# dafyddstephenson/ucla-roms

Hardware: AMD Instinct MI355X
Metric: grid-cell-updates/sec (higher is better)
Workload: dtype f64; 1 GPU; C3: basin 1024x1024x100, NONLIN+SPLIT EOS, T+S, LMD KPP/BKPP/RIMIX/NONLOCAL, dt=300s, ndtfast=60 (nfast=82); NT=2, nfast=82, parallelism=domain decomposition 1x1, halo_transport=none (single rank), fast_exchange_interval=1, exchange_order=none (single rank), s2d_window=True, comm_bootstrap=none (single rank)

## Files before the change

### include/roms_gpu.h

```cpp
#ifndef ROMS_GPU_H
#define ROMS_GPU_H

#ifdef __cplusplus
extern "C" {
#endif

#define ROMS_GPU_ABI_VERSION 20
#define ROMS_MAX_FAST 288

typedef struct roms_dims {
  int Lm, Mm, N, NT;
  int LLm, MMm;
  int np_xi, np_eta, inode, jnode;
  int iSW_corn, jSW_corn;
  int ew_periodic, ns_periodic;
  int west_exchng, east_exchng, south_exchng, north_exchng;
} roms_dims;

#define ROMS_LMD_MIXING   1
#define ROMS_LMD_KPP      2
#define ROMS_LMD_BKPP     4
#define ROMS_LMD_RIMIX    8
#define ROMS_LMD_CONVEC   16
#define ROMS_LMD_NONLOCAL 32
#define ROMS_LMD_ALL      63
#define ROMS_LMD_ICELAND  47
#define ROMS_LMD_DDMIX    64

typedef struct roms_cfg {
  int nonlin_eos;
  int salinity;
  int lmd_mixing;
  int uv_vis2, ts_dif2;
  double dt;
  int ndtfast, nfast;
  double weight[2][ROMS_MAX_FAST];
  double g, rho0, rdrg, rdrg2, Zob, gamma2;
  double Akv_bak, Akt_bak[2];
  double Tcoef, T0, Scoef, S0;
  double theta_s, theta_b, hc;
  int obc;
  double ubind;
  int curvgrid;
  int uv_adv, uv_cor;
  int pot_tides;
  int bulk_frc;
  int adv_isoneutral;
} roms_cfg;

typedef struct roms_tlev {
  int iic, ntstart, forw_start, iif, nfast, kstp, knew, nstp, nrhs, nnew;
} roms_tlev;

enum roms_field {
  ROMS_ALL = -1,
  ROMS_h = 0, ROMS_hinv, ROMS_f, ROMS_fomn, ROMS_pm, ROMS_pn, ROMS_dm_r, ROMS_dn_r, ROMS_dm_u, ROMS_dn_u,
  ROMS_dm_v, ROMS_dn_v, ROMS_dm_p, ROMS_dn_p, ROMS_pmon_u, ROMS_pnom_v, ROMS_rmask, ROMS_pmask, ROMS_umask,
  ROMS_vmask,
  ROMS_Cs_w, ROMS_Cs_r,
  ROMS_zeta, ROMS_ubar, ROMS_vbar, ROMS_u, ROMS_v, ROMS_t, ROMS_FlxU, ROMS_FlxV, ROMS_We, ROMS_Wi,
  ROMS_Hz, ROMS_Hz_u, ROMS_Hz_v, ROMS_z_r, ROMS_z_w,
  ROMS_rufrc, ROMS_rvfrc, ROMS_rhoA, ROMS_rhoS, ROMS_r_D, ROMS_Zt_avg1, ROMS_DU_avg1, ROMS_DV_avg1,
  ROMS_DU_avg2, ROMS_DV_avg2, ROMS_DU_avg_bak, ROMS_DV_avg_bak,
  ROMS_rho, ROMS_rho1, ROMS_qp1, ROMS_bvf, ROMS_Akv, ROMS_Akt, ROMS_visc2_r, ROMS_visc2_p, ROMS_diff2,
  ROMS_hbls, ROMS_hbbl, ROMS_ghat, ROMS_swr_frac,
  ROMS_sustr, ROMS_svstr, ROMS_stflx, ROMS_srflx, ROMS_swflx,
  ROMS_ru, ROMS_rv,
  ROMS_zeta_west, ROMS_zeta_east, ROMS_zeta_south, ROMS_zeta_north,
  ROMS_ubar_west, ROMS_ubar_east, ROMS_ubar_south, ROMS_ubar_north,
  ROMS_vbar_west, ROMS_vbar_east, ROMS_vbar_south, ROMS_vbar_north,
  ROMS_u_west, ROMS_u_east, ROMS_u_south, ROMS_u_north,
  ROMS_v_west, ROMS_v_east, ROMS_v_south, ROMS_v_north,
  ROMS_t_west, ROMS_t_east, ROMS_t_south, ROMS_t_north,
  ROMS_dndx, ROMS_dmde,
  ROMS_ptide,
  ROMS_uwnd, ROMS_vwnd, ROMS_tair, ROMS_qair, ROMS_prate, ROMS_swrad, ROMS_lwrad, ROMS_sustr_r, ROMS_svstr_r,
  ROMS_NFIELDS
};

int  roms_gpu_abi_version(void);
int  roms_gpu_init(const roms_dims *dims, const roms_cfg *cfg, int device, void *comm);
int  roms_gpu_finalize(void);
const char *roms_gpu_last_error(void);
long roms_gpu_field_size(int field_id);
int  roms_gpu_register(int field_id, double *host_ptr, long count);
int  roms_gpu_upload(int field_id);
int  roms_gpu_download(int field_id);
int  roms_gpu_copy_in(int field_id, const double *src, long count);
int  roms_gpu_copy_out(int field_id, double *dst, long count);
int  roms_gpu_sync(void);
void *roms_gpu_stream(void);

int roms_gpu_rho_eos(int tidx, const roms_tlev *t);
int roms_gpu_set_huv(const roms_tlev *t);
int roms_gpu_omega(const roms_tlev *t);
int roms_gpu_lmd_vmix(int tind, const roms_tlev *t);
int roms_gpu_prsgrd(const roms_tlev *t);
int roms_gpu_pre_step3d(const roms_tlev *t);
int roms_gpu_set_huv1(const roms_tlev *t);
int roms_gpu_step3d_uv1(const roms_tlev *t);
int roms_gpu_visc3d(const roms_tlev *t);
int roms_gpu_step2d(const roms_tlev *t);
int roms_gpu_step3d_uv2(const roms_tlev *t);
int roms_gpu_step3d_t(const roms_tlev *t);
int roms_gpu_t3dmix(const roms_tlev *t);
int roms_gpu_swr_frac(const roms_tlev *t);
int roms_gpu_set_pipe_frc(int npip, const int *pipe_idx, const double *pipe_flx, const double *pipe_prf,
                          const double *pipe_trc);
int roms_gpu_set_river_frc(int nriv, const double *riv_uflx, const double *riv_vflx, const double *riv_vol,
                           const double *riv_trc);
int roms_gpu_bulk_flux(const roms_tlev *t);
int roms_gpu_set_ub_tune(const double *ub_west, const double *ub_east, const double *ub_south, const double *ub_north);
int roms_gpu_set_depth(const roms_tlev *t);

int roms_gpu_step(roms_tlev *t);
int roms_gpu_init_sequence(roms_tlev *t);

enum roms_case_id { ROMS_CASE_FILAMENT = 0, ROMS_CASE_BASIN = 1, ROMS_CASE_PIPES = 2, ROMS_CASE_RIVERS = 3 };
typedef struct roms_case {
  int case_id, LLm, MMm, N, NT;
  int salinity, nonlin_eos, lmd_mixing;
  double dt; int ndtfast;
  double sizex, sizey;
  int surf_flux;
  int obc;
  double v_sponge;
  int island;
  int curvgrid;
  int uv_adv, uv_cor;
  int bulk_frc;
  int adv_isoneutral;
} roms_case;
int roms_gpu_init_case(const roms_case *c, int device, roms_tlev *t);
int roms_gpu_init_case_comm(const roms_case *c, int np_xi, int np_eta, void *comm, int device, roms_tlev *t);

int roms_gpu_comm_unique_id(void *id128);
int roms_gpu_comm_create(const void *id128, int nranks, int rank, int device, void **comm);
int roms_gpu_comm_create_local(int group, int nranks, int rank, void **comm);
typedef int (*roms_host_allgather_fn)(void *ctx, const void *send, long nbytes, void *recv);
int roms_gpu_comm_create_host(int nranks, int rank, int device, roms_host_allgather_fn allgather, void *ctx,
                              void **comm);
int roms_gpu_comm_destroy(void *comm);
int roms_gpu_halo_transport(void);
int roms_gpu_halo_exchanges(long *per_step, int *fast_interval);
int roms_gpu_halo_overlap(void);
int roms_gpu_s2d_window(void);
#define ROMS_COLPATH_SEG 1
#define ROMS_COLPATH_GLOBAL 2
int roms_gpu_column_path(void);
int roms_gpu_kpp_lean(void);
int roms_gpu_vgrid(void);
int roms_gpu_vgrid_check(long out[3]);
int roms_gpu_horizontal_path(int out[8]);
int roms_gpu_selftest_zero_fill(long n, int chunks, long *bad);
int roms_gpu_halo_plan(int Lm, int Mm, int np_xi, int np_eta, int inode, int jnode, int ew_periodic,
                       int ns_periodic, int peer[8], long count[8], int strip[4]);
long roms_gpu_halo_map(int Lm, int Mm, int np_xi, int np_eta, int inode, int jnode, int ew_periodic,
                       int ns_periodic, int dir, int unpack, int *i, int *j, long cap);
long roms_gpu_halo_map_wide(int Lm, int Mm, int np_xi, int np_eta, int inode, int jnode, int ew_periodic,
                            int ns_periodic, int width, int dir, int unpack, int *i, int *j, long cap);

#define ROMS_FRC_SURFACE 1
#define ROMS_FRC_BRY     2
int roms_gpu_frc_record(int field_id, int slot, double rec_time, const double *data);
int roms_gpu_frc_interp(double modtime, int kinds);
int roms_gpu_frc_clock(double start_time, int on);
int roms_gpu_set_tide_data(int ntides, const double *ftide, const double *pot_re, const double *pot_im,
                           const double *ztide_re, const double *ztide_im, const double *utide_re,
                           const double *utide_im, const double *vtide_re, const double *vtide_im);
int roms_gpu_set_tides(double time);

#define ROMS_WRT_Z    1
#define ROMS_WRT_UB   2
#define ROMS_WRT_VB   4
#define ROMS_WRT_U    8
#define ROMS_WRT_V    16
#define ROMS_WRT_T    32
#define ROMS_WRT_R    64
#define ROMS_WRT_O    128
#define ROMS_WRT_AKV  256
#define ROMS_WRT_AKT  512
#define ROMS_WRT_AKS  1024
#define ROMS_WRT_HBLS 2048
#define ROMS_WRT_HBBL 4096
#define ROMS_WRT_DEFAULT 63
int roms_gpu_wrt_rst(const char *path, int rec, int total_rec, double time, const roms_tlev *t);
int roms_gpu_wrt_his(const char *path, int rec, int total_rec, double time, const roms_tlev *t, int wrt_mask);
int roms_gpu_io_wait(void);
int roms_gpu_io_tracer_name(int itrc, const char *name, const char *units, const char *long_name);
int roms_gpu_get_init(const char *path, int req_rec, int tindx, roms_tlev *t, double *start_time);

int roms_gpu_diag(const roms_tlev *t, double norms[4]);
int roms_gpu_set_weights(int ndtfast, double weight[2][ROMS_MAX_FAST]);
int roms_gpu_time_steps(roms_tlev *t, int n, double *ms);
enum roms_routine {
  ROMS_R_RHO_EOS = 0, ROMS_R_SET_HUV, ROMS_R_OMEGA, ROMS_R_PRSGRD, ROMS_R_PRE_STEP3D, ROMS_R_SET_HUV1,
  ROMS_R_STEP3D_UV1, ROMS_R_VISC3D, ROMS_R_STEP2D, ROMS_R_STEP3D_UV2, ROMS_R_STEP3D_T, ROMS_R_T3DMIX,
  ROMS_R_LMD_VMIX,
  ROMS_R_K_S2D_FB,
  ROMS_R_K_PRE_UV_SEG,
  ROMS_R_K_UV1_SEG,
  ROMS_R_K_STEP3D_T_SEG,
  ROMS_R_K_PRSGRD_UV,
  ROMS_R_K_HALO_PACK,
  ROMS_R_K_HALO_WAIT,
  ROMS_R_K_HALO_UNPACK,
  ROMS_R_COUNT
};
int roms_gpu_time_routine(int routine, int nsteps, roms_tlev *t, double *avg_ms, long *launches);

#ifdef __cplusplus
}
#endif
#endif
```

### ucla-roms_amd/csrc/k_chain.h

```cpp
#pragma once
#include "roms_dev.h"

namespace roms {

constexpr int kChainCW = 16;
constexpr int kChainG = 4;

struct ChainLane {
  int col, g;
  int i, j;
  int lo, nk;
  bool in;
};
template <int KL>
__device__ __forceinline__ ChainLane chain_lane(const Range& R, const uint3& bI, int N) {
  ChainLane c;
  const int l = (int)(threadIdx.x & 63u), w = (int)(threadIdx.x >> 6);
  c.col = l & (kChainCW - 1);
  c.g = l / kChainCW;
  c.i = tile_i0(R.i0) + (int)bI.x * kChainCW + c.col;
  c.in = c.i >= R.i0;
  c.j = R.j0 + (int)bI.y * 4 + w;
  c.lo = 1 + c.g * KL;
  c.nk = max(0, min(N, c.lo + KL - 1) - c.lo + 1);
  return c;
}
inline dim3 chain_grid_of(const Range& R) {
  return dim3((R.i1 - tile_i0(R.i0) + kChainCW) / kChainCW, (R.j1 - R.j0 + 4) / 4);
}
inline int chain_kl(int N) {
  const int kl = (N + kChainG - 1) / kChainG;
  return kl <= 5 ? 5 : kl <= 13 ? 13 : kl <= 25 ? 25 : 0;
}

template <class Body>
__device__ __forceinline__ void chain_down(const ChainLane& c, double& s1, double& s2, Body&& body) {
  s1 = 0.0; s2 = 0.0;
#pragma unroll
  for (int st = kChainG - 1; st >= 0; st--) {
    const double in1 = __shfl_down(s1, kChainCW), in2 = __shfl_down(s2, kChainCW);
    if (c.g == st) {
      if (st < kChainG - 1) { s1 = in1; s2 = in2; }
      body(s1, s2);
    }
  }
  s1 = __shfl(s1, c.col);
  s2 = __shfl(s2, c.col);
}
template <class Body>
__device__ __forceinline__ void chain_up(const ChainLane& c, double& s, Body&& body) {
  s = 0.0;
#pragma unroll
  for (int st = 0; st < kChainG; st++) {
    const double in = __shfl_up(s, kChainCW);
    if (c.g == st) {
      if (st > 0) s = in;
      body(s);
    }
  }
  s = __shfl(s, (kChainG - 1) * kChainCW + c.col);
}

}
```

### ucla-roms_amd/csrc/k_step3d_t.hip

```cpp
#include "k_colseg.h"

namespace roms {

__global__ void __launch_bounds__(256) k_step3d_t_h(Dev d, Range R, int nnew, int nrhs, int up) {
  const uint3 bI = xcd_tile();
  __shared__ TracerWin W;
  const Bounds& b = d.b;
  const Fields& F = d.f;
  const int k = 1 + (int)bI.z;
  const int i0 = tile_i0(R.i0) + (int)bI.x * kBX, j0 = R.j0 + (int)bI.y * kBY;
  const int ib = i0 - 2, jb = j0 - 2;
  const long kk = (long)(k - 1) * b.n2;
  tracer_win_fill(b, F, W, ib, jb, kk, nullptr);
  const int i = i0 + (int)threadIdx.x, j = j0 + (int)threadIdx.y;
  const bool act = i >= R.i0 && i <= R.i1 && j <= R.j1;
  const long ij = IJ(b, i, j), o = ij + kk;
  const AccTL a{W.T, W.UM, W.VM, W.FU, W.FV, ib, jb};
  for (int itrc = 1; itrc <= b.NT; itrc++) {
    const long tb = (long)(itrc - 1) * 3 * b.n3;
    const double* Tr = F.t + (long)(nrhs - 1) * b.n3 + tb;
    __syncthreads();
    tracer_win_fill(b, F, W, ib, jb, kk, Tr);
    __syncthreads();
    if (!act) continue;
// ... 435 lines not shown
    const double c = DC0 * LD(Wi, vo, w);
    fc = in ? f : 0.0;
    wc = in ? c : 0.0;
  };
  double fcl, wcl;
  fcw(0, fcl, wcl);
  __syncthreads();
  SegTri<KR> T;
  T.template eliminate<ROMS_SEG_T_GROUP>(n, [&](int p, double& a, double& bb, double& c, double& dd) {
    double fcu, wcu;
    fcw(p + 1, fcu, wcu);
    a = -(fcl + fmax0(wcl));
    bb = hz[p + 1] + fcu + fmax0(wcu) + fcl - fmin0(wcl);
    c = -(fcu - fmin0(wcu));
    dd = rhs[p];
    fcl = fcu; wcl = wcu;
  });
  double xL, xR;
  T.couple(sg, n, X, xL, xR);
  T.solve(n, xL, xR);
  const double rm = BufF64(F.rmask).ld(vo, 0);
  const unsigned vs = act ? vo : kBufOff;
#pragma unroll
  for (int p = 0; p < KR; p++) Tn.st(T.D[p] * rm, (p < n ? vs : kBufOff) + lev(c0 + p), 0u);
}

void setup_column_kernels_t(size_t bytes) {
  (void)hipFuncSetAttribute((const void*)k_step3d_t_v<ColLds>, hipFuncAttributeMaxDynamicSharedMemorySize,
                            (int)bytes);
  (void)hipFuncSetAttribute((const void*)k_step3d_t_v<ColLds, true>, hipFuncAttributeMaxDynamicSharedMemorySize,
                            (int)bytes);
}

void launch_step3d_t(const Dev& d, hipStream_t s, const Tlev& t, bool exchange) {
  const Bounds& b = d.b;
  Range R{b.istr, b.iend, b.jstr, b.jend};
  if (d.p.iso) {
    hipLaunchKernelGGL(k_step3d_t_h, grid3_of(R, b.N), dim3(kBX, kBY), 0, s, d, R, t.nnew, t.nrhs, 0);
    for (int itrc = 1; itrc <= b.NT; itrc++) launch_iso_tracer(d, s, t, itrc);
    dim3 gt = gridc_of(R);
    gt.z = b.NT;
    if (d.f.colscr)
      hipLaunchKernelGGL((k_step3d_t_v<ColGlb, true>), gt, dim3(kCX), 0, s, d, R, t.nnew, t.nrhs);
    else
      hipLaunchKernelGGL((k_step3d_t_v<ColLds, true>), gt, dim3(kCX), col_lds_bytes(2, b.N), s, d, R, t.nnew, t.nrhs);
    for (int itrc = 1; itrc <= b.NT; itrc++) launch_t3dbc(d, s, t, itrc);
    launch_exchange_tracers(d, s, t.nnew);
    return;
  }
  auto h_tiles = [&](const Range& r) {
    const dim3 gh = grid3_of(r, b.N), bh(kBX, kBY);
    if (d.p.hoist && b.NT == 2)
      hipLaunchKernelGGL(k_step3d_t_h1<2>, gh, bh, 0, s, d, r, t.nnew, t.nrhs);
    else if (d.p.hoist && b.NT == 1)
      hipLaunchKernelGGL(k_step3d_t_h1<1>, gh, bh, 0, s, d, r, t.nnew, t.nrhs);
    else
      hipLaunchKernelGGL(k_step3d_t_h, gh, bh, 0, s, d, r, t.nnew, t.nrhs, 1);
  };
  auto run = [&](const Range& r) {
    int jA = 0, jB = -1;
    if (d.p.hoist && launch_tracer_strip(d, s, r, 0, true, false, t.nnew, t.nrhs, 0.0, 0.0, 0.0, 0, jA, jB)) {
      if (jA > r.j0) h_tiles(Range{r.i0, r.i1, r.j0, jA - 1});
      if (jB < r.j1) h_tiles(Range{r.i0, r.i1, jB + 1, r.j1});
    } else {
      h_tiles(r);
    }
    dim3 gt = gridc_of(r);
    gt.z = b.NT;
    if (d.p.colseg) {
      ktimer_mark(s, kTimedStep3dTSeg, 0);
      if (d.p.seg_buf)
        hipLaunchKernelGGL(k_step3d_t_segb, seg_grid_of(r, b.NT), dim3(kCX, seg_waves(b.N)), 0, s, d, r, t.nnew, t.nrhs);
      else
        hipLaunchKernelGGL(k_step3d_t_seg, seg_grid_of(r, b.NT), dim3(kCX, seg_waves(b.N)), 0, s, d, r, t.nnew, t.nrhs);
      ktimer_mark(s, kTimedStep3dTSeg, 1, 1);
    }
    else if (d.f.colscr)
      hipLaunchKernelGGL(k_step3d_t_v<ColGlb>, gt, dim3(kCX), 0, s, d, r, t.nnew, t.nrhs);
    else
      hipLaunchKernelGGL(k_step3d_t_v<ColLds>, gt, dim3(kCX), col_lds_bytes(2, b.N), s, d, r, t.nnew, t.nrhs);
  };
  auto edges = [&] {
    for (int itrc = 1; itrc <= b.NT; itrc++) launch_t3dbc(d, s, t, itrc);
  };
  ExchList L;
  if (!exchange) {
    run(R);
    edges();
  } else if (tracer_exch_list(d, t.nnew, L)) {
    launch_rim_first(d, s, R, L, run, edges);
  } else {
    run(R);
    edges();
    launch_exchange_tracers(d, s, t.nnew);
  }
}

__global__ void __launch_bounds__(256) k_t3dmix(Dev d, Range R, int nnew, int nrhs) {
  ROMS_IJ_OR_RETURN(R)
  const Bounds& b = d.b;
  const Fields& F = d.f;
  const long ij = IJ(b, i, j), sj = b.nx2, n2 = b.n2;
  const double* __restrict__ Hz = F.Hz;
  const double pmn = d.p.dt * F.pm[ij] * F.pn[ij];
  if (b.NT == 2) {
    double ax0[2], ax1[2], ay0[2], ay1[2];
    const double* __restrict__ Tr[2];
    double* __restrict__ Tn[2];
#pragma unroll
    for (int q = 0; q < 2; q++) {
      const double* d2 = F.diff2 + (long)q * n2;
      Tr[q] = F.t + (long)(nrhs - 1) * b.n3 + (long)q * 3 * b.n3;
      Tn[q] = F.t + (long)(nnew - 1) * b.n3 + (long)q * 3 * b.n3;
      ax0[q] = 0.25 * (d2[ij] + d2[ij - 1]) * F.pmon_u[ij];
      ax1[q] = 0.25 * (d2[ij + 1] + d2[ij]) * F.pmon_u[ij + 1];
      ay0[q] = 0.25 * (d2[ij] + d2[ij - sj]) * F.pnom_v[ij];
      ay1[q] = 0.25 * (d2[ij + sj] + d2[ij]) * F.pnom_v[ij + sj];
    }
    const double um0 = F.umask[ij], um1 = F.umask[ij + 1], vm0 = F.vmask[ij], vm1 = F.vmask[ij + sj];
#pragma unroll 2
    for (int k = 1; k <= b.N; k++) {
      const long o = ij + (long)(k - 1) * n2;
#pragma unroll
      for (int q = 0; q < 2; q++) {
        const double FX1 = ax1[q] * (Hz[o + 1] + Hz[o]) * (Tr[q][o + 1] - Tr[q][o]) * um1;
        const double FX0 = ax0[q] * (Hz[o] + Hz[o - 1]) * (Tr[q][o] - Tr[q][o - 1]) * um0;
        const double FE1 = ay1[q] * (Hz[o + sj] + Hz[o]) * (Tr[q][o + sj] - Tr[q][o]) * vm1;
        const double FE0 = ay0[q] * (Hz[o] + Hz[o - sj]) * (Tr[q][o] - Tr[q][o - sj]) * vm0;
        Tn[q][o] = Tn[q][o] + pmn * (FX1 - FX0 + FE1 - FE0) / Hz[o];
      }
    }
    return;
  }
  for (int itrc = 1; itrc <= b.NT; itrc++) {
    const double* d2 = F.diff2 + (long)(itrc - 1) * n2;
    const double* __restrict__ Tr = F.t + (long)(nrhs - 1) * b.n3 + (long)(itrc - 1) * 3 * b.n3;
    double* __restrict__ Tn = F.t + (long)(nnew - 1) * b.n3 + (long)(itrc - 1) * 3 * b.n3;
    const double ax0 = 0.25 * (d2[ij] + d2[ij - 1]) * F.pmon_u[ij], ax1 = 0.25 * (d2[ij + 1] + d2[ij]) * F.pmon_u[ij + 1];
    const double ay0 = 0.25 * (d2[ij] + d2[ij - sj]) * F.pnom_v[ij], ay1 = 0.25 * (d2[ij + sj] + d2[ij]) * F.pnom_v[ij + sj];
    const double um0 = F.umask[ij], um1 = F.umask[ij + 1], vm0 = F.vmask[ij], vm1 = F.vmask[ij + sj];
#pragma unroll 2
    for (int k = 1; k <= b.N; k++) {
      const long o = ij + (long)(k - 1) * n2;
      const double FX1 = ax1 * (Hz[o + 1] + Hz[o]) * (Tr[o + 1] - Tr[o]) * um1;
      const double FX0 = ax0 * (Hz[o] + Hz[o - 1]) * (Tr[o] - Tr[o - 1]) * um0;
      const double FE1 = ay1 * (Hz[o + sj] + Hz[o]) * (Tr[o + sj] - Tr[o]) * vm1;
      const double FE0 = ay0 * (Hz[o] + Hz[o - sj]) * (Tr[o] - Tr[o - sj]) * vm0;
      Tn[o] = Tn[o] + pmn * (FX1 - FX0 + FE1 - FE0) / Hz[o];
    }
  }
}

constexpr int kTMW = kBX + 2, kTMN = kTMW * (kBY + 2), kTMQ = (3 * kTMN + kBX * kBY - 1) / (kBX * kBY);
__global__ void __launch_bounds__(256) k_t3dmix_stg(Dev d, Range R, int nnew, int nrhs) {
  const uint3 bI = xcd_tile();
  __shared__ double sW[3 * kTMN];
  const Bounds& b = d.b;
  const Fields& F = d.f;
  const int i0 = tile_i0(R.i0) + (int)bI.x * kBX, j0 = R.j0 + (int)bI.y * kBY;
  int i = i0 + (int)threadIdx.x, j = j0 + (int)threadIdx.y;
  const bool act = i >= R.i0 && i <= R.i1 && j <= R.j1;
  if (!act) { i = i < R.i0 ? R.i0 : (i < R.i1 ? i : R.i1); j = j < R.j1 ? j : R.j1; }
  const long ij = IJ(b, i, j), sj = b.nx2, n2 = b.n2;
  const int tid = threadIdx.x + kBX * threadIdx.y;
  const double pmn = d.p.dt * F.pm[ij] * F.pn[ij];
  double ax0[2], ax1[2], ay0[2], ay1[2];
  double* __restrict__ Tn[2];
  const double* Tr[2];
#pragma unroll
  for (int q = 0; q < 2; q++) {
    const double* d2 = F.diff2 + (long)q * n2;
    Tr[q] = F.t + (long)(nrhs - 1) * b.n3 + (long)q * 3 * b.n3;
    Tn[q] = F.t + (long)(nnew - 1) * b.n3 + (long)q * 3 * b.n3;
    ax0[q] = 0.25 * (d2[ij] + d2[ij - 1]) * F.pmon_u[ij];
    ax1[q] = 0.25 * (d2[ij + 1] + d2[ij]) * F.pmon_u[ij + 1];
    ay0[q] = 0.25 * (d2[ij] + d2[ij - sj]) * F.pnom_v[ij];
    ay1[q] = 0.25 * (d2[ij + sj] + d2[ij]) * F.pnom_v[ij + sj];
  }
  const double um0 = F.umask[ij], um1 = F.umask[ij + 1], vm0 = F.vmask[ij], vm1 = F.vmask[ij + sj];
  long wo[kTMQ];
  int wf[kTMQ];
#pragma unroll
  for (int m = 0; m < kTMQ; m++) {
    const int q = tid + m * kBX * kBY;
    const int f = q < 3 * kTMN ? q / kTMN : -1, qq = q - (f < 0 ? 0 : f) * kTMN;
    const int ii = i0 - 1 + qq % kTMW, jj = j0 - 1 + qq / kTMW;
    const bool ok = f >= 0 && ii >= -1 && ii <= b.Lm + 2 && jj >= -1 && jj <= b.Mm + 2;
    wf[m] = ok ? f : -1;
    wo[m] = ok ? IJ(b, ii, jj) : 0;
  }
  auto ldw = [&](int k, double (&x)[kTMQ]) {
    const long kk = (long)(k - 1) * n2;
#pragma unroll
    for (int m = 0; m < kTMQ; m++)
      x[m] = wf[m] == 0 ? F.Hz[wo[m] + kk] : wf[m] == 1 ? Tr[0][wo[m] + kk] : wf[m] == 2 ? Tr[1][wo[m] + kk] : 0.0;
  };
  const int c = (threadIdx.x + 1) + (threadIdx.y + 1) * kTMW;
  double w[kTMQ];
  ldw(1, w);
  for (int k = 1; k <= b.N; k++) {
    const long o = ij + (long)(k - 1) * n2;
    const double tn0 = Tn[0][o], tn1 = Tn[1][o];
    if (k > 1) __syncthreads();
#pragma unroll
    for (int m = 0; m < kTMQ; m++) {
      const int q = tid + m * kBX * kBY;
      if (q < 3 * kTMN) sW[q] = w[m];
    }
    if (k < b.N) ldw(k + 1, w);
    __syncthreads();
    const double* H = sW;
    const double hz = H[c];
#pragma unroll
    for (int q = 0; q < 2; q++) {
      const double* T = sW + (1 + q) * kTMN;
      const double FX1 = ax1[q] * (H[c + 1] + hz) * (T[c + 1] - T[c]) * um1;
      const double FX0 = ax0[q] * (hz + H[c - 1]) * (T[c] - T[c - 1]) * um0;
      const double FE1 = ay1[q] * (H[c + kTMW] + hz) * (T[c + kTMW] - T[c]) * vm1;
      const double FE0 = ay0[q] * (hz + H[c - kTMW]) * (T[c] - T[c - kTMW]) * vm0;
      if (act) Tn[q][o] = (q == 0 ? tn0 : tn1) + pmn * (FX1 - FX0 + FE1 - FE0) / hz;
    }
  }
}

void launch_t3dmix(const Dev& d, hipStream_t s, const Tlev& t) {
  const Bounds& b = d.b;
  Range R{b.istr, b.iend, b.jstr, b.jend};
  const bool stg = d.p.t3dmix_stg && b.NT == 2;
  auto run = [&](const Range& r) {
    if (stg) hipLaunchKernelGGL(k_t3dmix_stg, grid_of(r), dim3(kBX, kBY), 0, s, d, r, t.nnew, t.nrhs);
    else hipLaunchKernelGGL(k_t3dmix, grid_of(r), dim3(kBX, kBY), 0, s, d, r, t.nnew, t.nrhs);
  };
  ExchList L;
  if (tracer_exch_list(d, t.nnew, L)) {
    launch_rim_first(d, s, R, L, run, [] {});
  } else {
    run(R);
    launch_exchange_tracers(d, s, t.nnew);
  }
}

}
```

### ucla-roms_amd/csrc/k_step3d_uv.hip

```cpp
#include <vector>

#include "k_colseg.h"
#include "k_chain.h"

namespace roms {

void launch_uv_horiz(const Dev& d, hipStream_t s, int nrhs, int up);

#ifndef ROMS_UV1_PF
#define ROMS_UV1_PF 8
#endif
constexpr int kUv1PF = ROMS_UV1_PF;
template <class C>
__device__ __forceinline__ void uv1_col(const Dev& d, int i, int j, int dir, int nnew, int nrhs, const C& A,
                                        const C& B) {
  const Bounds& b = d.b;
  const Fields& F = d.f;
  const int N = b.N;
  const double dt = d.p.dt;
  const long n2 = b.n2, ij = IJ(b, i, j);
  const long s = dir == 0 ? 1 : b.nx2;
  uv_vert_flux_lds<(kUv1PF > 0)>(d, ij, nrhs, dir, A, B);
  double* __restrict__ Un = (dir == 0 ? F.u : F.v) + (long)(nnew - 1) * b.n3 + ij;
  double* __restrict__ rr = (dir == 0 ? F.ru : F.rv) + ij;
// ... 375 lines not shown
    hipLaunchKernelGGL(k_uv1<ColLds>, g, dim3(kCX), col_lds_bytes(2, b.N), s, d, R, t.nnew, t.nrhs);
}

__device__ __forceinline__ void visc_rho(const Dev& d, int i, int j, int k, int nstp, double& UFx, double& VFe) {
  const Bounds& b = d.b;
  const Fields& F = d.f;
  const long ij = IJ(b, i, j), o = ij + (long)(k - 1) * b.n2, l = (long)(nstp - 1) * b.n3;
  const double* pm = F.pm;
  const double* pn = F.pn;
  const long sj = b.nx2;
  const double cff = 0.5 * F.Hz[o] * F.visc2_r[ij] *
                     (F.dn_r[ij] * pm[ij] * ((pn[ij] + pn[ij + 1]) * F.u[o + 1 + l] - (pn[ij - 1] + pn[ij]) * F.u[o + l]) -
                      F.dm_r[ij] * pn[ij] * ((pm[ij] + pm[ij + sj]) * F.v[o + sj + l] - (pm[ij - sj] + pm[ij]) * F.v[o + l]));
  UFx = cff * F.dn_r[ij] * F.dn_r[ij];
  VFe = -cff * F.dm_r[ij] * F.dm_r[ij];
}
__device__ __forceinline__ void visc_psi(const Dev& d, int i, int j, int k, int nstp, double& UFe, double& VFx) {
  const Bounds& b = d.b;
  const Fields& F = d.f;
  const long sj = b.nx2;
  const long ij = IJ(b, i, j), o = ij + (long)(k - 1) * b.n2, l = (long)(nstp - 1) * b.n3;
  const double* pm = F.pm;
  const double* pn = F.pn;
  const double cff =
      0.125 * (F.Hz[o - 1] + F.Hz[o] + F.Hz[o - 1 - sj] + F.Hz[o - sj]) * F.visc2_p[ij] *
      (0.25 * (pm[ij - 1] + pm[ij] + pm[ij - 1 - sj] + pm[ij - sj]) * F.dn_p[ij] *
           ((pn[ij - sj] + pn[ij]) * F.v[o + l] - (pn[ij - 1 - sj] + pn[ij - 1]) * F.v[o - 1 + l]) +
       0.25 * (pn[ij - 1] + pn[ij] + pn[ij - 1 - sj] + pn[ij - sj]) * F.dm_p[ij] *
           ((pm[ij - 1] + pm[ij]) * F.u[o + l] - (pm[ij - 1 - sj] + pm[ij - sj]) * F.u[o - sj + l])) *
      F.pmask[ij];
  UFe = cff * F.dm_p[ij] * F.dm_p[ij];
  VFx = cff * F.dn_p[ij] * F.dn_p[ij];
}

constexpr int kVW = kBX + 1, kVN = kVW * (kBY + 1), kVQ = (kVN + kBX * kBY - 1) / (kBX * kBY);
struct ViscRho {
  double v2, X, sx1, sx0, Y, sy1, sy0, dn, dm;
  long ij;
  bool on;
};
struct ViscPsi {
  double v2, P1, P2, a1, a0, b1, b0, msk, dm, dn;
  long ij;
  bool on;
};
__global__ void __launch_bounds__(256) k_visc3d(Dev d, Range R, int nstp) {
  const uint3 bI = xcd_tile();
  __shared__ double sUFx[kVN], sVFe[kVN], sUFe[kVN], sVFx[kVN];
  const Bounds& b = d.b;
  const Fields& F = d.f;
  const int indx = 3 - nstp;
  const int i0 = tile_i0(R.i0) + (int)bI.x * kBX, j0 = R.j0 + (int)bI.y * kBY;
  const long sj = b.nx2;
  const double* pm = F.pm;
  const double* pn = F.pn;
  const int tid = threadIdx.x + kBX * threadIdx.y;
  ViscRho gr[kVQ];
  ViscPsi gp[kVQ];
#pragma unroll
  for (int m = 0; m < kVQ; m++) {
    const int q = tid + m * kBX * kBY;
    const int li = q % kVW, lj = q / kVW;
    const int ir = i0 - 1 + li, jr = j0 - 1 + lj;
    ViscRho& r = gr[m];
    r.on = q < kVN && ir >= 0 && ir <= b.Lm + 1 && jr >= 0 && jr <= b.Mm + 1;
    r.ij = IJ(b, ir, jr);
    if (r.on) {
      const long ij = r.ij;
      r.v2 = F.visc2_r[ij];
      r.X = F.dn_r[ij] * pm[ij]; r.sx1 = pn[ij] + pn[ij + 1]; r.sx0 = pn[ij - 1] + pn[ij];
      r.Y = F.dm_r[ij] * pn[ij]; r.sy1 = pm[ij] + pm[ij + sj]; r.sy0 = pm[ij - sj] + pm[ij];
      r.dn = F.dn_r[ij]; r.dm = F.dm_r[ij];
    }
    const int ip = i0 + li, jp = j0 + lj;
    ViscPsi& p = gp[m];
    p.on = q < kVN && ip >= 0 && ip <= b.Lm + 2 && jp >= 0 && jp <= b.Mm + 2;
    p.ij = IJ(b, ip, jp);
    if (p.on) {
      const long ij = p.ij;
      p.v2 = F.visc2_p[ij];
      p.P1 = 0.25 * (pm[ij - 1] + pm[ij] + pm[ij - 1 - sj] + pm[ij - sj]) * F.dn_p[ij];
      p.a1 = pn[ij - sj] + pn[ij]; p.a0 = pn[ij - 1 - sj] + pn[ij - 1];
      p.P2 = 0.25 * (pn[ij - 1] + pn[ij] + pn[ij - 1 - sj] + pn[ij - sj]) * F.dm_p[ij];
      p.b1 = pm[ij - 1] + pm[ij]; p.b0 = pm[ij - 1 - sj] + pm[ij - sj];
      p.msk = F.pmask[ij]; p.dm = F.dm_p[ij]; p.dn = F.dn_p[ij];
    }
  }
  const int i = i0 + (int)threadIdx.x, j = j0 + (int)threadIdx.y;
  const bool act = i >= R.i0 && i <= R.i1 && j <= R.j1;
  const long ij = IJ(b, i, j);
  const bool du = act && i >= b.istrU && i <= b.iend, dv = act && j >= b.jstrV && j <= b.jend;
  double cum = 0.0, cun = 0.0, cvm = 0.0, cvn = 0.0, fu = 0.0, fv = 0.0;
  if (du) { cum = pm[ij - 1] + pm[ij]; cun = pn[ij - 1] + pn[ij]; fu = F.rufrc[ij]; }
  if (dv) { cvm = pm[ij] + pm[ij - sj]; cvn = pn[ij] + pn[ij - sj]; fv = F.rvfrc[ij]; }
  const double cu0 = 0.125 * cum * cun, cv0 = 0.125 * cvm * cvn;
  const double* U = F.u + (long)(nstp - 1) * b.n3;
  const double* V = F.v + (long)(nstp - 1) * b.n3;
  double* Ui = F.u + (long)(indx - 1) * b.n3;
  double* Vi = F.v + (long)(indx - 1) * b.n3;
  const int qr = (threadIdx.x + 1) + (threadIdx.y + 1) * kVW;
  const int qp = threadIdx.x + threadIdx.y * kVW;
  for (int k = 1; k <= b.N; k++) {
    const long kk = (long)(k - 1) * b.n2;
    const double* Hk = F.Hz + kk;
    const double* Uk = U + kk;
    const double* Vk = V + kk;
    const double ui = du ? Ui[ij + kk] : 0.0, vi = dv ? Vi[ij + kk] : 0.0;
    if (k > 1) __syncthreads();
#pragma unroll
    for (int m = 0; m < kVQ; m++) {
      const int q = tid + m * kBX * kBY;
      if (q >= kVN) break;
      double ufx = 0.0, vfe = 0.0, ufe = 0.0, vfx = 0.0;
      const ViscRho& r = gr[m];
      if (r.on) {
        const long o = r.ij;
        const double cff = 0.5 * Hk[o] * r.v2 * (r.X * (r.sx1 * Uk[o + 1] - r.sx0 * Uk[o]) -
                                                 r.Y * (r.sy1 * Vk[o + sj] - r.sy0 * Vk[o]));
        ufx = cff * r.dn * r.dn;
        vfe = -cff * r.dm * r.dm;
      }
      const ViscPsi& p = gp[m];
      if (p.on) {
        const long o = p.ij;
        const double cff = 0.125 * (Hk[o - 1] + Hk[o] + Hk[o - 1 - sj] + Hk[o - sj]) * p.v2 *
                           (p.P1 * (p.a1 * Vk[o] - p.a0 * Vk[o - 1]) + p.P2 * (p.b1 * Uk[o] - p.b0 * Uk[o - sj])) *
                           p.msk;
        ufe = cff * p.dm * p.dm;
        vfx = cff * p.dn * p.dn;
      }
      sUFx[q] = ufx; sVFe[q] = vfe; sUFe[q] = ufe; sVFx[q] = vfx;
    }
    __syncthreads();
    const long o = ij + kk;
    if (du) {
      const double cff = cu0 * (cun * (sUFx[qr] - sUFx[qr - 1]) + cum * (sUFe[qp + kVW] - sUFe[qp]));
      Ui[o] = ui + d.p.dt * cff;
      fu = fu + cff;
    }
    if (dv) {
      const double cff = cv0 * (cvn * (sVFx[qp + 1] - sVFx[qp]) + cvm * (sVFe[qr] - sVFe[qr - kVW]));
      Vi[o] = vi + d.p.dt * cff;
      fv = fv + cff;
    }
  }
  if (du) F.rufrc[ij] = fu;
  if (dv) F.rvfrc[ij] = fv;
}

constexpr int kVUW = kBX + 3, kVUN = kVUW * (kBY + 2);
constexpr int kVVW = kBX + 2, kVVN = kVVW * (kBY + 3);
constexpr int kVHW = kBX + 2, kVHN = kVHW * (kBY + 2);
constexpr int kVSN = kVUN + kVVN + kVHN, kVSQ = (kVSN + kBX * kBY - 1) / (kBX * kBY);
__global__ void __launch_bounds__(256, 3) k_visc3d_stg(Dev d, Range R, int nstp) {
  const uint3 bI = xcd_tile();
  __shared__ double sUFx[kVN], sVFe[kVN], sUFe[kVN], sVFx[kVN];
  __shared__ double sRaw[kVSN];
  const Bounds& b = d.b;
  const Fields& F = d.f;
  const int indx = 3 - nstp;
  const int i0 = tile_i0(R.i0) + (int)bI.x * kBX, j0 = R.j0 + (int)bI.y * kBY;
  const long sj = b.nx2;
  const double* pm = F.pm;
  const double* pn = F.pn;
  const int tid = threadIdx.x + kBX * threadIdx.y;
  ViscRho gr[kVQ];
  ViscPsi gp[kVQ];
#pragma unroll
  for (int m = 0; m < kVQ; m++) {
    const int q = tid + m * kBX * kBY;
    const int li = q % kVW, lj = q / kVW;
    const int ir = i0 - 1 + li, jr = j0 - 1 + lj;
    ViscRho& r = gr[m];
    r.on = q < kVN && ir >= 0 && ir <= b.Lm + 1 && jr >= 0 && jr <= b.Mm + 1;
    r.ij = IJ(b, ir, jr);
    if (r.on) {
      const long ij = r.ij;
      r.v2 = F.visc2_r[ij];
      r.X = F.dn_r[ij] * pm[ij]; r.sx1 = pn[ij] + pn[ij + 1]; r.sx0 = pn[ij - 1] + pn[ij];
      r.Y = F.dm_r[ij] * pn[ij]; r.sy1 = pm[ij] + pm[ij + sj]; r.sy0 = pm[ij - sj] + pm[ij];
      r.dn = F.dn_r[ij]; r.dm = F.dm_r[ij];
    }
    const int ip = i0 + li, jp = j0 + lj;
    ViscPsi& p = gp[m];
    p.on = q < kVN && ip >= 0 && ip <= b.Lm + 2 && jp >= 0 && jp <= b.Mm + 2;
    p.ij = IJ(b, ip, jp);
    if (p.on) {
      const long ij = p.ij;
      p.v2 = F.visc2_p[ij];
      p.P1 = 0.25 * (pm[ij - 1] + pm[ij] + pm[ij - 1 - sj] + pm[ij - sj]) * F.dn_p[ij];
      p.a1 = pn[ij - sj] + pn[ij]; p.a0 = pn[ij - 1 - sj] + pn[ij - 1];
      p.P2 = 0.25 * (pn[ij - 1] + pn[ij] + pn[ij - 1 - sj] + pn[ij - sj]) * F.dm_p[ij];
      p.b1 = pm[ij - 1] + pm[ij]; p.b0 = pm[ij - 1 - sj] + pm[ij - sj];
      p.msk = F.pmask[ij]; p.dm = F.dm_p[ij]; p.dn = F.dn_p[ij];
    }
  }
  const double* U = F.u + (long)(nstp - 1) * b.n3;
  const double* V = F.v + (long)(nstp - 1) * b.n3;
  long wo[kVSQ];
  int wf[kVSQ];
#pragma unroll
  for (int m = 0; m < kVSQ; m++) {
    const int q = tid + m * kBX * kBY;
    int ii = 0, jj = 0, f = -1;
    if (q < kVUN) { f = 0; ii = i0 - 1 + q % kVUW; jj = j0 - 1 + q / kVUW; }
    else if (q < kVUN + kVVN) { const int qq = q - kVUN; f = 1; ii = i0 - 1 + qq % kVVW; jj = j0 - 1 + qq / kVVW; }
    else if (q < kVSN) { const int qq = q - kVUN - kVVN; f = 2; ii = i0 - 1 + qq % kVHW; jj = j0 - 1 + qq / kVHW; }
    if (f >= 0 && !(ii >= -1 && ii <= b.Lm + 2 && jj >= -1 && jj <= b.Mm + 2)) f = -1;
    wf[m] = f;
    wo[m] = f >= 0 ? IJ(b, ii, jj) : 0;
  }
  auto ldraw = [&](int k, double (&x)[kVSQ]) {
    const long kk = (long)(k - 1) * b.n2;
#pragma unroll
    for (int m = 0; m < kVSQ; m++)
      x[m] = wf[m] == 0 ? U[wo[m] + kk] : wf[m] == 1 ? V[wo[m] + kk] : wf[m] == 2 ? F.Hz[wo[m] + kk] : 0.0;
  };
  auto Uw = [&](int ii, int jj) { return sRaw[(ii - (i0 - 1)) + (jj - (j0 - 1)) * kVUW]; };
  auto Vw = [&](int ii, int jj) { return sRaw[kVUN + (ii - (i0 - 1)) + (jj - (j0 - 1)) * kVVW]; };
  auto Hw = [&](int ii, int jj) { return sRaw[kVUN + kVVN + (ii - (i0 - 1)) + (jj - (j0 - 1)) * kVHW]; };
  const int i = i0 + (int)threadIdx.x, j = j0 + (int)threadIdx.y;
  const bool act = i >= R.i0 && i <= R.i1 && j <= R.j1;
  const long ij = IJ(b, i, j);
  const bool du = act && i >= b.istrU && i <= b.iend, dv = act && j >= b.jstrV && j <= b.jend;
  double cum = 0.0, cun = 0.0, cvm = 0.0, cvn = 0.0, fu = 0.0, fv = 0.0;
  if (du) { cum = pm[ij - 1] + pm[ij]; cun = pn[ij - 1] + pn[ij]; fu = F.rufrc[ij]; }
  if (dv) { cvm = pm[ij] + pm[ij - sj]; cvn = pn[ij] + pn[ij - sj]; fv = F.rvfrc[ij]; }
  const double cu0 = 0.125 * cum * cun, cv0 = 0.125 * cvm * cvn;
  double* Ui = F.u + (long)(indx - 1) * b.n3;
  double* Vi = F.v + (long)(indx - 1) * b.n3;
  const int qr = (threadIdx.x + 1) + (threadIdx.y + 1) * kVW;
  const int qp = threadIdx.x + threadIdx.y * kVW;
  double raw[kVSQ];
  ldraw(1, raw);
  double nui = du ? Ui[ij] : 0.0, nvi = dv ? Vi[ij] : 0.0;
  for (int k = 1; k <= b.N; k++) {
    const long kk = (long)(k - 1) * b.n2;
    const double ui = nui, vi = nvi;
#pragma unroll
    for (int m = 0; m < kVSQ; m++) {
      const int q = tid + m * kBX * kBY;
      if (q < kVSN) sRaw[q] = raw[m];
    }
    if (k < b.N) {
      ldraw(k + 1, raw);
      nui = du ? Ui[ij + kk + b.n2] : 0.0;
      nvi = dv ? Vi[ij + kk + b.n2] : 0.0;
    }
    __syncthreads();
#pragma unroll
    for (int m = 0; m < kVQ; m++) {
      const int q = tid + m * kBX * kBY;
      if (q >= kVN) break;
      const int li = q % kVW, lj = q / kVW;
      double ufx = 0.0, vfe = 0.0, ufe = 0.0, vfx = 0.0;
      const ViscRho& r = gr[m];
      if (r.on) {
        const int ir = i0 - 1 + li, jr = j0 - 1 + lj;
        const double cff = 0.5 * Hw(ir, jr) * r.v2 * (r.X * (r.sx1 * Uw(ir + 1, jr) - r.sx0 * Uw(ir, jr)) -
                                                      r.Y * (r.sy1 * Vw(ir, jr + 1) - r.sy0 * Vw(ir, jr)));
        ufx = cff * r.dn * r.dn;
        vfe = -cff * r.dm * r.dm;
      }
      const ViscPsi& p = gp[m];
      if (p.on) {
        const int ip = i0 + li, jp = j0 + lj;
        const double cff = 0.125 * (Hw(ip - 1, jp) + Hw(ip, jp) + Hw(ip - 1, jp - 1) + Hw(ip, jp - 1)) * p.v2 *
                           (p.P1 * (p.a1 * Vw(ip, jp) - p.a0 * Vw(ip - 1, jp)) +
                            p.P2 * (p.b1 * Uw(ip, jp) - p.b0 * Uw(ip, jp - 1))) *
                           p.msk;
        ufe = cff * p.dm * p.dm;
        vfx = cff * p.dn * p.dn;
      }
      sUFx[q] = ufx; sVFe[q] = vfe; sUFe[q] = ufe; sVFx[q] = vfx;
    }
    __syncthreads();
    const long o = ij + kk;
    if (du) {
      const double cff = cu0 * (cun * (sUFx[qr] - sUFx[qr - 1]) + cum * (sUFe[qp + kVW] - sUFe[qp]));
      Ui[o] = ui + d.p.dt * cff;
      fu = fu + cff;
    }
    if (dv) {
      const double cff = cv0 * (cvn * (sVFx[qp + 1] - sVFx[qp]) + cvm * (sVFe[qr] - sVFe[qr - kVW]));
      Vi[o] = vi + d.p.dt * cff;
      fv = fv + cff;
    }
  }
  if (du) F.rufrc[ij] = fu;
  if (dv) F.rvfrc[ij] = fv;
}

void launch_visc3d(const Dev& d, hipStream_t s, const Tlev& t) {
  const Bounds& b = d.b;
  Range R{b.istr, b.iend, b.jstr, b.jend};
  if (d.p.visc_stg)
    hipLaunchKernelGGL(k_visc3d_stg, grid_of(R), dim3(kBX, kBY), 0, s, d, R, t.nstp);
  else
    hipLaunchKernelGGL(k_visc3d, grid_of(R), dim3(kBX, kBY), 0, s, d, R, t.nstp);
}

__host__ __device__ __forceinline__ bool uv2_fused_in(const Bounds& b, int dir, int i, int j) {
  if (dir == 0)
    return i >= b.istrU && i <= b.iend && j >= b.jstr + (b.south_edge ? 1 : 0) && j <= b.jend - (b.north_edge ? 1 : 0);
  return i >= b.istr + (b.west_edge ? 1 : 0) && i <= b.iend - (b.east_edge ? 1 : 0) && j >= b.jstrV && j <= b.jend;
}

__global__ void __launch_bounds__(256) k_uv2_couple(Dev d, Range R, int nnew, int edges) {
  ROMS_IJ_OR_RETURN(R)
  const Bounds& b = d.b;
  const Fields& F = d.f;
  const int N = b.N;
  const long ij = IJ(b, i, j), n2 = b.n2;
  for (int dir = 0; dir < 2; dir++) {
    if (dir == 0 && !(i >= b.istrU)) continue;
    if (dir == 1 && !(j >= b.jstrV)) continue;
    if (edges && uv2_fused_in(b, dir, i, j)) continue;
    const long s = dir == 0 ? 1 : b.nx2;
    double* __restrict__ Un = (dir == 0 ? F.u : F.v) + (long)(nnew - 1) * b.n3 + ij;
    const double* __restrict__ Hz = F.Hz + ij;
    const double dn = dir == 0 ? F.dn_u[ij] : F.dm_v[ij];
    const double avg1 = dir == 0 ? F.DU_avg1[ij] : F.DV_avg1[ij];
    const double msk = dir == 0 ? F.umask[ij] : F.vmask[ij];
    long o = (long)(N - 1) * n2;
    double CF0 = 0.5 * (Hz[o] + Hz[o - s]);
    double DC0 = Un[o];
#pragma unroll 8
    for (int k = N - 1; k >= 1; k--) {
      o = (long)(k - 1) * n2;
      CF0 = CF0 + 0.5 * (Hz[o] + Hz[o - s]);
      DC0 = DC0 + Un[o];
    }
    DC0 = (DC0 * dn - avg1) / (CF0 * dn);
    constexpr int CH = 8;
    for (int k0 = 1; k0 <= N; k0 += CH) {
      double uc[CH], cc[CH];
#pragma unroll
      for (int q = 0; q < CH; q++) {
        const long oq = (long)(min(k0 + q, N) - 1) * n2;
        uc[q] = Un[oq];
        cc[q] = 0.5 * (Hz[oq] + Hz[oq - s]);
      }
#pragma unroll
      for (int q = 0; q < CH; q++)
        if (k0 + q <= N) Un[(long)(k0 + q - 1) * n2] = (uc[q] / cc[q] - DC0) * msk;
    }
  }
}

__global__ void __launch_bounds__(256) k_uv2_flux(Dev d, Range R, int nnew, int nstp, int knew, int iu0, int iu1, int iv0,
                                                  int iv1, int edges) {
  ROMS_IJ_OR_RETURN(R)
  const Bounds& b = d.b;
  const Fields& F = d.f;
  const int N = b.N;
  const long ij = IJ(b, i, j), n2 = b.n2;
  const double DELTA = 0.28, EPSIL = 0.36;
  for (int dir = 0; dir < 2; dir++) {
    if (dir == 0 && !(i >= iu0 && i <= iu1)) continue;
    if (dir == 1 && !(i >= iv0 && i <= iv1 && j >= b.jstr)) continue;
    if (edges && uv2_fused_in(b, dir, i, j)) continue;
    const long s = dir == 0 ? 1 : b.nx2;
    double* __restrict__ Un = (dir == 0 ? F.u : F.v) + (long)(nnew - 1) * b.n3 + ij;
    const double* __restrict__ Us = (dir == 0 ? F.u : F.v) + (long)(nstp - 1) * b.n3 + ij;
    double* __restrict__ Flx = (dir == 0 ? F.FlxU : F.FlxV) + ij;
    const double* __restrict__ Hz = F.Hz + ij;
    double* __restrict__ CFs = F.c0 + ij;
    const double dn = dir == 0 ? F.dn_u[ij] : F.dm_v[ij];
    const double avg1 = dir == 0 ? F.DU_avg1[ij] : F.DV_avg1[ij];
    const double avg2 = dir == 0 ? F.DU_avg2[ij] : F.DV_avg2[ij];
    const double msk = dir == 0 ? F.umask[ij] : F.vmask[ij];
    auto DCk = [&](int k) { const long o = (long)(k - 1) * n2; return 0.5 * (Hz[o] + Hz[o - s]) * dn; };
    long o = (long)(N - 1) * n2;
    const double dcN = DCk(N);
    double DC0 = dcN, FC0 = dcN * Un[o];
#pragma unroll 8
    for (int k = N - 1; k >= 1; k--) {
      o = (long)(k - 1) * n2;
      const double dck = DCk(k);
      DC0 = DC0 + dck;
      FC0 = FC0 + dck * Un[o];
    }
    DC0 = 1.0 / DC0;
    if (dir == 0) F.ubar[IJL(b, i, j, knew)] = DC0 * avg1;
    else F.vbar[IJL(b, i, j, knew)] = DC0 * avg1;
    FC0 = DC0 * (FC0 - avg1);
    double CF0 = 0.0;
    constexpr int CH = 8;
    for (int k0 = N; k0 >= 1; k0 -= CH) {
      double uc[CH], fc[CH], sc[CH], dc[CH];
#pragma unroll
      for (int q = 0; q < CH; q++) {
        const int k = max(k0 - q, 1);
        const long oq = (long)(k - 1) * n2;
        uc[q] = Un[oq]; fc[q] = Flx[oq]; sc[q] = Us[oq]; dc[q] = DCk(k);
      }
#pragma unroll
      for (int q = 0; q < CH; q++) {
        const int k = k0 - q;
        if (k >= 1) {
          const long oq = (long)(k - 1) * n2;
          const double un = (uc[q] - FC0) * msk;
          Un[oq] = un;
          const double cfk = DELTA * fc[q] + EPSIL * dc[q] * (sc[q] + un);
          CFs[(long)k * n2] = cfk;
          CF0 = CF0 + cfk;
        }
      }
    }
    CF0 = DC0 * (CF0 - avg2);
#pragma unroll 8
    for (int k = 1; k <= N; k++) {
      o = (long)(k - 1) * n2;
      Flx[o] = CFs[(long)k * n2] - DCk(k) * CF0;
    }
  }
}

template <int KL, bool FULL = false>
__global__ void __launch_bounds__(256, KL > 13 ? 3 : 4) k_uv2_fused(Dev d, Range R, int nnew, int nstp, int knew) {
  constexpr bool kHcLds = KL > 13;
  __shared__ double sHc[kHcLds ? KL * 256 : 1];
  const uint3 bI = xcd_tile();
  const Bounds& b = d.b;
  const Fields& F = d.f;
  const int N = b.N;
  const double DELTA = 0.28, EPSIL = 0.36;
  const ChainLane cl = chain_lane<KL>(R, bI, N);
  const int i = cl.i, j = cl.j, g = cl.g, lo = cl.lo, nk = FULL ? KL : cl.nk;
  const long n2 = b.n2;
  auto chain2 = [&](double& s1, double& s2, auto&& body) { chain_down(cl, s1, s2, body); };
  const int d0 = gridDim.z == 2 ? (int)bI.z : 0, d1 = gridDim.z == 2 ? d0 + 1 : 2;
  for (int dir = d0; dir < d1; dir++) {
    const int ilo = dir == 0 ? b.istrU : b.istr, jlo = dir == 0 ? b.jstr : b.jstrV;
    const int ic = min(max(i, ilo), b.iend), jc = min(max(j, jlo), b.jend);
    const bool act = ic == i && jc == j && cl.in && uv2_fused_in(b, dir, i, j);
    const long ij = IJ(b, ic, jc), s = dir == 0 ? 1 : b.nx2;
    const double dn = dir == 0 ? F.dn_u[ij] : F.dm_v[ij];
    const double avg1 = dir == 0 ? F.DU_avg1[ij] : F.DV_avg1[ij];
    const double avg2 = dir == 0 ? F.DU_avg2[ij] : F.DV_avg2[ij];
    const double msk = dir == 0 ? F.umask[ij] : F.vmask[ij];
    const double* const Ub = (dir == 0 ? F.u : F.v);
    const BufF64 bUn(Ub + (long)(nnew - 1) * b.n3, b.n3), bUs(Ub + (long)(nstp - 1) * b.n3, b.n3), bHz(F.Hz, b.n3),
        bFl(dir == 0 ? F.FlxU : F.FlxV, b.n3);
    const unsigned vo = (unsigned)((ij + (long)(lo - 1) * n2) * 8), vom = vo - (unsigned)(s * 8);
    auto so = [&](int q) { return (unsigned)((long)q * n2 * 8); };
    auto vq = [&](int q) { return q < nk ? vo : kBufOff; };
    auto vqm = [&](int q) { return q < nk ? vom : kBufOff; };
    auto vsq = [&](int q) { return act && q < nk ? vo : kBufOff; };
    double un[KL];
    double hcr[kHcLds ? 1 : KL];
    struct HcRef {
      double* l;
      double* r;
      __device__ __forceinline__ double& operator[](int q) const { return kHcLds ? l[q * 256] : r[q]; }
    } const hc{sHc + threadIdx.x, hcr};
#pragma unroll
    for (int q = 0; q < KL; q++) {
      un[q] = bUn.ld(vq(q), so(q));
      hc[q] = 0.5 * (bHz.ld(vq(q), so(q)) + bHz.ld(vqm(q), so(q)));
      if (q % 8 == 7) __builtin_amdgcn_sched_barrier(0);
    }
    double CF0, DC0;
    chain2(CF0, DC0, [&](double& a, double& c) {
#pragma unroll
      for (int q = KL - 1; q >= 0; q--) {
        a = q < nk ? a + hc[q] : a;
        c = q < nk ? c + un[q] : c;
      }
    });
    DC0 = (DC0 * dn - avg1) / (CF0 * dn);
#pragma unroll
    for (int q = 0; q < KL; q++) un[q] = (un[q] / hc[q] - DC0) * msk;
    double DS, FC0;
    chain2(DS, FC0, [&](double& a, double& c) {
#pragma unroll
      for (int q = KL - 1; q >= 0; q--) {
        const double dck = hc[q] * dn;
        a = q < nk ? a + dck : a;
        c = q < nk ? c + dck * un[q] : c;
      }
    });
    const double DCi = 1.0 / DS;
    if (act && g == 0) {
      if (dir == 0) F.ubar[IJL(b, i, j, knew)] = DCi * avg1;
      else F.vbar[IJL(b, i, j, knew)] = DCi * avg1;
    }
    FC0 = DCi * (FC0 - avg1);
    __builtin_amdgcn_sched_barrier(0);
#pragma unroll
    for (int q = 0; q < KL; q++) {
      const double u1 = (un[q] - FC0) * msk;
      bUn.st(u1, vsq(q), so(q));
      un[q] = DELTA * bFl.ld(vq(q), so(q)) + EPSIL * (hc[q] * dn) * (bUs.ld(vq(q), so(q)) + u1);
      if (q % 8 == 7) __builtin_amdgcn_sched_barrier(0);
    }
    double CS, unused;
    chain2(CS, unused, [&](double& a, double& c) {
#pragma unroll
      for (int q = KL - 1; q >= 0; q--) a = q < nk ? a + un[q] : a;
    });
    const double CF1 = DCi * (CS - avg2);
#pragma unroll
    for (int q = 0; q < KL; q++) bFl.st(un[q] - (hc[q] * dn) * CF1, vsq(q), so(q));
  }
}

template <int KL, bool kCouple>
__global__ void __launch_bounds__(256) k_uv2_edge(Dev d, const int* __restrict__ cols, int ncol, int nnew, int nstp,
                                                  int knew) {
  const Bounds& b = d.b;
  const Fields& F = d.f;
  const int N = b.N;
  const double DELTA = 0.28, EPSIL = 0.36;
  const int l = (int)(threadIdx.x & 63u), w = (int)(threadIdx.x >> 6);
  ChainLane cl;
  cl.col = l & (kChainCW - 1);
  cl.g = l / kChainCW;
  cl.lo = 1 + cl.g * KL;
  cl.nk = max(0, min(N, cl.lo + KL - 1) - cl.lo + 1);
  const int c = ((int)blockIdx.x * 4 + w) * kChainCW + cl.col;
  const bool act = c < ncol;
  const int cc = act ? c : ncol - 1;
  const int dir = cols[3 * cc], i = cols[3 * cc + 1], j = cols[3 * cc + 2];
  cl.i = i; cl.j = j; cl.in = true;
  const long n2 = b.n2, ij = IJ(b, i, j), s = dir == 0 ? 1 : b.nx2;
  auto chain2 = [&](double& s1, double& s2, auto&& body) { chain_down(cl, s1, s2, body); };
  double* __restrict__ Un = (dir == 0 ? F.u : F.v) + (long)(nnew - 1) * b.n3 + ij;
  const double* __restrict__ Hz = F.Hz + ij;
  const double dn = dir == 0 ? F.dn_u[ij] : F.dm_v[ij];
  const double avg1 = dir == 0 ? F.DU_avg1[ij] : F.DV_avg1[ij];
  const double msk = dir == 0 ? F.umask[ij] : F.vmask[ij];
  double un[KL], hc[KL];
#pragma unroll
  for (int q = 0; q < KL; q++) {
    if (q < cl.nk) {
      const long o = (long)(cl.lo + q - 1) * n2;
      un[q] = Un[o];
      hc[q] = 0.5 * (Hz[o] + Hz[o - s]);
    }
  }
  if constexpr (kCouple) {
    double CF0, DC0;
    chain2(CF0, DC0, [&](double& a, double& c2) {
#pragma unroll
      for (int q = KL - 1; q >= 0; q--)
        if (q < cl.nk) { a = a + hc[q]; c2 = c2 + un[q]; }
    });
    DC0 = (DC0 * dn - avg1) / (CF0 * dn);
    if (act) {
#pragma unroll
      for (int q = 0; q < KL; q++)
        if (q < cl.nk) Un[(long)(cl.lo + q - 1) * n2] = (un[q] / hc[q] - DC0) * msk;
    }
  } else {
    const double* __restrict__ Us = (dir == 0 ? F.u : F.v) + (long)(nstp - 1) * b.n3 + ij;
    double* __restrict__ Flx = (dir == 0 ? F.FlxU : F.FlxV) + ij;
    const double avg2 = dir == 0 ? F.DU_avg2[ij] : F.DV_avg2[ij];
    double DS, FC0;
    chain2(DS, FC0, [&](double& a, double& c2) {
#pragma unroll
      for (int q = KL - 1; q >= 0; q--)
        if (q < cl.nk) { const double dck = hc[q] * dn; a = a + dck; c2 = c2 + dck * un[q]; }
    });
    const double DCi = 1.0 / DS;
    if (act && cl.g == 0) {
      if (dir == 0) F.ubar[IJL(b, i, j, knew)] = DCi * avg1;
      else F.vbar[IJL(b, i, j, knew)] = DCi * avg1;
    }
    FC0 = DCi * (FC0 - avg1);
#pragma unroll
    for (int q = 0; q < KL; q++) {
      if (q < cl.nk) {
        const long o = (long)(cl.lo + q - 1) * n2;
        const double u1 = (un[q] - FC0) * msk;
        if (act) Un[o] = u1;
        un[q] = DELTA * Flx[o] + EPSIL * (hc[q] * dn) * (Us[o] + u1);
      }
    }
    double CS, unused;
    chain2(CS, unused, [&](double& a, double& c2) {
#pragma unroll
      for (int q = KL - 1; q >= 0; q--)
        if (q < cl.nk) a = a + un[q];
    });
    const double CF1 = DCi * (CS - avg2);
    if (act) {
#pragma unroll
      for (int q = 0; q < KL; q++)
        if (q < cl.nk) Flx[(long)(cl.lo + q - 1) * n2] = un[q] - (hc[q] * dn) * CF1;
    }
  }
}

void uv2_edge_lists(const Bounds& b, std::vector<int>& couple, std::vector<int>& flux) {
  couple.clear();
  flux.clear();
  if (!(b.west_edge || b.east_edge || b.south_edge || b.north_edge)) return;
  const int iu0 = b.istr, iu1 = b.ew_periodic ? b.iend : b.iendR;
  const int iv0 = b.ew_periodic ? b.istr : b.istrR, iv1 = b.ew_periodic ? b.iend : b.iendR;
  const int j0 = b.ns_periodic ? b.jstr : b.jstrR, j1 = b.ns_periodic ? b.jend : b.jendR;
  for (int dir = 0; dir < 2; dir++)
    for (int j = b.jstr; j <= b.jend; j++)
      for (int i = b.istr; i <= b.iend; i++) {
        if (dir == 0 && !(i >= b.istrU)) continue;
        if (dir == 1 && !(j >= b.jstrV)) continue;
        if (uv2_fused_in(b, dir, i, j)) continue;
        couple.insert(couple.end(), {dir, i, j});
      }
  for (int dir = 0; dir < 2; dir++)
    for (int j = j0; j <= j1; j++)
      for (int i = (iv0 < iu0 ? iv0 : iu0); i <= (iu1 > iv1 ? iu1 : iv1); i++) {
        if (dir == 0 && !(i >= iu0 && i <= iu1)) continue;
        if (dir == 1 && !(i >= iv0 && i <= iv1 && j >= b.jstr)) continue;
        if (uv2_fused_in(b, dir, i, j)) continue;
        flux.insert(flux.end(), {dir, i, j});
      }
}

void launch_step3d_uv2(const Dev& d, hipStream_t s, const Tlev& t) {
  const Bounds& b = d.b;
  Range R1{b.istr, b.iend, b.jstr, b.jend};
  const int iu0 = b.istr, iu1 = b.ew_periodic ? b.iend : b.iendR;
  const int iv0 = b.ew_periodic ? b.istr : b.istrR, iv1 = b.ew_periodic ? b.iend : b.iendR;
  const int j0 = b.ns_periodic ? b.jstr : b.jstrR, j1 = b.ns_periodic ? b.jend : b.jendR;
  Range R2{iv0 < iu0 ? iv0 : iu0, iu1 > iv1 ? iu1 : iv1, j0, j1};
  const int kl = (b.N + 3) / 4;
  if (!d.p.obc && d.p.uv2_fused && kl <= 25) {
    dim3 gf = chain_grid_of(R1);
    gf.z = d.p.chain_dirz ? 2 : 1;
    if (kl <= 5) hipLaunchKernelGGL(k_uv2_fused<5>, gf, dim3(256), 0, s, d, R1, t.nnew, t.nstp, t.knew);
    else if (kl <= 13) hipLaunchKernelGGL(k_uv2_fused<13>, gf, dim3(256), 0, s, d, R1, t.nnew, t.nstp, t.knew);
    else if (b.N == 100) hipLaunchKernelGGL((k_uv2_fused<25, true>), gf, dim3(256), 0, s, d, R1, t.nnew, t.nstp, t.knew);
    else hipLaunchKernelGGL(k_uv2_fused<25>, gf, dim3(256), 0, s, d, R1, t.nnew, t.nstp, t.knew);
    if (d.f.uv2e_couple && d.p.uv2e_nc > 0 && d.p.uv2e_nf > 0) {
      const int nc = d.p.uv2e_nc, nf = d.p.uv2e_nf;
      const dim3 gc((nc + 63) / 64), gf2((nf + 63) / 64);
      if (kl <= 5) hipLaunchKernelGGL((k_uv2_edge<5, true>), gc, dim3(256), 0, s, d, d.f.uv2e_couple, nc, t.nnew, t.nstp, t.knew);
      else if (kl <= 13) hipLaunchKernelGGL((k_uv2_edge<13, true>), gc, dim3(256), 0, s, d, d.f.uv2e_couple, nc, t.nnew, t.nstp, t.knew);
      else hipLaunchKernelGGL((k_uv2_edge<25, true>), gc, dim3(256), 0, s, d, d.f.uv2e_couple, nc, t.nnew, t.nstp, t.knew);
      launch_u3dbc(d, s, t);
      launch_v3dbc(d, s, t);
      if (kl <= 5) hipLaunchKernelGGL((k_uv2_edge<5, false>), gf2, dim3(256), 0, s, d, d.f.uv2e_flux, nf, t.nnew, t.nstp, t.knew);
      else if (kl <= 13) hipLaunchKernelGGL((k_uv2_edge<13, false>), gf2, dim3(256), 0, s, d, d.f.uv2e_flux, nf, t.nnew, t.nstp, t.knew);
      else hipLaunchKernelGGL((k_uv2_edge<25, false>), gf2, dim3(256), 0, s, d, d.f.uv2e_flux, nf, t.nnew, t.nstp, t.knew);
    } else if (b.west_edge || b.east_edge || b.south_edge || b.north_edge) {
      hipLaunchKernelGGL(k_uv2_couple, grid_of(R1), dim3(kBX, kBY), 0, s, d, R1, t.nnew, 1);
      launch_u3dbc(d, s, t);
      launch_v3dbc(d, s, t);
      hipLaunchKernelGGL(k_uv2_flux, grid_of(R2), dim3(kBX, kBY), 0, s, d, R2, t.nnew, t.nstp, t.knew, iu0, iu1, iv0,
                         iv1, 1);
    }
  } else {
    hipLaunchKernelGGL(k_uv2_couple, grid_of(R1), dim3(kBX, kBY), 0, s, d, R1, t.nnew, 0);
    launch_u3dbc(d, s, t);
    launch_v3dbc(d, s, t);
    hipLaunchKernelGGL(k_uv2_flux, grid_of(R2), dim3(kBX, kBY), 0, s, d, R2, t.nnew, t.nstp, t.knew, iu0, iu1, iv0, iv1,
                       0);
  }
  if (d.p.iso) launch_iso_diff3(d, s, t, iu0, iu1, iv0, iv1, j0, j1);
  launch_river_uv(d, s, t.nnew, 0);
  if (d.p.iso) launch_iso_exch_diff3(d, s);
  launch_exchange_list(d, s, ExchList{{d.f.FlxU, d.f.u + (long)(t.nnew - 1) * b.n3, d.f.ubar + (long)(t.knew - 1) * b.n2,
                                        d.f.FlxV, d.f.v + (long)(t.nnew - 1) * b.n3, d.f.vbar + (long)(t.knew - 1) * b.n2},
                                       {b.N, b.N, 1, b.N, b.N, 1}, 6});
}

}
```

### ucla-roms_amd/csrc/k_vertical.hip

```cpp
#include "roms_dev.h"
#include "k_chain.h"
#include "k_colseg.h"

namespace roms {

__global__ void __launch_bounds__(256) k_set_depth(Dev d, Range R, int iic, int knew, int last) {
  ROMS_IJ_OR_RETURN(R)
  const Bounds& b = d.b;
  const Fields& F = d.f;
  const long ij = IJ(b, i, j);
  if (iic == 0) {
    F.hinv[ij] = 1.0 / (F.h[ij] + d.p.hc);
    if (i >= b.istr)
      F.DU_avg1[ij] = 0.5 * (F.h[IJ(b, i - 1, j)] + F.h[ij] + F.zeta[IJL(b, i, j, 1)] + F.zeta[IJL(b, i - 1, j, 1)]) *
                      F.dn_u[ij] * (F.ubar[IJL(b, i, j, 1)]);
    if (j >= b.jstr)
      F.DV_avg1[ij] = 0.5 * (F.h[ij] + F.h[IJ(b, i, j - 1)] + F.zeta[IJL(b, i, j, 1)] + F.zeta[IJL(b, i, j - 1, 1)]) *
                      F.dm_v[ij] * (F.vbar[IJL(b, i, j, 1)]);
  }
  const int N = b.N;
  const double hh = F.h[ij];
  const double hi = iic == 0 ? 1.0 / (hh + d.p.hc) : F.hinv[ij];
  double z;
  if (last) {
// ... 21 lines not shown
  const Bounds& b = d.b;
  const Fields& F = d.f;
  const long ij = IJ(b, i, j);
  const VGrid vg = vg_column(d, ij);
  auto differ = [](double a, double c) { return __builtin_bit_cast(long long, a) != __builtin_bit_cast(long long, c); };
  unsigned nw = 0, nr = 0, nh = 0;
  double zw_prev = vg.zw0();
  nw += differ(F.z_w[ij], zw_prev);
  for (int k = 1; k <= b.N; k++) {
    const double zw = vg.zw1(k);
    nw += differ(F.z_w[ij + (long)k * b.n2], zw);
    nr += differ(F.z_r[ij + (long)(k - 1) * b.n2], vg.zr(k));
    nh += differ(F.Hz[ij + (long)(k - 1) * b.n2], zw - zw_prev);
    zw_prev = zw;
  }
  if (nw) atomicAdd(cnt, (unsigned long long)nw);
  if (nr) atomicAdd(cnt + 1, (unsigned long long)nr);
  if (nh) atomicAdd(cnt + 2, (unsigned long long)nh);
}
void launch_vgrid_check(const Dev& d, hipStream_t s, unsigned long long* cnt) {
  const Bounds& b = d.b;
  const Range R{b.istrE, b.iendE, b.jstrE, b.jendE};
  hipLaunchKernelGGL(k_vgrid_check, grid_of(R), dim3(kBX, kBY), 0, s, d, R, cnt);
}

void launch_set_depth(const Dev& d, hipStream_t s, const Tlev& t, bool exchange, bool last) {
  const Bounds& b = d.b;
  Range R{b.istrR, b.iendR, b.jstrR, b.jendR};
  hipLaunchKernelGGL(k_set_depth, grid_of(R), dim3(kBX, kBY), 0, s, d, R, t.iic, t.knew, (int)last);
  if (t.iic == 0) launch_exchange(d, s, d.f.hinv, 1);
  if (exchange) launch_exchange_list(d, s, ExchList{{d.f.z_w, d.f.z_r, d.f.Hz, d.f.z_sd}, {b.N + 1, b.N, b.N, 1}, 4});
}

template <bool VG>
__global__ void __launch_bounds__(256) k_set_huv(Dev d, Range R, int nrhs, int huv) {
  ROMS_IJ_OR_RETURN(R)
  const Bounds& b = d.b;
  const Fields& F = d.f;
  const bool du = i >= b.istr && i <= b.iendR && j >= b.jstrR && j <= b.jendR;
  const bool dv = i >= b.istrR && i <= b.iendR && j >= b.jstr && j <= b.jendR;
  const long ij = IJ(b, i, j), n2 = b.n2;
  if constexpr (VG) {
    const double dnu = du ? F.dn_u[ij] : 0.0, dmv = dv ? F.dm_v[ij] : 0.0;
    const VGrid g0 = vg_column(d, ij), gx = vg_column(d, du ? ij - 1 : ij), gy = vg_column(d, dv ? ij - b.nx2 : ij);
    const double* __restrict__ U = F.u + (long)(nrhs - 1) * b.n3 + ij;
    const double* __restrict__ V = F.v + (long)(nrhs - 1) * b.n3 + ij;
    double* __restrict__ FU = F.FlxU + ij;
    double* __restrict__ FV = F.FlxV + ij;
    double* __restrict__ HU = F.Hz_u + ij;
    double* __restrict__ HV = F.Hz_v + ij;
    double w0 = g0.zw0(), wx = gx.zw0(), wy = gy.zw0();
#pragma unroll 4
    for (int k = 1; k <= b.N; k++) {
      const long o = (long)(k - 1) * n2;
      const double z0 = g0.zw1(k), zx = gx.zw1(k), zy = gy.zw1(k);
      const double hz = z0 - w0;
      if (du) {
        const double hzm = zx - wx;
        FU[o] = 0.5 * (hz + hzm) * dnu * (U[o]);
        if (huv) HU[o] = 0.5 * (hz + hzm);
      }
      if (dv) {
        const double hzm = zy - wy;
        FV[o] = 0.5 * (hz + hzm) * dmv * (V[o]);
        if (huv) HV[o] = 0.5 * (hz + hzm);
      }
      w0 = z0; wx = zx; wy = zy;
    }
    return;
  }
  const double dnu = du ? F.dn_u[ij] : 0.0, dmv = dv ? F.dm_v[ij] : 0.0;
  const double* __restrict__ Hz = F.Hz + ij;
  const double* __restrict__ U = F.u + (long)(nrhs - 1) * b.n3 + ij;
  const double* __restrict__ V = F.v + (long)(nrhs - 1) * b.n3 + ij;
  double* __restrict__ FU = F.FlxU + ij;
  double* __restrict__ FV = F.FlxV + ij;
  double* __restrict__ HU = F.Hz_u + ij;
  double* __restrict__ HV = F.Hz_v + ij;
#pragma unroll 4
  for (int k = 1; k <= b.N; k++) {
    const long o = (long)(k - 1) * n2;
    const double hz = Hz[o];
    if (du) {
      const double hzm = Hz[o - 1];
      FU[o] = 0.5 * (hz + hzm) * dnu * (U[o]);
      if (huv) HU[o] = 0.5 * (hz + hzm);
    }
    if (dv) {
      const double hzm = Hz[o - b.nx2];
      FV[o] = 0.5 * (hz + hzm) * dmv * (V[o]);
      if (huv) HV[o] = 0.5 * (hz + hzm);
    }
  }
}

void launch_set_huv(const Dev& d, hipStream_t s, const Tlev& t, bool store_huv) {
  const Bounds& b = d.b;
  Range R{b.istrR < b.istr ? b.istrR : b.istr, b.iendR, b.jstrR < b.jstr ? b.jstrR : b.jstr, b.jendR};
  launch_rim_first(
      d, s, R, ExchList{{d.f.FlxU, d.f.FlxV}, {b.N, b.N}, 2},
      [&](const Range& r) {
        if (d.p.vg & kVgHuv)
          hipLaunchKernelGGL(k_set_huv<true>, grid_of(r), dim3(kBX, kBY), 0, s, d, r, t.nrhs, (int)store_huv);
        else
          hipLaunchKernelGGL(k_set_huv<false>, grid_of(r), dim3(kBX, kBY), 0, s, d, r, t.nrhs, (int)store_huv);
      },
      [] {});
}

__global__ void __launch_bounds__(256) k_set_huv1(Dev d, Range R, int nnew, int first) {
  ROMS_IJ_OR_RETURN(R)
  const Bounds& b = d.b;
  const Fields& F = d.f;
  const double NOW = 3.63, MID = 4.47, BAK = 2.05;
  const int N = b.N;
  const long ij = IJ(b, i, j), n2 = b.n2;
  for (int dir = 0; dir < 2; dir++) {
    if (dir == 0 && !(i >= b.istr && i <= b.iendR && j >= b.jstrR && j <= b.jendR)) continue;
    if (dir == 1 && !(i >= b.istrR && i <= b.iendR && j >= b.jstr && j <= b.jendR)) continue;
    const long s = dir == 0 ? 1 : b.nx2;
    const double dn = dir == 0 ? F.dn_u[ij] : F.dm_v[ij];
    double* __restrict__ u = (dir == 0 ? F.u : F.v) + (long)(nnew - 1) * b.n3 + ij;
    double* __restrict__ Flx = (dir == 0 ? F.FlxU : F.FlxV) + ij;
    const double* __restrict__ Hz = F.Hz + ij;
    long o = (long)(N - 1) * n2;
    double dcN = 0.5 * (Hz[o] + Hz[o - s]) * dn;
    double DC0 = dcN, FC0 = dcN * u[o];
#pragma unroll 8
    for (int k = N - 1; k >= 1; k--) {
      o = (long)(k - 1) * n2;
      const double dck = 0.5 * (Hz[o] + Hz[o - s]) * dn;
      DC0 = DC0 + dck;
      FC0 = FC0 + dck * u[o];
    }
    const double a1 = dir == 0 ? F.DU_avg1[ij] : F.DV_avg1[ij];
    if (first) FC0 = (FC0 - a1) / DC0;
    else {
      const double a2 = dir == 0 ? F.DU_avg2[ij] : F.DV_avg2[ij];
      const double ab = dir == 0 ? F.DU_avg_bak[ij] : F.DV_avg_bak[ij];
      FC0 = (FC0 - NOW * a1 + MID * a2 - BAK * ab) / DC0;
    }
    const double um = dir == 0 ? F.umask[ij] : F.vmask[ij];
#pragma unroll 8
    for (int k = 1; k <= N; k++) {
      o = (long)(k - 1) * n2;
      const double dck = 0.5 * (Hz[o] + Hz[o - s]) * dn;
      const double un = (u[o] - FC0) * um;
      u[o] = un;
      Flx[o] = dck * (un);
    }
  }
}

template <int KL, bool FULL = false>
__global__ void __launch_bounds__(256, KL > 13 ? 3 : 4) k_set_huv1_chain(Dev d, Range R, int nnew, int first) {
  constexpr bool kDcLds = KL > 13;
  __shared__ double sDc[kDcLds ? KL * 256 : 1];
  const uint3 bI = xcd_tile();
  const Bounds& b = d.b;
  const Fields& F = d.f;
  const double NOW = 3.63, MID = 4.47, BAK = 2.05;
  const int N = b.N;
  const ChainLane cl = chain_lane<KL>(R, bI, N);
  const int nk = FULL ? KL : cl.nk;
  const long n2 = b.n2;
  const int d0 = gridDim.z == 2 ? (int)bI.z : 0, d1 = gridDim.z == 2 ? d0 + 1 : 2;
#pragma unroll 1
  for (int dir = d0; dir < d1; dir++) {
    const int ilo = dir == 0 ? b.istr : b.istrR, jlo = dir == 0 ? b.jstrR : b.jstr;
    const int ic = min(max(cl.i, ilo), b.iendR), jc = min(max(cl.j, jlo), b.jendR);
    const bool act = ic == cl.i && jc == cl.j && cl.in;
    const long ij = IJ(b, ic, jc), s = dir == 0 ? 1 : b.nx2;
    const double dn = dir == 0 ? F.dn_u[ij] : F.dm_v[ij];
    const BufF64 bU((dir == 0 ? F.u : F.v) + (long)(nnew - 1) * b.n3, b.n3), bHz(F.Hz, b.n3),
        bFl(dir == 0 ? F.FlxU : F.FlxV, b.n3);
    const unsigned vo = (unsigned)((ij + (long)(cl.lo - 1) * n2) * 8), vom = vo - (unsigned)(s * 8);
    auto so = [&](int q) { return (unsigned)((long)q * n2 * 8); };
    auto vq = [&](int q) { return q < nk ? vo : kBufOff; };
    auto vqm = [&](int q) { return q < nk ? vom : kBufOff; };
    auto vsq = [&](int q) { return act && q < nk ? vo : kBufOff; };
    double uu[KL], dcr[kDcLds ? 1 : KL];
    struct DcRef {
      double* l;
      double* r;
      __device__ __forceinline__ double& operator[](int q) const { return kDcLds ? l[q * 256] : r[q]; }
    } const dc{sDc + threadIdx.x, dcr};
#pragma unroll
    for (int q = 0; q < KL; q++) {
      uu[q] = bU.ld(vq(q), so(q));
      dc[q] = 0.5 * (bHz.ld(vq(q), so(q)) + bHz.ld(vqm(q), so(q))) * dn;
      if (q % 8 == 7) __builtin_amdgcn_sched_barrier(0);
    }
    double DC0, FC0;
    chain_down(cl, DC0, FC0, [&](double& a, double& c) {
#pragma unroll
      for (int q = KL - 1; q >= 0; q--) {
        a = q < nk ? a + dc[q] : a;
        c = q < nk ? c + dc[q] * uu[q] : c;
      }
    });
    const double a1 = dir == 0 ? F.DU_avg1[ij] : F.DV_avg1[ij];
    if (first) FC0 = (FC0 - a1) / DC0;
    else {
      const double a2 = dir == 0 ? F.DU_avg2[ij] : F.DV_avg2[ij];
      const double ab = dir == 0 ? F.DU_avg_bak[ij] : F.DV_avg_bak[ij];
      FC0 = (FC0 - NOW * a1 + MID * a2 - BAK * ab) / DC0;
    }
    const double um = dir == 0 ? F.umask[ij] : F.vmask[ij];
#pragma unroll
    for (int q = 0; q < KL; q++) {
      const double un = (uu[q] - FC0) * um;
      bU.st(un, vsq(q), so(q));
      bFl.st(dc[q] * (un), vsq(q), so(q));
    }
  }
}

void launch_set_huv1(const Dev& d, hipStream_t s, const Tlev& t) {
  const Bounds& b = d.b;
  Range R{b.istrR < b.istr ? b.istrR : b.istr, b.iendR, b.jstrR < b.jstr ? b.jstrR : b.jstr, b.jendR};
  const int kl = chain_kl(b.N), first = (int)(t.iic == t.forw_start);
  dim3 gc = chain_grid_of(R);
  gc.z = d.p.chain_dirz ? 2 : 1;
  if (d.p.chain && kl == 5) hipLaunchKernelGGL(k_set_huv1_chain<5>, gc, dim3(256), 0, s, d, R, t.nnew, first);
  else if (d.p.chain && kl == 13) hipLaunchKernelGGL(k_set_huv1_chain<13>, gc, dim3(256), 0, s, d, R, t.nnew, first);
  else if (d.p.chain && kl == 25 && b.N == 100)
    hipLaunchKernelGGL((k_set_huv1_chain<25, true>), gc, dim3(256), 0, s, d, R, t.nnew, first);
  else if (d.p.chain && kl == 25) hipLaunchKernelGGL(k_set_huv1_chain<25>, gc, dim3(256), 0, s, d, R, t.nnew, first);
  else hipLaunchKernelGGL(k_set_huv1, grid_of(R), dim3(kBX, kBY), 0, s, d, R, t.nnew, first);
  launch_exchange_list(d, s, ExchList{{d.f.FlxU, d.f.FlxV, d.f.u + (long)(t.nnew - 1) * b.n3,
                                        d.f.v + (long)(t.nnew - 1) * b.n3}, {b.N, b.N, b.N, b.N}, 4});
}

#ifndef ROMS_OMEGA_PF
#define ROMS_OMEGA_PF 4
#endif
__global__ void __launch_bounds__(256) k_omega(Dev d, Range R, double dtau) {
  ROMS_IJ_OR_RETURN(R)
  const Bounds& b = d.b;
  const Fields& F = d.f;
  const int N = b.N;
  const double cu_min = 0.6, cu_max = 1.0, cmnx_ratio = cu_min / cu_max, cutoff = 2.0 - cmnx_ratio,
               r4cmx = 0.25 / (1.0 - cmnx_ratio);
  const long ij = IJ(b, i, j), n2 = b.n2, sj = b.nx2;
  const double* __restrict__ FU = F.FlxU + ij;
  const double* __restrict__ FV = F.FlxV + ij;
  const double* __restrict__ Hz = F.Hz + ij;
  const double* __restrict__ zw = F.z_w + ij;
  double* __restrict__ Wi = F.Wi + ij;
  double* __restrict__ We = F.We + ij;
  auto cx = [&](long o) { return fmax0(FU[o + 1]) - fmin0(FU[o]) + fmax0(FV[o + sj]) - fmin0(FV[o]); };
  const int pidx = d.p.npip > 0 ? F.pipe_idx[ij] : 0;
  const double pflx = pidx > 0 ? F.pipe_flx[ij] : 0.0;
  const double* __restrict__ prf = pidx > 0 ? F.pipe_prf + (pidx - 1) : nullptr;
  auto div = [&](int k, double wi) {
    const long o = (long)(k - 1) * n2;
    wi = wi - FU[o + 1] + FU[o] - FV[o + sj] + FV[o];
    if (pidx > 0) wi = wi + pflx * prf[(long)(k - 1) * d.p.npip];
    return wi;
  };
  double wi = 0.0;
#pragma unroll 8
  for (int k = 1; k <= N; k++) wi = div(k, wi);
  wi = wi + F.swflx[ij] * F.dm_r[ij] * F.dn_r[ij];
  const double zw0 = zw[0];
  const double wrk = wi / (zw[(long)N * n2] - zw0);
  Wi[0] = 0.0;
  We[0] = 0.0;
  Wi[(long)N * n2] = 0.0;
  We[(long)N * n2] = 0.0;
  const double CX0 = dtau * F.pm[ij] * F.pn[ij];
#if ROMS_OMEGA_PF > 0
  struct Lv { double fu1, fu0, fv1, fv0, hz, zw; };
  auto ld = [&](int m) {
    m = m > N ? N : m;
    const long o = (long)(m - 1) * n2;
    return Lv{FU[o + 1], FU[o], FV[o + sj], FV[o], Hz[o], zw[o]};
  };
  Lv cur = ld(1);
  double cx_k = fmax0(cur.fu1) - fmin0(cur.fu0) + fmax0(cur.fv1) - fmin0(cur.fv0), hz_k = cur.hz;
  wi = 0.0;
  auto lev = [&](int k, const Lv& up) {
    const long o1 = (long)k * n2;
    wi = wi - cur.fu1 + cur.fu0 - cur.fv1 + cur.fv0;
    if (pidx > 0) wi = wi + pflx * prf[(long)(k - 1) * d.p.npip];
    double w = wi - wrk * (up.zw - zw0);
    const double cx_up = fmax0(up.fu1) - fmin0(up.fu0) + fmax0(up.fv1) - fmin0(up.fv0);
    const double hz_up = up.hz;
    const double c2d = dmax(cx_k, cx_up);
    const double dh = dmin(hz_k, hz_up);
    const double cw_max = cu_max * dh - c2d * CX0;
    double we;
    if (cw_max > 0.0) {
      const double cw_max2 = cw_max * cw_max;
      const double cw_min = cw_max * cmnx_ratio;
      const double cw = fabs(w) * CX0;
      double cff;
      if (cw < cw_min) cff = cw_max2;
      else if (cw < cutoff * cw_max) cff = cw_max2 + r4cmx * ((cw - cw_min) * (cw - cw_min));
      else cff = cw_max * cw;
      we = cw_max2 * w / cff;
      w = w - we;
    } else {
      we = 0.0;
    }
    We[o1] = we;
    Wi[o1] = w;
    cx_k = cx_up;
    hz_k = hz_up;
    cur = up;
  };
  constexpr int PF = ROMS_OMEGA_PF;
  Lv ring[PF];
#pragma unroll
  for (int q = 0; q < PF; q++) ring[q] = ld(2 + q);
  int k0 = 1;
  for (; k0 + PF - 1 <= N - 1; k0 += PF) {
#pragma unroll
    for (int q = 0; q < PF; q++) {
      const Lv up = ring[q];
      ring[q] = ld(k0 + q + 1 + PF);
      lev(k0 + q, up);
    }
  }
#pragma unroll
  for (int q = 0; q < PF; q++)
    if (k0 + q <= N - 1) lev(k0 + q, ring[q]);
}
#else
  double cx_k = cx(0), hz_k = Hz[0];
  wi = 0.0;
#pragma unroll 8
  for (int k = 1; k <= N - 1; k++) {
    const long o1 = (long)k * n2;
    wi = div(k, wi);
    double w = wi - wrk * (zw[o1] - zw0);
    const double cx_up = cx(o1);
    const double hz_up = Hz[o1];
    const double c2d = dmax(cx_k, cx_up);
    const double dh = dmin(hz_k, hz_up);
    const double cw_max = cu_max * dh - c2d * CX0;
    double we;
    if (cw_max > 0.0) {
      const double cw_max2 = cw_max * cw_max;
      const double cw_min = cw_max * cmnx_ratio;
      const double cw = fabs(w) * CX0;
      double cff;
      if (cw < cw_min) cff = cw_max2;
      else if (cw < cutoff * cw_max) cff = cw_max2 + r4cmx * ((cw - cw_min) * (cw - cw_min));
      else cff = cw_max * cw;
      we = cw_max2 * w / cff;
      w = w - we;
    } else {
      we = 0.0;
    }
    We[o1] = we;
    Wi[o1] = w;
    cx_k = cx_up;
    hz_k = hz_up;
  }
}
#endif

constexpr int kOmR = kSegRows;
constexpr int kOmCW = kCX, kOmBlock = kSegMaxS * kOmCW;
template <bool kHB, int CW = kOmCW>
__global__ void __launch_bounds__(kSegMaxS * CW, 2) k_omega_seg(Dev d, Range R, double dtau, double hcff) {
  const uint3 bI = xcd_tile();
  const Bounds& b = d.b;
  const Fields& F = d.f;
  const int N = b.N;
  const double cu_min = 0.6, cu_max = 1.0, cmnx_ratio = cu_min / cu_max, cutoff = 2.0 - cmnx_ratio,
               r4cmx = 0.25 / (1.0 - cmnx_ratio);
  SegSpan sg = seg_span<CW>(N);
  constexpr bool kU = CW == kCX;
  if constexpr (kU) seg_uniform<CW>(sg);
  const int s = sg.s, S = sg.S, c0 = sg.c0, n = sg.n, l = sg.col;
  const int iu = tile_i0(R.i0) + (int)bI.x * CW + l, ju = R.j0 + (int)bI.y;
  const bool act = iu >= R.i0 && iu <= R.i1 && ju <= R.j1;
  const int i = iu < R.i0 ? R.i0 : (iu < R.i1 ? iu : R.i1), j = ju < R.j1 ? ju : R.j1;
  const long ij = IJ(b, i, j), n2 = b.n2, sj = b.nx2;
  const unsigned vo = (unsigned)ij * 8u, lv = (unsigned)n2 * 8u;
  const BufF64 FU(F.FlxU), FV(F.FlxV), Hz(F.Hz), zw(F.z_w);
  auto LD = [&](const BufF64& B, unsigned v, unsigned o) { return kU ? B.ld(v, o) : B.ld(v + o, 0u); };
  auto ST = [&](const BufF64& B, double x, unsigned v, unsigned o) {
    if constexpr (kU) B.st(x, v, o);
    else B.st(x, v + o, 0u);
  };
  __shared__ double Lw[kSegMaxS][CW], Lcx[kSegMaxS][CW], Lhz[kSegMaxS][CW];
  __shared__ double Lte[kHB ? kSegMaxS : 1][CW], Lti[kHB ? kSegMaxS : 1][CW];
  double fu1[kOmR], fu0[kOmR], fv1[kOmR], fv0[kOmR], cx[kOmR], hz[kOmR], zk[kOmR];
#pragma unroll
  for (int q = 0; q < kOmR; q++) {
    const int k = min(c0 + q, N);
    const unsigned o = (unsigned)(k - 1) * lv;
    fu1[q] = LD(FU, vo + 8u, o); fu0[q] = LD(FU, vo, o); fv1[q] = LD(FV, vo + (unsigned)sj * 8u, o); fv0[q] = LD(FV, vo, o);
    hz[q] = LD(Hz, vo, o);
    zk[q] = LD(zw, vo, (unsigned)k * lv);
  }
  const double zw0 = zw.ld(vo, 0), zwN = zw.ld(vo, (unsigned)N * lv);
  const double wsrf = F.swflx[ij] * F.dm_r[ij] * F.dn_r[ij];
  const double CX0 = dtau * F.pm[ij] * F.pn[ij];
  const int pidx = d.p.npip > 0 ? F.pipe_idx[ij] : 0;
  const double pflx = pidx > 0 ? F.pipe_flx[ij] : 0.0;
  const double* __restrict__ prf = pidx > 0 ? F.pipe_prf + (pidx - 1) : nullptr;
#pragma unroll
  for (int q = 0; q < kOmR; q++) cx[q] = fmax0(fu1[q]) - fmin0(fu0[q]) + fmax0(fv1[q]) - fmin0(fv0[q]);
  const int nthr = (int)(blockDim.x * blockDim.y);
  int tl = (int)(threadIdx.x + blockDim.x * threadIdx.y);
  __asm__ volatile("" : "+v"(tl));
  if constexpr (kHB) {
#pragma unroll
    for (int q = 0; q < kOmR; q++) roms_smem[q * nthr + tl] = fu1[q] - fu0[q] + fv1[q] - fv0[q];
  }
  Lcx[s][l] = cx[0];
  Lhz[s][l] = hz[0];
  double wk[kOmR];
  for (int t = 0; t < S; t++) {
    if (s == t) {
      double wi = t == 0 ? 0.0 : Lw[t - 1][l];
#pragma unroll
      for (int q = 0; q < kOmR; q++) {
        double v = wi - fu1[q] + fu0[q] - fv1[q] + fv0[q];
        if (pidx > 0) v = v + pflx * prf[(long)(min(c0 + q, N) - 1) * d.p.npip];
        wi = q < n ? v : wi;
        wk[q] = wi;
      }
      Lw[t][l] = wi;
    }
    __syncthreads();
  }
  const double wrk = (Lw[S - 1][l] + wsrf) / (zwN - zw0);
  const double cx_top = s + 1 < S ? Lcx[s + 1][l] : 0.0, hz_top = s + 1 < S ? Lhz[s + 1][l] : 0.0;
  if (!kHB && !act) return;
  const BufF64 Wi(F.Wi), We(F.We);
  const unsigned vs = act ? vo : kBufOff;
  const double hbf = kHB ? hcff * F.pm[ij] * F.pn[ij] : 0.0;
  const BufF64 Hf(F.c2), Hb(F.c3);
  double we_p = 0.0, wi_p = 0.0, we_f = 0.0, wi_f = 0.0;
  int tr = tl;
  __asm__ volatile("" : "+v"(tr));
  auto hb_store = [&](int q, double we1, double wi1, double we0, double wi0) {
    const double div = roms_smem[q * nthr + tr];
    const double FlxDiv = hbf * (div + we1 + wi1 - we0 - wi0);
    const unsigned o = (unsigned)(c0 + q - 1) * lv;
    ST(Hf, hz[q] - FlxDiv, vs, o);
    ST(Hb, hz[q] + FlxDiv, vs, o);
  };
  if (s == 0) {
    ST(Wi, 0.0, vs, 0);
    ST(We, 0.0, vs, 0);
    ST(Wi, 0.0, vs, (unsigned)N * lv);
    ST(We, 0.0, vs, (unsigned)N * lv);
  }
#pragma unroll
  for (int q = 0; q < kOmR; q++) {
    const int k = c0 + q;
    double w = wk[q] - wrk * (zk[q] - zw0);
    const double cx_up = q + 1 < n ? cx[q + 1 < kOmR ? q + 1 : kOmR - 1] : cx_top;
    const double hz_up = q + 1 < n ? hz[q + 1 < kOmR ? q + 1 : kOmR - 1] : hz_top;
    const double c2d = dmax(cx[q], cx_up);
    const double dh = dmin(hz[q], hz_up);
    const double cw_max = cu_max * dh - c2d * CX0;
    double we;
    if (cw_max > 0.0) {
      const double cw_max2 = cw_max * cw_max;
      const double cw_min = cw_max * cmnx_ratio;
      const double cw = fabs(w) * CX0;
      double cff;
      if (cw < cw_min) cff = cw_max2;
      else if (cw < cutoff * cw_max) cff = cw_max2 + r4cmx * ((cw - cw_min) * (cw - cw_min));
      else cff = cw_max * cw;
      we = cw_max2 * w / cff;
      w = w - we;
    } else {
      we = 0.0;
    }
    if (q < n && k <= N - 1) {
      ST(We, we, vs, (unsigned)k * lv);
      ST(Wi, w, vs, (unsigned)k * lv);
    }
    if constexpr (kHB) {
      const double we1 = k <= N - 1 ? we : 0.0, wi1 = k <= N - 1 ? w : 0.0;
      if (q == 0) { we_f = we1; wi_f = wi1; }
      if (q >= 1 && q < n) hb_store(q, we1, wi1, we_p, wi_p);
      if (q == n - 1) { Lte[s][l] = we1; Lti[s][l] = wi1; }
      we_p = we1; wi_p = wi1;
    }
  }
  if constexpr (kHB) {
    __syncthreads();
    const double we0 = s > 0 ? Lte[s - 1][l] : 0.0, wi0 = s > 0 ? Lti[s - 1][l] : 0.0;
    hb_store(0, we_f, wi_f, we0, wi0);
  }
}

__global__ void k_omega_edges(Dev d) {
  const Bounds& b = d.b;
  const Fields& F = d.f;
  const int p = blockIdx.x * blockDim.x + threadIdx.x, k = (int)blockIdx.y;
  const int nj = b.jend - b.jstr + 1, ni = b.iend - b.istr + 1;
  int di = 0, dj = 0, si = 0, sj = 0;
  if (p < nj) {
    if (!b.west_edge) return;
    dj = sj = b.jstr + p; di = b.istr - 1; si = b.istr;
  } else if (p < 2 * nj) {
    if (!b.east_edge) return;
    dj = sj = b.jstr + p - nj; di = b.iend + 1; si = b.iend;
  } else if (p < 2 * nj + ni) {
    if (!b.south_edge) return;
    di = si = b.istr + p - 2 * nj; dj = b.jstr - 1; sj = b.jstr;
  } else if (p < 2 * nj + 2 * ni) {
    if (!b.north_edge) return;
    di = si = b.istr + p - 2 * nj - ni; dj = b.jend + 1; sj = b.jend;
  } else {
    const int c = p - 2 * nj - 2 * ni;
    if (c == 0 && b.west_edge && b.south_edge) { di = b.istr - 1; dj = b.jstr - 1; si = b.istr; sj = b.jstr; }
    else if (c == 1 && b.west_edge && b.north_edge) { di = b.istr - 1; dj = b.jend + 1; si = b.istr; sj = b.jend; }
    else if (c == 2 && b.east_edge && b.south_edge) { di = b.iend + 1; dj = b.jstr - 1; si = b.iend; sj = b.jstr; }
    else if (c == 3 && b.east_edge && b.north_edge) { di = b.iend + 1; dj = b.jend + 1; si = b.iend; sj = b.jend; }
    else return;
  }
  const long dst = IJ(b, di, dj) + (long)k * b.n2, src = IJ(b, si, sj) + (long)k * b.n2;
  F.We[dst] = F.We[src];
  F.Wi[dst] = F.Wi[src];
}

static size_t omega_hb_lds_bytes(unsigned nthr) { return (size_t)kOmR * nthr * sizeof(double); }
void setup_omega_seg() {
  (void)hipFuncSetAttribute((const void*)k_omega_seg<true>, hipFuncAttributeMaxDynamicSharedMemorySize,
                            (int)omega_hb_lds_bytes(kOmBlock));
}

template <bool kHB, int CW>
static void omega_seg_cw(const Dev& d, hipStream_t s, const Range& r, double dtau, double hcff) {
  const Bounds& b = d.b;
  const dim3 gs((r.i1 - tile_i0(r.i0) + CW) / CW, r.j1 - r.j0 + 1), bs(kCX, seg_waves<CW>(b.N));
  const size_t lds = kHB ? omega_hb_lds_bytes(bs.x * bs.y) : 0;
  hipLaunchKernelGGL((k_omega_seg<kHB, CW>), gs, bs, lds, s, d, r, dtau, hcff);
}
template <bool kHB>
static void omega_seg(const Dev& d, hipStream_t s, const Range& r, double dtau, double hcff) {
  if (d.p.omega_cw == 16) omega_seg_cw<kHB, 16>(d, s, r, dtau, hcff);
  else if (d.p.omega_cw == 32) omega_seg_cw<kHB, 32>(d, s, r, dtau, hcff);
  else omega_seg_cw<kHB, kOmCW>(d, s, r, dtau, hcff);
}

bool omega_takes_seg(const Dev& d, int width) {
  return d.p.omega_seg && d.b.N <= kSegRows * kSegMaxS && width >= 32;
}
bool launch_omega(const Dev& d, hipStream_t s, const Tlev& t, double hcff) {
  const Bounds& b = d.b;
  double dtau;
  if (t.nrhs == 3) dtau = d.p.dt;
  else if (t.iic == t.forw_start) dtau = 0.5 * d.p.dt;
  else dtau = 0.6 * d.p.dt;
  Range R{b.istr, b.iend, b.jstr, b.jend};
  const bool hb = hcff > 0.0 && omega_takes_seg(d, R.i1 - R.i0 + 1) && !rim_overlap_on(d, R);
  launch_rim_first(
      d, s, R, ExchList{{d.f.We, d.f.Wi}, {b.N + 1, b.N + 1}, 2},
      [&](const Range& r) {
        if (hb)
          omega_seg<true>(d, s, r, dtau, hcff);
        else if (omega_takes_seg(d, r.i1 - r.i0 + 1))
          omega_seg<false>(d, s, r, dtau, 0.0);
        else
          hipLaunchKernelGGL(k_omega, grid_of(r), dim3(kBX, kBY), 0, s, d, r, dtau);
      },
      [&] {
        if (b.west_edge || b.east_edge || b.south_edge || b.north_edge) {
          const int n = 2 * (b.jend - b.jstr + 1) + 2 * (b.iend - b.istr + 1) + 4;
          hipLaunchKernelGGL(k_omega_edges, dim3((n + 255) / 256, b.N + 1), dim3(256), 0, s, d);
        }
      });
  return hb;
}

struct PColumn {
  double g, grho, HalfGRho, qp2, zwN, ptide;
  bool split, tides;
  BufF64 Pb{nullptr};
  unsigned vP, lv;
  int N;
  double zC, rC, qC;
  double eZk, eRk, dZ1, dR1, P1, z1, v1;
  __device__ __forceinline__ double rhov(double r1, double q1, double z) const {
    if (split) {
      const double dpth = -z;
      return r1 + q1 * dpth * (1.0 - qp2 * dpth);
    }
    return r1;
  }
  __device__ __forceinline__ double eRof(double ru, double rl, double qu, double ql, double zu, double zl) const {
    if (split) {
      const double dpth = -0.5 * (zu + zl);
      return ru - rl + (qu - ql) * dpth * (1.0 - qp2 * dpth);
    }
    return ru - rl;
  }
  __device__ __forceinline__ void iter(int m, double zM, double rM, double qM) {
    const double OneFifth = 0.2, OneTwelfth = 1.0 / 12.0;
    if (m == N) {
      eZk = zC - zM;
      eRk = eRof(rC, rM, qC, qM, zC, zM);
      dZ1 = 0.0; dR1 = 0.0; P1 = 0.0; z1 = 0.0; v1 = 0.0;
    }
    double eZm, eRm;
    if (m >= 2) { eZm = zC - zM; eRm = eRof(rC, rM, qC, qM, zC, zM); }
    else { eZm = eZk; eRm = eRk; }
    const double dZk = [&] { const double c = 2.0 * eZk * eZm; return c / (eZk + eZm); }();
    double dRk;
    {
      const double c = 2.0 * eRk * eRm;
      dRk = c > 0.0 ? c / (eRk + eRm) : 0.0;
    }
    const double v0 = rhov(rC, qC, zC);
    if (split) {
      const double dpth = -zC;
      dRk = dRk - qC * dZk * (1.0 - 2.0 * qp2 * dpth);
    }
    double Pk;
    if (m == N) {
      const double rNm = rhov(rM, qM, zM);
      Pk = g * zwN + grho * (v0 + 0.5 * (v0 - rNm) * (zwN - zC) / (zC - zM)) * (zwN - zC);
      if (tides) Pk = Pk - g * ptide;
    } else {
      Pk = P1 + HalfGRho * ((v1 + v0) * (z1 - zC) -
                            OneFifth * ((dR1 - dRk) * (z1 - zC - OneTwelfth * (dZ1 + dZk)) -
                                        (dZ1 - dZk) * (v1 - v0 - OneTwelfth * (dR1 + dRk))));
    }
    Pb.st(Pk, vP, (unsigned)(m - 1) * lv);
    P1 = Pk;
    dZ1 = dZk; dR1 = dRk;
    eZk = eZm; eRk = eRm;
    z1 = zC; v1 = v0;
  }
  __device__ __forceinline__ void level(int k, double z, double r, double q) {
    if (k < N) iter(k + 1, z, r, q);
    zC = z; rC = r; qC = q;
  }
  __device__ __forceinline__ void last() { iter(1, 0.0, 0.0, 0.0); }
};
__device__ __forceinline__ PColumn p_column(const Dev& d, int i, int j, long ij, bool split, bool have_zwN = false,
                                            double zwN = 0.0) {
  const Bounds& b = d.b;
  PColumn c;
  c.g = d.p.g; c.grho = d.p.g / d.p.rho0; c.HalfGRho = 0.5 * c.grho; c.qp2 = d.p.qp2;
  c.split = split; c.tides = d.p.tides != 0; c.N = b.N; c.lv = (unsigned)b.n2 * 8u;
  const bool doP = i >= 0 && i <= b.Lm && j >= 0 && j <= b.Mm && i >= b.istrU - 1 && i <= b.iend;
  c.Pb = BufF64(d.f.P);
  c.vP = doP ? (unsigned)ij * 8u : kBufOff;
  c.zwN = have_zwN ? zwN : d.f.z_w[ij + (long)b.N * b.n2];
  c.ptide = c.tides ? d.f.ptide[ij] : 0.0;
  return c;
}

template <bool kP>
__global__ void __launch_bounds__(256) k_rho_eos_linear(Dev d, Range R, int tidx) {
  ROMS_IJ_OR_RETURN(R)
  const Bounds& b = d.b;
  const Fields& F = d.f;
  const Params& P = d.p;
  const int N = b.N;
  const long ij = IJ(b, i, j), n2 = b.n2;
  const double rm = F.rmask[ij];
  const double cff0 = P.salinity ? (P.Tcoef * P.T0 - P.Scoef * P.S0) : (P.Tcoef * P.T0);
  const double* __restrict__ T = F.t + (long)(tidx - 1) * b.n3 + ij;
  const double* __restrict__ Sa = T + 3 * b.n3;
  const double* __restrict__ Hz = F.Hz + ij;
  double* __restrict__ rho = F.rho + ij;
  const bool salt = P.salinity;
  auto rhok = [&](long o) {
    double r = cff0 - P.Tcoef * T[o];
    if (salt) r = r + P.Scoef * Sa[o];
    return r * rm;
  };
  PColumn pc;
  if constexpr (kP) pc = p_column(d, i, j, ij, false);
  const double* __restrict__ zrp = F.z_r + ij;
  long o = (long)(N - 1) * n2;
  double rk = rhok(o);
  rho[o] = rk;
  if constexpr (kP) pc.level(N, zrp[o], rk, 0.0);
  double cff = Hz[o] * rk;
  double rhoS = 0.5 * cff * Hz[o];
  double rhoA = cff;
#pragma unroll 8
  for (int k = N - 1; k >= 1; k--) {
    o = (long)(k - 1) * n2;
    rk = rhok(o);
    rho[o] = rk;
    if constexpr (kP) pc.level(k, zrp[o], rk, 0.0);
// ... 166 lines not shown
```

### ucla-roms_amd/csrc/roms_dev.h

```cpp
#pragma once
#include <hip/hip_runtime.h>
#include <cstddef>
#include <cstdint>

namespace roms {

constexpr int kMaxFast = 288;
constexpr int kRowAlign = 16;
constexpr int kAlignOff = 14;

struct Bounds {
  int Lm, Mm, N, NT, nTS, nx2;
  long n2, n3, n3w;
  int gx;
  int istr, iend, jstr, jend;
  int istrU, istrR, iendR, jstrV, jstrR, jendR;
  int istrE, iendE, jstrE, jendE;
  int west_edge, east_edge, south_edge, north_edge;
  int ew_periodic, ns_periodic;
  int west_exch, east_exch, south_exch, north_exch;
};

struct Params {
  int nonlin_eos, salinity, lmd, uv_vis2, ts_dif2;
  int lmd_rimix, lmd_convec, lmd_nonlocal;
  int lmd_ddmix;
  int iso;
  int uv_adv, uv_cor;
  int tides;
  int bulk_frc;
  int prs_split;
  int s2d_split;
  int colseg;
  int colreg;
  int uv2_fused;
  int chain;
  int seg_order;
  int seg_xg;
  int s2d_fold;
  int hoist;
  int chain_dirz;
  int prs_fuse_uv;
  int h_jc;
  int prs_buf;
  int prs_strip;
  int t_strip;
  int visc_stg;
  int t3dmix_stg;
  int kpp_ty;
  int uv1_lds;
  int omega_seg;
  int omega_cw;
  int p_in_rho;
  int omega_hb;
  int preuv_lds;
  int seg_jrows;
  int seg_buf;
  int reserved_[8];
  int s2d_k;
  int uv2e_nc, uv2e_nf;
  int npip;
  int nriv, nrivf;
  int curvgrid;
  int obc;
  short kpp_lean;
  short kpp_fckeep;
  short vgrid;
  short vg;
  double ubind;
  double dt, dtfast, g, rho0, vonKar, qp2, gamma2, hc;
  double rdrg, Zob, Tcoef, T0, Scoef, S0;
  double Akv_bak, Akt_bak[2];
};

struct Fields {
  double *h, *hinv, *f, *fomn, *pm, *pn, *dm_r, *dn_r, *dm_u, *dn_u, *dm_v, *dn_v, *dm_p, *dn_p,
      *pmon_u, *pnom_v, *rmask, *pmask, *umask, *vmask;
  double *dndx, *dmde;
  double* ptide;
  double *uwnd, *vwnd, *tair, *qair, *prate, *swrad, *lwrad, *sustr_r, *svstr_r;
  double *Cs_w, *Cs_r;
  double* z_sd;
  double *zeta, *ubar, *vbar, *u, *v, *t;
  double *FlxU, *FlxV, *We, *Wi, *Hz, *Hz_u, *Hz_v, *z_r, *z_w;
  double *rufrc, *rvfrc, *rhoA, *rhoS, *r_D, *Zt_avg1, *DU_avg1, *DV_avg1, *DU_avg2, *DV_avg2,
      *DU_avg_bak, *DV_avg_bak;
  double *rho, *rho1, *qp1, *bvf, *Akv, *Akt, *visc2_r, *visc2_p, *diff2;
  double *hbls, *hbbl, *ghat, *swr_frac;
  double *sustr, *svstr, *stflx, *srflx, *swflx;
  double *ru, *rv, *P, *rhos;
  double *c0, *c1, *c2, *c3;
  double *s0, *s1, *s2, *s3, *s4, *s5, *s6, *s7, *s8, *s9;
  double *lmd_rig, *lmd_hbl, *lmd_bbl, *lmd_Bo, *lmd_Bosol, *lmd_ustar;
  int* pipe_idx;
  double *pipe_flx, *pipe_prf, *pipe_trc;
  double *riv_uflx, *riv_vflx, *riv_vol, *riv_trc;
  int* riv_face;
  int *uv2e_couple, *uv2e_flux;
  double *bzeta[4], *bubar[4], *bvbar[4], *bu[4], *bv[4], *bt[4];
  double* ub[4];
  double* colscr;
  double *dRdx, *dRde, *idRz, *diff3u, *diff3v, *Akz;
  double *iso_dTdz, *iso_FSC, *iso_dTdx, *iso_dTde, *iso_LapT;
};

enum S2dWinField : int {
  kW_zeta, kW_ubar, kW_vbar, kW_h, kW_dn_u, kW_dm_v, kW_pm, kW_pn, kW_swflx, kW_rmask, kW_rhoS, kW_rhoA, kW_umask,
  kW_vmask, kW_rufrc, kW_rvfrc, kW_DU_avg1, kW_DV_avg1, kW_DU_avg2, kW_DV_avg2, kW_Zt_avg1, kW_DU_avg_bak,
  kW_DV_avg_bak, kW_s0, kW_s1, kWinN
};
struct S2dWin {
  const double* base;
  int lead;
  unsigned off[kWinN];
};

struct Halo;
struct Dev {
  Bounds b;
  Params p;
  Fields f;
  const Halo* halo;
  S2dWin w2;
};

__host__ __device__ __forceinline__ long IJ(const Bounds& b, int i, int j) {
  return (long)(i + 1) + (long)(j + 1) * b.nx2;
}
__host__ __device__ __forceinline__ long IJK(const Bounds& b, int i, int j, int k) {
  return IJ(b, i, j) + (long)(k - 1) * b.n2;
}
__host__ __device__ __forceinline__ long IJW(const Bounds& b, int i, int j, int k) {
  return IJ(b, i, j) + (long)k * b.n2;
}
__host__ __device__ __forceinline__ long IJL(const Bounds& b, int i, int j, int l) {
  return IJ(b, i, j) + (long)(l - 1) * b.n2;
}
__host__ __device__ __forceinline__ long IJKL(const Bounds& b, int i, int j, int k, int l) {
  return IJ(b, i, j) + (long)(k - 1) * b.n2 + (long)(l - 1) * b.n3;
}
__host__ __device__ __forceinline__ long TIDX(const Bounds& b, int i, int j, int k, int l, int itrc) {
  return IJKL(b, i, j, k, l) + (long)(itrc - 1) * 3 * b.n3;
}

__device__ __forceinline__ double fmax0(double a) { return a > 0.0 ? a : 0.0; }
__device__ __forceinline__ double fmin0(double a) { return a < 0.0 ? a : 0.0; }
__device__ __forceinline__ double dmax(double a, double b) { return a > b ? a : b; }
__device__ __forceinline__ double dmin(double a, double b) { return a < b ? a : b; }
__device__ __forceinline__ int iclamp(int x, int lo, int hi) { return x < lo ? lo : (x > hi ? hi : x); }

constexpr int kVgRho = 1, kVgKppExt = 2, kVgKppInt = 4, kVgHuv = 8, kVgAll = 15;
constexpr int kVgDefault = kVgRho | kVgKppExt | kVgHuv;
struct VGrid {
  const double *Cs_w, *Cs_r;
  double z, h, hinv, hc, ds;
  int N;
  __device__ __forceinline__ double zw0() const { return -h; }
  __device__ __forceinline__ double zw1(int k, double csw) const {
    const double cff_w = hc * ds * (double)(k - N);
    return z + (z + h) * (cff_w + csw * h) * hinv;
  }
  __device__ __forceinline__ double zr(int k, double csr) const {
    const double cff_r = hc * ds * ((double)(k - N) - 0.5);
    return z + (z + h) * (cff_r + csr * h) * hinv;
  }
  __device__ __forceinline__ double zw(int k, double csw) const { return k == 0 ? zw0() : zw1(k, csw); }
  __device__ __forceinline__ double zw1(int k) const { return zw1(k, Cs_w[k]); }
  __device__ __forceinline__ double zr(int k) const { return zr(k, Cs_r[k]); }
};
__device__ __forceinline__ double vg_zw(const VGrid& g, int k) { return k == 0 ? g.zw0() : g.zw1(k); }
__device__ __forceinline__ double vg_zr(const VGrid& g, int k) { return g.zr(k); }
__device__ __forceinline__ double vg_hz(const VGrid& g, int k) { return g.zw1(k) - vg_zw(g, k - 1); }
__device__ __forceinline__ VGrid vg_make(const Dev& d, double z, double h, double hinv) {
  return VGrid{d.f.Cs_w, d.f.Cs_r, z, h, hinv, d.p.hc, 1.0 / (double)d.b.N, d.b.N};
}
__device__ __forceinline__ VGrid vg_column(const Dev& d, long ij) {
  return vg_make(d, d.f.z_sd[ij], d.f.h[ij], d.f.hinv[ij]);
}

__device__ __forceinline__ uint3 xcd_tile() {
  const unsigned gx = gridDim.x, gy = gridDim.y;
  const unsigned total = gx * gy * gridDim.z;
  const unsigned phys = blockIdx.x + gx * (blockIdx.y + gy * blockIdx.z);
  const unsigned q = total >> 3, r = total & 7u, x = phys & 7u, slot = phys >> 3;
  const unsigned logical = x * q + (x < r ? x : r) + slot;
  uint3 t;
  t.x = logical % gx;
  t.y = (logical / gx) % gy;
  t.z = logical / (gx * gy);
  return t;
}

#define ROMS_LEVEL_FENCE() __asm__ volatile("" ::: "memory")
#ifndef ROMS_FENCE_EVERY
#define ROMS_FENCE_EVERY 1000
#endif
#define ROMS_LEVEL_FENCE_AT(k) do { if ((k) % ROMS_FENCE_EVERY == 0) ROMS_LEVEL_FENCE(); } while (0)

struct Range {
  int i0, i1, j0, j1;
};
constexpr int kBX = 64, kBY = 4;
#ifndef ROMS_TILE_ALIGN
#define ROMS_TILE_ALIGN 1
#endif
__host__ __device__ __forceinline__ int tile_i0(int i0) { return ROMS_TILE_ALIGN ? i0 - ((i0 - 1) & (kRowAlign - 1)) : i0; }
inline dim3 grid_of(const Range& r) {
  int ni = r.i1 - tile_i0(r.i0) + 1, nj = r.j1 - r.j0 + 1;
  if (ni < 1) ni = 1;
  if (nj < 1) nj = 1;
  return dim3((ni + kBX - 1) / kBX, (nj + kBY - 1) / kBY, 1);
}
inline dim3 grid3_of(const Range& r, int nk) {
  dim3 g = grid_of(r);
  g.z = nk;
  return g;
}
constexpr int kCX = 64;
#ifndef ROMS_SEG_ROWS
#define ROMS_SEG_ROWS 13
#endif
#ifndef ROMS_SEG_MAXS
#define ROMS_SEG_MAXS 8
#endif
constexpr int kSegRows = ROMS_SEG_ROWS;
constexpr int kSegMaxS = ROMS_SEG_MAXS;
#ifndef ROMS_SEG_CW
#define ROMS_SEG_CW 16
#endif
constexpr int kSegCW = ROMS_SEG_CW;
constexpr int kSegBlock = ((kSegMaxS * kSegCW + 63) / 64) * 64;
#ifndef ROMS_SEG_JMAX
#define ROMS_SEG_JMAX 1
#endif
constexpr int kSegJMax = ROMS_SEG_JMAX;
#ifndef ROMS_SEG_NMIN
#define ROMS_SEG_NMIN 11
#endif
constexpr int kSegNMin = ROMS_SEG_NMIN;
#ifndef ROMS_SEG_BUF_WAVES
#define ROMS_SEG_BUF_WAVES 2
#endif
#ifndef ROMS_PRE_T_SEG_WAVES
#define ROMS_PRE_T_SEG_WAVES ROMS_SEG_BUF_WAVES
#endif
#ifndef ROMS_T_SEG_WAVES
#define ROMS_T_SEG_WAVES ROMS_SEG_BUF_WAVES
#endif
inline int seg_count(int N) {
  const int per = kCX / kSegCW, S = (N + kSegRows - 1) / kSegRows;
  return (S + per - 1) / per * per;
}
inline bool seg_rows_ok(int N) { return N / seg_count(N) >= kSegNMin; }
inline dim3 gridc_of(const Range& r) {
  int ni = r.i1 - tile_i0(r.i0) + 1, nj = r.j1 - r.j0 + 1;
  if (ni < 1) ni = 1;
  if (nj < 1) nj = 1;
  return dim3((ni + kCX - 1) / kCX, nj, 1);
}
#define ROMS_IJC_OR_RETURN(R)                                       \
  const uint3 bI = xcd_tile();                                      \
  const int i = tile_i0((R).i0) + (int)(bI.x * kCX + threadIdx.x);  \
  const int j = (R).j0 + (int)bI.y;                                 \
  if (i < (R).i0 || i > (R).i1 || j > (R).j1) return;
#define ROMS_IJ_OR_RETURN(R)                                        \
  const uint3 bI = xcd_tile();                                      \
  const int i = tile_i0((R).i0) + (int)(bI.x * kBX + threadIdx.x); \
  const int j = (R).j0 + (int)(bI.y * kBY + threadIdx.y);           \
  if (i < (R).i0 || i > (R).i1 || j > (R).j1) return;

struct Tlev {
  int iic, ntstart, forw_start, iif, nfast, kstp, knew, nstp, nrhs, nnew;
};

constexpr int kTimedS2dFb = 13;
constexpr int kTimedPreUvSeg = 14, kTimedUv1Seg = 15, kTimedStep3dTSeg = 16;
constexpr int kTimedPrsgrdUv = 17;
constexpr int kTimedHaloPack = 18, kTimedHaloWait = 19, kTimedHaloUnpack = 20;
void ktimer_mark(hipStream_t s, int kernel_id, int end, int count = 0);

inline bool buffer_span_ok(const Bounds& b) { return b.n3w * 8 < 2147483648L; }

void launch_exchange(const Dev& d, hipStream_t s, double* a, int nlev);
constexpr int kExchMax = 16;
struct ExchList {
  double* p[kExchMax];
  int nlev[kExchMax];
  int n;
  int w = 2;
};
void launch_exchange_list(const Dev& d, hipStream_t s, const ExchList& L);
bool rim_overlap_on(const Dev& d, const Range& R);
void rim_fork(const Dev& d, hipStream_t s, const ExchList& L);
void rim_join(const Dev& d, hipStream_t s);
template <class Run, class Edges>
void launch_rim_first(const Dev& d, hipStream_t s, const Range& R, const ExchList& L, Run&& run, Edges&& edges) {
  if (!rim_overlap_on(d, R)) {
    run(R);
    edges();
    launch_exchange_list(d, s, L);
    return;
  }
  run(Range{R.i0, R.i0 + 1, R.j0, R.j1});
  run(Range{R.i1 - 1, R.i1, R.j0, R.j1});
  run(Range{R.i0 + 2, R.i1 - 2, R.j0, R.j0 + 1});
// ... 61 lines not shown
```

### ucla-roms_amd/csrc/roms_shim.cpp

```cpp
#include <hip/hip_runtime.h>

#include <algorithm>
#include <cmath>
#include <cstdlib>
#include <cstdio>
#include <cstring>
#include <map>
#include <string>
#include <vector>

#include "../../include/roms_gpu.h"
#include "halo.h"
#include "host_init.h"
#include "roms_dev.h"
#include "shim_state.h"

using namespace roms;

namespace {

struct FieldDesc {
  double* d = nullptr;
  long count = 0;
  long hcount = 0;
  bool planar = false;
  double* host = nullptr;
  long host_count = 0;
};

struct Ctx {
  bool inited = false;
  Dev d{};
  hipStream_t s = nullptr;
  FieldDesc f[ROMS_NFIELDS];
  std::vector<double*> scratch;
  roms_dims dims{};
  roms_cfg cfg{};
  double w1[kMaxFast], w2[kMaxFast];
  double area = 0.0, volume = 0.0;
  bool have_volume = false;
  long riv_maxidx = 0;
  bool have_swr = false;
  long graph_frc_gen = 0;
  int rho_slot = 0;
  bool hzuv_env = false;
  bool hzuv_valid = true;
  bool rho_reuse = true;
  bool vgrid_valid = false;
  std::string err;
  std::map<long, hipGraphExec_t> graphs;
  bool use_graphs = true;
  double* h_diag = nullptr;
  double* d_diag = nullptr;
  Halo halo;
  int timed = -1;
  std::vector<hipEvent_t> ev;
  size_t nev = 0;
  long kcount = 0;
  bool guard = false;
  std::map<double*, double*> guard_base;
  double* arena = nullptr;
  long arena_n = 0, arena_used = 0;
  double* small = nullptr;
  long small_n = 0;
  long off = 0;
  Bounds hb{};
  double* stage = nullptr;
  long stage_n = 0;
  int par = 0;
  long step_exch = 0;
  hipStream_t s2 = nullptr;
  hipEvent_t pev[8] = {};
};
thread_local Ctx g;

double tree_sum(std::vector<double> v) {
  int size = (int)v.size();
  while (size > 1) {
    const int step = (size + 1) / 2;
    for (int r = 0; r < size - step; r++) v[r] = v[r] + v[r + step];
    size = step;
  }
  return v.empty() ? 0.0 : v[0];
}
void rank_extent(int LL, int np, int node, int& len, int& sw) {
  const int base = (LL + np - 1) / np, off = np * base - LL;
  sw = node == 0 ? 0 : node * base - off / 2;
  len = base;
  if (node == 0) len -= off / 2;
  if (node == np - 1) len -= (off + 1) / 2;
}
int min_rank_extent(int LL, int np) {
  int mn = LL, len, sw;
  for (int node : {0, np - 1}) {
    rank_extent(LL, np, node, len, sw);
    mn = len < mn ? len : mn;
  }
  if (np > 2) {
    rank_extent(LL, np, 1, len, sw);
    mn = len < mn ? len : mn;
  }
  return mn;
}

void drop_graphs() {
  for (auto& kv : g.graphs) (void)hipGraphExecDestroy(kv.second);
  g.graphs.clear();
}
void vg_set(bool valid) {
  g.vgrid_valid = valid;
  g.d.p.vg = valid ? g.d.p.vgrid : (short)0;
}
void vg_host_write(int id) {
  if (id != ROMS_Hz && id != ROMS_z_r && id != ROMS_z_w && id != ROMS_h && id != ROMS_hinv && id != ROMS_Cs_w &&
      id != ROMS_Cs_r)
    return;
  if (g.vgrid_valid && !g.graphs.empty()) {
    (void)hipStreamSynchronize(g.s);
    drop_graphs();
  }
  vg_set(false);
}

#define CHECK_HIP(x)                                                                  \
  do {                                                                                \
    hipError_t e_ = (x);                                                              \
    if (e_ != hipSuccess) {                                                           \
      g.err = std::string(#x) + ": " + hipGetErrorString(e_);                         \
      return -2;                                                                      \
    }                                                                                 \
  } while (0)

#define REQUIRE_INIT_NOJOIN()                           \
  do {                                                  \
    if (!g.inited) {                                    \
      g.err = "roms_gpu: not initialised";              \
      return -1;                                        \
    }                                                   \
  } while (0)
#define REQUIRE_HALO_OK()                                                                    \
  do {                                                                                       \
    if (g.d.halo && halo_failed(g.halo)) {                                                   \
      g.err = "roms_gpu: a halo exchange wait timed out (IPC transport, ROMS_GPU_IPC_TIMEOUT);" \
              " the state since is invalid";                                                 \
      return -6;                                                                             \
    }                                                                                        \
  } while (0)
#define REQUIRE_INIT()                                  \
  do {                                                  \
    REQUIRE_INIT_NOJOIN();                              \
    REQUIRE_HALO_OK();                                  \
    if (g.d.halo) halo_join(g.halo, g.s);               \
    g.rho_slot = 0;                                     \
  } while (0)
#define REQUIRE_INIT_RO()                               \
  const int rho_keep_ = g.rho_slot;                     \
  REQUIRE_INIT();                                       \
  g.rho_slot = rho_keep_

int post_launch() {
  hipError_t e = hipGetLastError();
  if (e != hipSuccess) {
    g.err = std::string("kernel launch: ") + hipGetErrorString(e);
    return -3;
  }
  return 0;
}

bool env_off(const char* name) {
  const char* e = getenv(name);
  return e && e[0] == '0';
}
bool env_on(const char* name) {
  const char* e = getenv(name);
  return e && e[0] == '1';
}
int env_int(const char* name, int def, int lo, int hi) {
  const char* e = getenv(name);
  if (!e || !((e[0] >= '0' && e[0] <= '9') || (e[0] == '-' && e[1] >= '0' && e[1] <= '9'))) return def;
  const int v = atoi(e);
  return v >= lo && v <= hi ? v : def;
}

Bounds make_bounds(const roms_dims& D, int pitch, int gx = 0) {
  Bounds b{};
  b.Lm = D.Lm; b.Mm = D.Mm; b.N = D.N; b.NT = D.NT;
  b.nTS = 1;
  b.nx2 = pitch;
  b.gx = gx;
  b.n2 = (long)pitch * (D.Mm + 4 + 2 * gx);
  b.n3 = b.n2 * D.N;
  b.n3w = b.n2 * (D.N + 1);
  b.istr = 1; b.iend = D.Lm; b.jstr = 1; b.jend = D.Mm;
  b.ew_periodic = D.ew_periodic; b.ns_periodic = D.ns_periodic;
  b.west_exch = D.west_exchng; b.east_exch = D.east_exchng;
  b.south_exch = D.south_exchng; b.north_exch = D.north_exchng;
  b.west_edge = !D.ew_periodic && !D.west_exchng;
  b.east_edge = !D.ew_periodic && !D.east_exchng;
  b.south_edge = !D.ns_periodic && !D.south_exchng;
  b.north_edge = !D.ns_periodic && !D.north_exchng;
  b.istrR = b.west_edge ? b.istr - 1 : b.istr;
  b.istrU = b.west_edge ? b.istr + 1 : b.istr;
  b.iendR = b.east_edge ? b.iend + 1 : b.iend;
  b.jstrR = b.south_edge ? b.jstr - 1 : b.jstr;
  b.jstrV = b.south_edge ? b.jstr + 1 : b.jstr;
  b.jendR = b.north_edge ? b.jend + 1 : b.jend;
  b.istrE = (D.ew_periodic || D.west_exchng) ? b.istr - 2 : b.istr - 1;
  b.iendE = (D.ew_periodic || D.east_exchng) ? b.iend + 2 : b.iend + 1;
  b.jstrE = (D.ns_periodic || D.south_exchng) ? b.jstr - 2 : b.jstr - 1;
  b.jendE = (D.ns_periodic || D.north_exchng) ? b.jend + 2 : b.jend + 1;
  return b;
}

bool planar_field(int id) { return !(id == ROMS_Cs_w || id == ROMS_Cs_r || (id >= ROMS_zeta_west && id <= ROMS_t_north)); }

long field_count(int id, const Bounds& b) {
  const long n2 = b.n2, n3 = b.n3, n3w = b.n3w;
  switch (id) {
    case ROMS_Cs_w: case ROMS_Cs_r: return b.N + 1;
    case ROMS_zeta: case ROMS_ubar: case ROMS_vbar: return 4 * n2;
    case ROMS_u: case ROMS_v: return 3 * n3;
    case ROMS_t: return 3 * n3 * b.NT;
    case ROMS_FlxU: case ROMS_FlxV: case ROMS_Hz: case ROMS_Hz_u: case ROMS_Hz_v: case ROMS_z_r: case ROMS_rho:
    case ROMS_rho1: case ROMS_qp1: case ROMS_ru: case ROMS_rv: return n3;
    case ROMS_We: case ROMS_Wi: case ROMS_z_w: case ROMS_bvf: case ROMS_Akv: case ROMS_ghat: case ROMS_swr_frac:
      return n3w;
    case ROMS_Akt: return n3w * b.nTS;
    case ROMS_diff2: case ROMS_stflx: return n2 * b.NT;
    default: break;
  }
  if (id >= ROMS_zeta_west && id <= ROMS_t_north) {
    const int side = (id - ROMS_zeta_west) % 4, var = (id - ROMS_zeta_west) / 4;
    const long nb = side < 2 ? b.Mm + 2 : b.Lm + 2;
    return var < 3 ? nb : var < 5 ? nb * b.N : nb * b.N * b.NT;
  }
  return n2;
}

double** field_slot(Fields& F, int id) {
  switch (id) {
    case ROMS_h: return &F.h; case ROMS_hinv: return &F.hinv; case ROMS_f: return &F.f; case ROMS_fomn: return &F.fomn;
    case ROMS_pm: return &F.pm; case ROMS_pn: return &F.pn; case ROMS_dm_r: return &F.dm_r; case ROMS_dn_r: return &F.dn_r;
    case ROMS_dm_u: return &F.dm_u; case ROMS_dn_u: return &F.dn_u; case ROMS_dm_v: return &F.dm_v;
    case ROMS_dn_v: return &F.dn_v; case ROMS_dm_p: return &F.dm_p; case ROMS_dn_p: return &F.dn_p;
    case ROMS_pmon_u: return &F.pmon_u; case ROMS_pnom_v: return &F.pnom_v; case ROMS_rmask: return &F.rmask;
    case ROMS_pmask: return &F.pmask; case ROMS_umask: return &F.umask; case ROMS_vmask: return &F.vmask;
    case ROMS_Cs_w: return &F.Cs_w; case ROMS_Cs_r: return &F.Cs_r;
    case ROMS_zeta: return &F.zeta; case ROMS_ubar: return &F.ubar; case ROMS_vbar: return &F.vbar;
    case ROMS_u: return &F.u; case ROMS_v: return &F.v; case ROMS_t: return &F.t; case ROMS_FlxU: return &F.FlxU;
    case ROMS_FlxV: return &F.FlxV; case ROMS_We: return &F.We; case ROMS_Wi: return &F.Wi; case ROMS_Hz: return &F.Hz;
    case ROMS_Hz_u: return &F.Hz_u; case ROMS_Hz_v: return &F.Hz_v; case ROMS_z_r: return &F.z_r; case ROMS_z_w: return &F.z_w;
    case ROMS_rufrc: return &F.rufrc; case ROMS_rvfrc: return &F.rvfrc; case ROMS_rhoA: return &F.rhoA;
    case ROMS_rhoS: return &F.rhoS; case ROMS_r_D: return &F.r_D; case ROMS_Zt_avg1: return &F.Zt_avg1;
    case ROMS_DU_avg1: return &F.DU_avg1; case ROMS_DV_avg1: return &F.DV_avg1; case ROMS_DU_avg2: return &F.DU_avg2;
    case ROMS_DV_avg2: return &F.DV_avg2; case ROMS_DU_avg_bak: return &F.DU_avg_bak;
    case ROMS_DV_avg_bak: return &F.DV_avg_bak; case ROMS_rho: return &F.rho; case ROMS_rho1: return &F.rho1;
    case ROMS_qp1: return &F.qp1; case ROMS_bvf: return &F.bvf; case ROMS_Akv: return &F.Akv; case ROMS_Akt: return &F.Akt;
    case ROMS_visc2_r: return &F.visc2_r; case ROMS_visc2_p: return &F.visc2_p; case ROMS_diff2: return &F.diff2;
    case ROMS_hbls: return &F.hbls; case ROMS_hbbl: return &F.hbbl; case ROMS_ghat: return &F.ghat;
    case ROMS_swr_frac: return &F.swr_frac; case ROMS_sustr: return &F.sustr; case ROMS_svstr: return &F.svstr;
    case ROMS_stflx: return &F.stflx; case ROMS_srflx: return &F.srflx; case ROMS_swflx: return &F.swflx;
    case ROMS_ru: return &F.ru; case ROMS_rv: return &F.rv;
    case ROMS_dndx: return &F.dndx; case ROMS_dmde: return &F.dmde; case ROMS_ptide: return &F.ptide;
    case ROMS_uwnd: return &F.uwnd; case ROMS_vwnd: return &F.vwnd; case ROMS_tair: return &F.tair;
// ... 339 lines not shown
        (void)hipFree(dev_base(p));
        g.guard_base.erase(p);
      } else {
        (void)hipFree(p);
      }
      p = nullptr;
    }
    if (cnt) { (void)hipFree(cnt); cnt = nullptr; }
  };
  auto fail = [&](hipError_t e, const char* what) -> int {
    g.err = std::string("roms_gpu_selftest_zero_fill: ") + what + ": " + hipGetErrorString(e);
    release();
    return -2;
  };
  hipError_t e;
  for (double*& p : a) {
    if ((e = hipMalloc(&p, (size_t)n * sizeof(double))) != hipSuccess) { p = nullptr; return fail(e, "hipMalloc"); }
    launch_fill_ones(p, n, g.s);
  }
  if ((e = hipStreamSynchronize(g.s)) != hipSuccess) return fail(e, "fill");
  for (double*& p : a) {
    (void)hipFree(p);
    p = nullptr;
  }
  if ((e = hipMalloc(&cnt, 2 * sizeof(unsigned long long))) != hipSuccess) { cnt = nullptr; return fail(e, "hipMalloc"); }
  if ((e = hipMemsetAsync(cnt, 0, 2 * sizeof(unsigned long long), g.s)) != hipSuccess) return fail(e, "memset");
  if ((e = hipStreamSynchronize(g.s)) != hipSuccess) return fail(e, "memset");
  guarded = true;
  for (double*& p : a) {
    if ((e = dev_alloc(p, n)) != hipSuccess) { p = nullptr; return fail(e, "dev_alloc"); }
    launch_count_nonzero(p, n, cnt, g.s, 0.0);
    launch_fill_ones(p, n, g.s);
  }
  if ((e = hipDeviceSynchronize()) != hipSuccess) return fail(e, "drain");
  for (double* p : a) launch_count_nonzero(p, n, cnt + 1, g.s, 1.0);
  unsigned long long h[2] = {0, 0};
  if ((e = hipMemcpyAsync(h, cnt, sizeof(h), hipMemcpyDeviceToHost, g.s)) != hipSuccess) return fail(e, "copy");
  if ((e = hipStreamSynchronize(g.s)) != hipSuccess) return fail(e, "copy");
  release();
  *bad = (long)(h[0] + h[1]);
  return 0;
}
const char* roms_gpu_last_error(void) { return g.err.c_str(); }
void* roms_gpu_stream(void) { return (void*)g.s; }

int roms_gpu_init(const roms_dims* dims, const roms_cfg* cfg, int device, void* comm) {
  if (g.inited) free_all();
  if (!dims || !cfg) { g.err = "roms_gpu_init: null argument"; return -1; }
  if (dims->N < 2 || dims->Lm < 2 || dims->Mm < 2 || dims->NT < 1) { g.err = "roms_gpu_init: bad dims"; return -1; }
  if (cfg->nfast < 1 || cfg->nfast > ROMS_MAX_FAST) { g.err = "roms_gpu_init: bad nfast"; return -1; }
  const int nranks = dims->np_xi * dims->np_eta;
  if (nranks < 1) { g.err = "roms_gpu_init: bad processor grid"; return -1; }
  if (nranks > 1 && comm == nullptr) { g.err = "roms_gpu_init: np_xi*np_eta > 1 needs a communicator"; return -1; }
  if (comm != nullptr) {
    RomsComm* c = (RomsComm*)comm;
    if (comm_size(c) != nranks || comm_rank(c) != dims->inode + dims->jnode * dims->np_xi) {
      g.err = "roms_gpu_init: communicator size/rank does not match np_xi*np_eta / inode+jnode*np_xi";
      return -1;
    }
  }
  g.dims = *dims;
  g.cfg = *cfg;
  g.have_volume = false;
  g.area = g.volume = 0.0;
  g.d = Dev{};
  (void)s2d_edge_modes_taken(true);
  {
    const bool pad = !env_off("ROMS_GPU_PITCH");
    const int hx = dims->Lm + 4;
    int k = env_int("ROMS_GPU_S2D_K", 4, 1, 8);
    const bool split = env_on("ROMS_GPU_S2D_SPLIT");
    const int obc = cfg->obc & ((dims->ew_periodic ? 0 : 3) | (dims->ns_periodic ? 0 : 12));
    if (comm == nullptr || split || obc) k = 1;
    const int mext = std::min(min_rank_extent(dims->LLm, dims->np_xi), min_rank_extent(dims->MMm, dims->np_eta));
    while (k > 1 && mext < 2 * k + 2) k--;
    const int gx = 2 * (k - 1);
    g.off = pad ? kAlignOff : 0;
    const int w = hx + 2 * gx;
    g.d.b = make_bounds(*dims, pad ? (w + kRowAlign - 1) / kRowAlign * kRowAlign : w, gx);
    g.hb = make_bounds(*dims, hx);
    g.d.p.s2d_k = k;
  }
  if (!buffer_span_ok(g.d.b)) {
    g.err = "roms_gpu_init: subdomain too large for one GPU rank: a w-point field (n2*(N+1)*8 B) reaches 2 GiB, "
            "the limit of the kernels' 32-bit buffer offsets (k_common.h BufF64); split the grid over more ranks";
    return -1;
  }
  CHECK_HIP(hipSetDevice(device));
  g.d.b.nTS = g.hb.nTS = cfg->salinity ? 2 : 1;
  Params& P = g.d.p;
  {
    const int m = cfg->lmd_mixing, base = ROMS_LMD_MIXING | ROMS_LMD_KPP | ROMS_LMD_BKPP;
    if (m != 0 && ((m & ~(ROMS_LMD_ALL | ROMS_LMD_DDMIX)) || (m & base) != base ||
                   ((m & ROMS_LMD_CONVEC) && !(m & ROMS_LMD_RIMIX)) || ((m & ROMS_LMD_DDMIX) && !cfg->salinity))) {
      g.err = "roms_gpu_init: lmd_mixing must be 0 or LMD_MIXING|LMD_KPP|LMD_BKPP [|RIMIX|NONLOCAL|CONVEC(needs RIMIX)"
              "|DDMIX(needs SALINITY)]";
      return -1;
    }
  }
  P.nonlin_eos = cfg->nonlin_eos; P.salinity = cfg->salinity; P.lmd = cfg->lmd_mixing != 0;
  P.lmd_rimix = (cfg->lmd_mixing & ROMS_LMD_RIMIX) != 0;
  P.lmd_convec = (cfg->lmd_mixing & ROMS_LMD_CONVEC) != 0;
  P.lmd_nonlocal = (cfg->lmd_mixing & ROMS_LMD_NONLOCAL) != 0;
  P.lmd_ddmix = (cfg->lmd_mixing & ROMS_LMD_DDMIX) != 0;
  P.uv_adv = cfg->uv_adv != 0; P.uv_cor = cfg->uv_cor != 0;
  P.tides = cfg->pot_tides != 0;
  P.bulk_frc = cfg->bulk_frc != 0;
  P.iso = cfg->adv_isoneutral != 0;
  P.prs_split = !env_on("ROMS_GPU_PRSGRD_FUSED");
  P.uv_vis2 = cfg->uv_vis2; P.ts_dif2 = cfg->ts_dif2;
  P.s2d_split = env_on("ROMS_GPU_S2D_SPLIT");
  P.dt = cfg->dt; P.dtfast = cfg->dt / (double)cfg->ndtfast; P.g = cfg->g; P.rho0 = cfg->rho0;
  P.vonKar = 0.41; P.qp2 = 0.0000172; P.gamma2 = cfg->gamma2; P.hc = cfg->hc;
  P.rdrg = cfg->rdrg; P.Zob = cfg->Zob; P.Tcoef = cfg->Tcoef; P.T0 = cfg->T0; P.Scoef = cfg->Scoef; P.S0 = cfg->S0;
  P.Akv_bak = cfg->Akv_bak; P.Akt_bak[0] = cfg->Akt_bak[0]; P.Akt_bak[1] = cfg->Akt_bak[1];
  P.npip = 0;
  if (cfg->obc < 0 || cfg->obc > 15) { g.err = "roms_gpu_init: obc must be a 4-bit edge mask"; return -1; }
  P.obc = cfg->obc & ((dims->ew_periodic ? 0 : 3) | (dims->ns_periodic ? 0 : 12));
  P.ubind = cfg->ubind;
  P.curvgrid = cfg->curvgrid && cfg->uv_adv;
  if (P.obc) P.s2d_split = 1;
  for (int i = 0; i < kMaxFast; i++) { g.w1[i] = cfg->weight[0][i]; g.w2[i] = cfg->weight[1][i]; }
  const bool seg_fits = dims->N <= kSegRows * kSegMaxS && seg_rows_ok(dims->N);
  P.colseg = (size_t)2 * (dims->N + 1) * kCX * sizeof(double) > 64 * 1024 && seg_fits;
  if (env_off("ROMS_GPU_COLSEG")) P.colseg = 0;
  if (env_on("ROMS_GPU_COLSEG")) P.colseg = seg_fits;
  P.colreg = env_int("ROMS_GPU_COLREG", 2, 0, 3);
  P.uv2_fused = !env_off("ROMS_GPU_UV2_FUSED");
  P.chain = !env_off("ROMS_GPU_CHAIN");
  P.seg_order = env_int("ROMS_GPU_SEG_ORDER", 3, 0, 3);
  P.seg_xg = env_int("ROMS_GPU_SEG_XG", 8, 1, 1 << 30);
  P.s2d_fold = !env_on("ROMS_GPU_S2D_EDGES");
  P.chain_dirz = !env_off("ROMS_GPU_CHAIN_DIRZ");
  P.prs_fuse_uv = !env_off("ROMS_GPU_PRS_UV");
  P.uv1_lds = !env_off("ROMS_GPU_UV1_LDS");
  P.p_in_rho = !env_off("ROMS_GPU_P_IN_RHO");
  P.omega_hb = !env_off("ROMS_GPU_OMEGA_HB");
  P.omega_seg = !env_off("ROMS_GPU_OMEGA_SEG");
  {
    const int v = env_int("ROMS_GPU_OMEGA_CW", dims->N > 63 ? 16 : 64, 0, 1 << 30);
    P.omega_cw = v == 32 || v == 64 ? v : 16;
  }
  P.preuv_lds = !env_off("ROMS_GPU_PREUV_LDS");
  P.h_jc = env_int("ROMS_GPU_HJC", 0, 0, 1 << 30) / 4 * 4;
  P.visc_stg = !env_off("ROMS_GPU_VISC_STG");
  P.t3dmix_stg = !env_off("ROMS_GPU_T3DMIX_STG");
  {
    const int v = env_int("ROMS_GPU_KPP_TY", 4, 0, 43);
    P.kpp_ty = v == 0 || v == 2 || v == 8 || v == 43 ? v : 4;
  }
  P.kpp_lean = (short)env_int("ROMS_GPU_KPP_LEAN", 7, 0, 7);
  P.kpp_fckeep = (short)env_int("ROMS_GPU_KPP_FCKEEP", kKppFcKeepMax, 1, kKppFcKeepMax);
  P.vgrid = (short)env_int("ROMS_GPU_VGRID", kVgDefault, 0, kVgAll);
  P.vg = 0;
  g.vgrid_valid = false;
  P.hoist = !env_off("ROMS_GPU_HOIST");
  P.prs_buf = !env_off("ROMS_GPU_PRS_BUF");
  P.prs_strip = !env_off("ROMS_GPU_PRS_STRIP");
  P.t_strip = env_on("ROMS_GPU_T_STRIP");
  P.seg_buf = !env_off("ROMS_GPU_SEG_BUF");
  P.seg_jrows = env_int("ROMS_GPU_SEG_JROWS", kSegJMax < 2 ? kSegJMax : 2, 1, kSegJMax);
  bool col_global = (size_t)2 * (dims->N + 1) * kCX * sizeof(double) > 64 * 1024;
  if (env_on("ROMS_GPU_COL_GLOBAL")) col_global = true;
  if (env_off("ROMS_GPU_COL_GLOBAL")) col_global = false;
  setup_uv1_seg();
  setup_pre_uv_seg();
  setup_omega_seg();
  if (!col_global && !setup_column_kernels(dims->N)) {
    g.err = "roms_gpu_init: N too large for the LDS column kernels (2*(N+1)*512 B > 160 KB)";
    return -2;
  }
  CHECK_HIP(hipStreamCreateWithFlags(&g.s, hipStreamNonBlocking));
  CHECK_HIP(hipStreamCreateWithFlags(&g.s2, hipStreamNonBlocking));
  for (hipEvent_t& e : g.pev) CHECK_HIP(hipEventCreateWithFlags(&e, hipEventDisableTiming));
  {
    const char* em = getenv("ROMS_GPU_PAR_MASK");
    g.par = env_on("ROMS_GPU_PAR") ? 31 : 0;
    if (em) g.par = atoi(em) & 31;
  }
  g.guard = env_on("ROMS_GPU_GUARD");
  const Bounds& b = g.d.b;
  auto field = [&](int id) -> int {
    const long n = field_count(id, b);
    double* p = nullptr;
    CHECK_HIP(dev_alloc(p, n));
    g.f[id].d = p;
    g.f[id].count = n;
    g.f[id].hcount = field_count(id, g.hb);
    g.f[id].planar = planar_field(id);
    *field_slot(g.d.f, id) = p;
    return 0;
  };
  auto planar2d = [&](int id) { return planar_field(id) && field_count(id, b) <= 4 * b.n2; };
  {
    long n = 11 * dev_alloc_size(b.n2);
    for (int id = 0; id < ROMS_NFIELDS; id++)
      if (planar2d(id)) n += dev_alloc_size(field_count(id, b));
    if (n * 8 < 2147483648L - (1L << 20)) {
      CHECK_HIP(hipMalloc(&g.arena, (size_t)n * sizeof(double)));
      g.arena_n = n;
      g.arena_used = 0;
    }
  }
  for (int id = 0; id < ROMS_NFIELDS; id++)
    if (planar2d(id) && field(id)) return -2;
  auto scratch = [&](double*& p, long n) -> int {
    CHECK_HIP(dev_alloc(p, n));
    g.scratch.push_back(p);
    return 0;
  };
  Fields& F = g.d.f;
  double** s2[] = {&F.s0, &F.s1, &F.s2, &F.s3, &F.s4, &F.s5, &F.s6, &F.s7, &F.s8, &F.s9};
  for (double** q : s2)
    if (scratch(*q, b.n2)) return -2;
  if (scratch(F.z_sd, b.n2)) return -2;
  g.arena_n = g.arena_used;
  for (int id = 0; id < ROMS_NFIELDS; id++)
    if (!planar2d(id) && field(id)) return -2;
  if (scratch(F.P, b.n3) || scratch(F.rhos, b.n3) || scratch(F.c0, b.n3w) || scratch(F.c1, b.n3w) ||
      scratch(F.c2, b.n3w) || scratch(F.c3, b.n3w))
    return -2;
  {
    g.d.w2 = S2dWin{};
    const double* wp[kWinN] = {F.zeta,  F.ubar,  F.vbar,    F.h,       F.dn_u,    F.dm_v,       F.pm,
                               F.pn,    F.swflx, F.rmask,   F.rhoS,    F.rhoA,    F.umask,      F.vmask,
                               F.rufrc, F.rvfrc, F.DU_avg1, F.DV_avg1, F.DU_avg2, F.DV_avg2,    F.Zt_avg1,
                               F.DU_avg_bak, F.DV_avg_bak, F.s0, F.s1};
    const long lead = (long)b.gx * b.nx2 + b.gx + kRowAlign;
    uintptr_t lo = UINTPTR_MAX, hi = 0;
    for (int f = 0; f < kWinN; f++) {
      const long cnt = f <= kW_vbar ? 4 * b.n2 : b.n2;
      lo = std::min(lo, (uintptr_t)wp[f] - (uintptr_t)lead * 8u);
      hi = std::max(hi, (uintptr_t)wp[f] + (uintptr_t)cnt * 8u);
    }
    if (!env_off("ROMS_GPU_S2D_WIN") && hi - lo < (uintptr_t)2147483648u - (1u << 20)) {
      g.d.w2.base = (const double*)lo;
      g.d.w2.lead = (int)lead;
      for (int f = 0; f < kWinN; f++) g.d.w2.off[f] = (unsigned)((uintptr_t)wp[f] - (uintptr_t)lead * 8u - lo);
    }
  }
  if (col_global && scratch(F.colscr, 2L * (b.NT > 2 ? b.NT : 2) * b.n3w)) return -2;
  if (P.iso) {
    double** r3[] = {&F.dRdx, &F.dRde, &F.diff3u, &F.diff3v, &F.iso_dTdx, &F.iso_dTde, &F.iso_LapT};
    for (double** q : r3)
      if (scratch(*q, b.n3)) return -2;
    double** w3[] = {&F.idRz, &F.Akz, &F.iso_dTdz, &F.iso_FSC};
    for (double** q : w3)
      if (scratch(*q, b.n3w)) return -2;
  }
  if (P.lmd) {
    if (scratch(F.lmd_rig, b.n3w)) return -2;
    double** l2[] = {&F.lmd_hbl, &F.lmd_bbl, &F.lmd_Bo, &F.lmd_Bosol, &F.lmd_ustar};
    for (double** q : l2)
      if (scratch(*q, b.n2)) return -2;
  }
  {
    std::vector<int> lc, lf;
    if (!env_off("ROMS_GPU_UV2_EDGE")) uv2_edge_lists(b, lc, lf);
    if (!lc.empty() && !lf.empty()) {
      CHECK_HIP(hipMalloc(&F.uv2e_couple, lc.size() * sizeof(int)));
      CHECK_HIP(hipMalloc(&F.uv2e_flux, lf.size() * sizeof(int)));
      CHECK_HIP(copy_on(F.uv2e_couple, lc.data(), lc.size() * sizeof(int), hipMemcpyHostToDevice, g.s));
      CHECK_HIP(copy_on(F.uv2e_flux, lf.data(), lf.size() * sizeof(int), hipMemcpyHostToDevice, g.s));
      P.uv2e_nc = (int)(lc.size() / 3);
      P.uv2e_nf = (int)(lf.size() / 3);
    }
  }
  CHECK_HIP(hipHostMalloc(&g.h_diag, 8 * sizeof(double), hipHostMallocDefault));
  CHECK_HIP(hipMalloc(&g.d_diag, 8 * sizeof(double)));
  if (comm != nullptr) {
    HaloPlan plan = halo_plan(dims->Lm, dims->Mm, dims->np_xi, dims->np_eta, dims->inode, dims->jnode,
                              dims->ew_periodic, dims->ns_periodic);
    plan.g.nx2 = b.nx2;
    plan.g.n2 = b.n2;
    HaloPlan wide{};
    if (P.s2d_k > 1) {
      wide = halo_plan(dims->Lm, dims->Mm, dims->np_xi, dims->np_eta, dims->inode, dims->jnode, dims->ew_periodic,
                       dims->ns_periodic, 2 * P.s2d_k);
      wide.g.nx2 = b.nx2;
      wide.g.n2 = b.n2;
    }
    const int r = halo_setup(g.halo, (RomsComm*)comm, plan, 8 * (dims->N + 1), wide, kExchMax, g.err);
    if (r) return r;
    g.halo.ls = g.s;
    g.d.halo = &g.halo;
  }
  g.hzuv_env = env_on("ROMS_GPU_HZ_UV");
  g.hzuv_valid = true;
  g.use_graphs = !env_on("ROMS_GPU_NO_GRAPH") && halo_graph_safe(g.d.halo);
  g.rho_reuse = !env_off("ROMS_GPU_RHO_REUSE");
  g.rho_slot = 0;
  g.inited = true;
  return 0;
}

int roms_gpu_finalize(void) {
  if (g.inited) {
    (void)hipStreamSynchronize(g.s);
    free_all();
  }
  return 0;
}

long roms_gpu_field_size(int id) {
  if (!g.inited || id < 0 || id >= ROMS_NFIELDS) return -1;
  return g.f[id].hcount;
}

int roms_gpu_register(int id, double* host, long count) {
  REQUIRE_INIT();
  if (id < 0 || id >= ROMS_NFIELDS) { g.err = "roms_gpu_register: bad field id"; return -1; }
  if (count != g.f[id].hcount) { g.err = "roms_gpu_register: size mismatch for field"; return -1; }
  g.f[id].host = host;
  g.f[id].host_count = count;
  return 0;
}

static bool hzuv_readable(int id) {
  if ((id != ROMS_Hz_u && id != ROMS_Hz_v) || g.hzuv_valid) return true;
  g.err = "Hz_u/Hz_v are not maintained by whole steps unless registered for transfer or ROMS_GPU_HZ_UV=1 "
          "(extract_data inputs, set_depth.F:220,227)";
  return false;
}
static int xfer(int id, bool up) {
  if (id == ROMS_ALL) {
    for (int q = 0; q < ROMS_NFIELDS; q++)
      if (g.f[q].host) {
        const int r = xfer(q, up);
        if (r) return r;
      }
    return 0;
  }
  if (id < 0 || id >= ROMS_NFIELDS) { g.err = "bad field id"; return -1; }
  if (!g.f[id].host) { g.err = "field not registered"; return -1; }
  if (!up && !hzuv_readable(id)) return -5;
  if (up && (id == ROMS_Hz_u || id == ROMS_Hz_v)) g.hzuv_valid = true;
  if (up) vg_host_write(id);
  CHECK_HIP(up ? field_h2d(id, g.f[id].d, g.f[id].host) : field_d2h(id, g.f[id].host, g.f[id].d));
  return 0;
}
int roms_gpu_upload(int id) { REQUIRE_INIT(); return xfer(id, true); }
int roms_gpu_download(int id) { REQUIRE_INIT_RO(); return xfer(id, false); }

int roms_gpu_copy_in(int id, const double* src, long count) {
  REQUIRE_INIT();
  if (id < 0 || id >= ROMS_NFIELDS || count != g.f[id].hcount) { g.err = "roms_gpu_copy_in: bad field/size"; return -1; }
  if (id == ROMS_Hz_u || id == ROMS_Hz_v) g.hzuv_valid = true;
  vg_host_write(id);
  CHECK_HIP(field_h2d(id, g.f[id].d, src));
  return 0;
}
int roms_gpu_copy_out(int id, double* dst, long count) {
  REQUIRE_INIT_RO();
  if (id < 0 || id >= ROMS_NFIELDS || count != g.f[id].hcount) { g.err = "roms_gpu_copy_out: bad field/size"; return -1; }
  if (!hzuv_readable(id)) return -5;
  CHECK_HIP(field_d2h(id, dst, g.f[id].d));
  REQUIRE_HALO_OK();
  return 0;
}
int roms_gpu_sync(void) {
  REQUIRE_INIT_RO();
  CHECK_HIP(hipStreamSynchronize(g.s));
  REQUIRE_HALO_OK();
  return post_launch();
}

#define ROUTINE(name, call)           \
  int name(const roms_tlev* t) {      \
    REQUIRE_INIT();                   \
    const Tlev T = to_tlev(t);        \
    call;                             \
    return post_launch();             \
  }
ROUTINE(roms_gpu_set_huv, (launch_set_huv(g.d, g.s, T), g.hzuv_valid = true))
ROUTINE(roms_gpu_omega, launch_omega(g.d, g.s, T))
ROUTINE(roms_gpu_prsgrd, launch_prsgrd(g.d, g.s, T))
ROUTINE(roms_gpu_pre_step3d, launch_pre_step3d(g.d, g.s, T))
ROUTINE(roms_gpu_set_huv1, launch_set_huv1(g.d, g.s, T))
ROUTINE(roms_gpu_step3d_uv1, launch_step3d_uv1(g.d, g.s, T))
ROUTINE(roms_gpu_visc3d, launch_visc3d(g.d, g.s, T))
ROUTINE(roms_gpu_step3d_uv2, launch_step3d_uv2(g.d, g.s, T))
ROUTINE(roms_gpu_step3d_t, launch_step3d_t(g.d, g.s, T))
ROUTINE(roms_gpu_t3dmix, launch_t3dmix(g.d, g.s, T))
ROUTINE(roms_gpu_set_depth, (launch_set_depth(g.d, g.s, T), vg_set(true)))
#undef ROUTINE

int roms_gpu_halo_transport(void) {
  REQUIRE_INIT_NOJOIN();
  return g.d.halo ? halo_transport(g.halo) : 0;
}

int roms_gpu_halo_overlap(void) {
  REQUIRE_INIT_NOJOIN();
  return g.d.halo && g.halo.xoverlap > 0 ? 1 : 0;
}

int roms_gpu_s2d_window(void) {
  REQUIRE_INIT_NOJOIN();
  return g.d.w2.base ? 1 : 0;
}

int roms_gpu_column_path(void) {
  REQUIRE_INIT_NOJOIN();
  return (g.d.p.colseg ? ROMS_COLPATH_SEG : 0) | (g.d.f.colscr ? ROMS_COLPATH_GLOBAL : 0);
}

int roms_gpu_vgrid(void) {
  REQUIRE_INIT_NOJOIN();
  return g.d.p.vgrid + (g.vgrid_valid ? 256 : 0);
}

int roms_gpu_vgrid_check(long out[3]) {
  REQUIRE_INIT_RO();
  if (!out) { g.err = "roms_gpu_vgrid_check: null argument"; return -1; }
  unsigned long long* cnt = (unsigned long long*)shim_scratch_small(3);
  if (!cnt) { g.err = "roms_gpu_vgrid_check: out of device memory"; return -2; }
  CHECK_HIP(hipMemsetAsync(cnt, 0, 3 * sizeof(unsigned long long), g.s));
  launch_vgrid_check(g.d, g.s, cnt);
  unsigned long long h[3] = {0, 0, 0};
  CHECK_HIP(copy_on(h, cnt, sizeof(h), hipMemcpyDeviceToHost, g.s));
  for (int q = 0; q < 3; q++) out[q] = (long)h[q];
  return post_launch();
}

int roms_gpu_kpp_lean(void) {
  REQUIRE_INIT_NOJOIN();
  return g.d.p.kpp_lean + 256 * g.d.p.kpp_fckeep;
}

int roms_gpu_horizontal_path(int out[8]) {
  REQUIRE_INIT_NOJOIN();
  if (!out) { g.err = "roms_gpu_horizontal_path: null argument"; return -1; }
  const Dev& d = g.d;
  int jA = 0, jB = -1, nstrip = 0;
  const bool strips = prsgrd_takes_strips(d, prsgrd_can_fuse_uv(d), jA, jB, nstrip);
  out[0] = s2d_edge_mode(d);
  out[1] = strips ? 1 : 0;
  out[2] = strips ? nstrip : 0;
  out[3] = strips ? jA : 0;
  out[4] = strips ? jB : -1;
  out[5] = omega_takes_seg(d, d.b.iend - d.b.istr + 1) ? 1 : 0;
  out[6] = s2d_edge_modes_taken();
  out[7] = 0;
  return 0;
}

int roms_gpu_halo_exchanges(long* per_step, int* fast_interval) {
  REQUIRE_INIT_NOJOIN();
  if (per_step) *per_step = g.step_exch;
  if (fast_interval) *fast_interval = g.d.p.s2d_k;
  return 0;
}

int roms_gpu_step2d(const roms_tlev* t) {
  REQUIRE_INIT_NOJOIN();
  REQUIRE_HALO_OK();
  const Tlev T = to_tlev(t);
  launch_step2d(g.d, g.s, T, g.w1, g.w2);
  if (T.iif == T.nfast) vg_set(true);
  return post_launch();
}

int roms_gpu_rho_eos(int tidx, const roms_tlev* t) {
  REQUIRE_INIT();
  launch_rho_eos(g.d, g.s, to_tlev(t), tidx);
  return post_launch();
}
int roms_gpu_lmd_vmix(int tind, const roms_tlev* t) {
  REQUIRE_INIT();
  if (!g.cfg.lmd_mixing) { g.err = "roms_gpu_lmd_vmix: library initialised without lmd_mixing"; return -4; }
  if (tind < 1 || tind > 3) { g.err = "roms_gpu_lmd_vmix: bad time index"; return -1; }
  launch_lmd_vmix(g.d, g.s, to_tlev(t), tind);
  return post_launch();
}
int roms_gpu_swr_frac(const roms_tlev* t) {
  (void)t;
  REQUIRE_INIT();
  launch_swr_frac(g.d, g.s);
  g.have_swr = true;
  return post_launch();
}
int roms_gpu_set_pipe_frc(int npip, const int* pipe_idx, const double* pipe_flx, const double* pipe_prf,
                          const double* pipe_trc) {
  REQUIRE_INIT();
  const Bounds& b = g.d.b;
  Fields& F = g.d.f;
  if (npip < 0 || (npip > 0 && (!pipe_idx || !pipe_flx || !pipe_prf || !pipe_trc))) {
    g.err = "roms_gpu_set_pipe_frc: bad argument";
    return -1;
  }
  if (npip == 0) { g.d.p.npip = 0; return 0; }
  for (long q = 0; q < g.hb.n2; q++)
    if (pipe_idx[q] < 0 || pipe_idx[q] > npip) { g.err = "roms_gpu_set_pipe_frc: pipe_idx out of 0..npip"; return -1; }
  CHECK_HIP(hipStreamSynchronize(g.s));
  if (npip != g.d.p.npip || !F.pipe_idx) {
    for (auto& kv : g.graphs) (void)hipGraphExecDestroy(kv.second);
    g.graphs.clear();
    if (F.pipe_idx) (void)hipFree(F.pipe_idx);
    F.pipe_idx = nullptr;
    for (double** q : {&F.pipe_flx, &F.pipe_prf, &F.pipe_trc}) {
      if (!*q) continue;
      for (size_t k = 0; k < g.scratch.size(); k++)
        if (g.scratch[k] == *q) { g.scratch.erase(g.scratch.begin() + (long)k); break; }
      (void)hipFree(dev_base(*q));
      *q = nullptr;
    }
    g.d.p.npip = 0;
    CHECK_HIP(hipMalloc(&F.pipe_idx, (size_t)b.n2 * sizeof(int)));
    auto scratch = [&](double*& p, long n) -> int {
      CHECK_HIP(hipMalloc(&p, (size_t)n * sizeof(double)));
      g.scratch.push_back(p);
      return 0;
    };
    if (scratch(F.pipe_flx, b.n2) || scratch(F.pipe_prf, (long)npip * b.N) || scratch(F.pipe_trc, (long)npip * b.NT))
      return -2;
    g.d.p.npip = npip;
  }
  {
    const std::vector<int> di = to_dev_layout(pipe_idx, 1);
    const std::vector<double> df = to_dev_layout(pipe_flx, 1);
    CHECK_HIP(copy_on(F.pipe_idx, di.data(), (size_t)b.n2 * sizeof(int), hipMemcpyHostToDevice, g.s));
    CHECK_HIP(copy_on(F.pipe_flx, df.data(), (size_t)b.n2 * sizeof(double), hipMemcpyHostToDevice, g.s));
  }
  CHECK_HIP(copy_on(F.pipe_prf, pipe_prf, (size_t)npip * b.N * sizeof(double), hipMemcpyHostToDevice, g.s));
  CHECK_HIP(copy_on(F.pipe_trc, pipe_trc, (size_t)npip * b.NT * sizeof(double), hipMemcpyHostToDevice, g.s));
  return 0;
}

int roms_gpu_set_river_frc(int nriv, const double* riv_uflx, const double* riv_vflx, const double* riv_vol,
                           const double* riv_trc) {
  REQUIRE_INIT();
  const Bounds& b = g.d.b;
  Fields& F = g.d.f;
  if (nriv < 0 || nriv > 4096 || (nriv > 0 && (!riv_vol || !riv_trc)) || (!riv_uflx) != (!riv_vflx)) {
    g.err = "roms_gpu_set_river_frc: bad argument";
    return -1;
  }
  CHECK_HIP(hipStreamSynchronize(g.s));
  if (nriv == 0) {
    if (g.d.p.nriv) drop_graphs();
    g.d.p.nriv = 0;
    return 0;
  }
  if (!riv_uflx && !F.riv_uflx) { g.err = "roms_gpu_set_river_frc: river faces never set"; return -1; }
  if (!riv_uflx && nriv < g.riv_maxidx) {
    g.err = "roms_gpu_set_river_frc: nriv smaller than the largest river index of the faces on the device "
            "(pass riv_uflx/riv_vflx again)";
    return -1;
  }
  std::vector<int> faces;
  long maxidx = 0;
  if (riv_uflx) {
    for (int dir = 0; dir < 2; dir++) {
      const double* a = dir == 0 ? riv_uflx : riv_vflx;
      for (int j = -1; j <= b.Mm + 2; j++)
        for (int i = -1; i <= b.Lm + 2; i++) {
          const double v = a[IJ(g.hb, i, j)];
          if (!(std::fabs(v) > 1e-3)) continue;
          const long ir = std::lround(v / 10);
          if (ir < 1 || ir > nriv) { g.err = "roms_gpu_set_river_frc: river index nint(riv_flx/10) out of 1..nriv"; return -1; }
          faces.push_back(dir); faces.push_back(i); faces.push_back(j);
          if (ir > maxidx) maxidx = ir;
// ... 447 lines not shown
```

### ucla-roms_amd/romsgpu/__init__.py

```python
import ctypes
import os

import numpy as np

_HERE = os.path.dirname(os.path.abspath(__file__))
_PKG = os.path.dirname(_HERE)
LIB_PATH = os.environ.get("ROMS_GPU_LIB") or os.path.join(_PKG, "libromsgpu.so")
MAX_FAST = 288

FIELDS = ["h", "hinv", "f", "fomn", "pm", "pn", "dm_r", "dn_r", "dm_u", "dn_u", "dm_v", "dn_v", "dm_p", "dn_p",
          "pmon_u", "pnom_v", "rmask", "pmask", "umask", "vmask", "Cs_w", "Cs_r",
          "zeta", "ubar", "vbar", "u", "v", "t", "FlxU", "FlxV", "We", "Wi", "Hz", "Hz_u", "Hz_v", "z_r", "z_w",
          "rufrc", "rvfrc", "rhoA", "rhoS", "r_D", "Zt_avg1", "DU_avg1", "DV_avg1", "DU_avg2", "DV_avg2",
          "DU_avg_bak", "DV_avg_bak", "rho", "rho1", "qp1", "bvf", "Akv", "Akt", "visc2_r", "visc2_p", "diff2",
          "hbls", "hbbl", "ghat", "swr_frac", "sustr", "svstr", "stflx", "srflx", "swflx", "ru", "rv"] + \
         ["%s_%s" % (v, e) for v in ("zeta", "ubar", "vbar", "u", "v", "t") for e in ("west", "east", "south", "north")] + \
         ["dndx", "dmde", "ptide", "uwnd", "vwnd", "tair", "qair", "prate", "swrad", "lwrad", "sustr_r", "svstr_r"]
FIELD_ID = {n: i for i, n in enumerate(FIELDS)}
CASE_FILAMENT, CASE_BASIN, CASE_PIPES, CASE_RIVERS = 0, 1, 2, 3
LMD_MIXING, LMD_KPP, LMD_BKPP, LMD_RIMIX, LMD_CONVEC, LMD_NONLOCAL = 1, 2, 4, 8, 16, 32
LMD_DDMIX = 64
LMD_ALL = 63
LMD_ICELAND = 47

# ... 311 lines not shown
    def get(self, name):
        fid = FIELD_ID[name]
        n = self.L.roms_gpu_field_size(fid)
        a = np.empty(n, dtype=np.float64)
        self._chk(self.L.roms_gpu_copy_out(fid, a.ctypes.data, n), "copy_out " + name)
        n2 = self.shape2[0] * self.shape2[1]
        return a.reshape((n // n2,) + self.shape2) if n % n2 == 0 else a

    def put(self, name, arr):
        fid = FIELD_ID[name]
        a = np.ascontiguousarray(arr, dtype=np.float64).ravel()
        n = self.L.roms_gpu_field_size(fid)
        if a.size != n:
            raise ValueError("%s: expected %d elements, got %d" % (name, n, a.size))
        self._chk(self.L.roms_gpu_copy_in(fid, a.ctypes.data, n), "copy_in " + name)

    def set_tindex(self, iic, kstp, knew, nstp, nrhs, nnew, iif=1, forw_start=1, ntstart=1, nfast=None):
        self.t.iic, self.t.kstp, self.t.knew, self.t.nstp, self.t.nrhs, self.t.nnew = iic, kstp, knew, nstp, nrhs, nnew
        self.t.iif, self.t.forw_start, self.t.ntstart = iif, forw_start, ntstart
        if nfast is not None:
            self.t.nfast = nfast

    def sync(self):
        self._chk(self.L.roms_gpu_sync(), "sync")

    def rho_eos(self, tidx):
        self._chk(self.L.roms_gpu_rho_eos(tidx, ctypes.byref(self.t)), "rho_eos")

    def lmd_vmix(self, tind):
        self._chk(self.L.roms_gpu_lmd_vmix(tind, ctypes.byref(self.t)), "lmd_vmix")

    def set_pipe_frc(self, pipe_idx, pipe_flx, pipe_prf, pipe_trc):
        prf = np.asarray(pipe_prf, dtype=np.float64)
        npip = prf.shape[0]
        idx = np.ascontiguousarray(pipe_idx, dtype=np.int32).ravel()
        flx = np.ascontiguousarray(pipe_flx, dtype=np.float64).ravel()
        prf = np.asfortranarray(prf).ravel(order="F")
        trc = np.asarray(pipe_trc, dtype=np.float64).ravel(order="F")
        P = ctypes.POINTER
        self._chk(self.L.roms_gpu_set_pipe_frc(npip, idx.ctypes.data_as(P(ctypes.c_int)), flx.ctypes.data_as(P(ctypes.c_double)),
                                               prf.ctypes.data_as(P(ctypes.c_double)), trc.ctypes.data_as(P(ctypes.c_double))),
                  "set_pipe_frc")

    def set_river_frc(self, riv_vol, riv_trc, riv_uflx=None, riv_vflx=None):
        vol = np.ascontiguousarray(riv_vol, dtype=np.float64).ravel()
        nriv = vol.shape[0]
        trc = np.asfortranarray(np.asarray(riv_trc, dtype=np.float64).reshape(nriv, -1)).ravel(order="F")
        P = ctypes.POINTER
        D = P(ctypes.c_double)
        if riv_uflx is None:
            uf = vf = None
        else:
            uf = np.ascontiguousarray(riv_uflx, dtype=np.float64).ravel()
            vf = np.ascontiguousarray(riv_vflx, dtype=np.float64).ravel()
        self._chk(self.L.roms_gpu_set_river_frc(nriv, uf.ctypes.data_as(D) if uf is not None else None,
                                                vf.ctypes.data_as(D) if vf is not None else None,
                                                vol.ctypes.data_as(D), trc.ctypes.data_as(D)), "set_river_frc")

    def set_ub_tune(self, ub):
        D = ctypes.POINTER(ctypes.c_double)
        keep = [None if a is None else np.ascontiguousarray(a, dtype=np.float64) for a in ub]
        self._chk(self.L.roms_gpu_set_ub_tune(*[None if a is None else a.ctypes.data_as(D) for a in keep]),
                  "set_ub_tune")

    FRC_SURFACE, FRC_BRY = 1, 2

    def frc_record(self, name, slot, rec_time, arr):
        a = np.ascontiguousarray(arr, dtype=np.float64).ravel()
        if a.size != self.L.roms_gpu_field_size(FIELD_ID[name]):
            raise ValueError("frc_record: %s has %d elements" % (name, a.size))
        self._chk(self.L.roms_gpu_frc_record(FIELD_ID[name], slot, rec_time,
                                             a.ctypes.data_as(ctypes.POINTER(ctypes.c_double))), "frc_record")

    def frc_interp(self, modtime, kinds=3):
        self._chk(self.L.roms_gpu_frc_interp(modtime, kinds), "frc_interp")

    def frc_clock(self, start_time, on=True):
        self._chk(self.L.roms_gpu_frc_clock(start_time, int(on)), "frc_clock")

    def set_tide_data(self, ftide, pot=None, bry=None):
        D = ctypes.POINTER(ctypes.c_double)
        keep = [np.ascontiguousarray(ftide, dtype=np.float64)]
        def ptr(a):
            if a is None:
                return None
            keep.append(np.ascontiguousarray(a, dtype=np.float64))
            return keep[-1].ctypes.data_as(D)
        pr, pi = pot if pot is not None else (None, None)
        (zr, zi), (ur, ui), (vr, vi) = bry if bry is not None else ((None, None),) * 3
        self._chk(self.L.roms_gpu_set_tide_data(len(keep[0]), keep[0].ctypes.data_as(D), ptr(pr), ptr(pi), ptr(zr),
                                                ptr(zi), ptr(ur), ptr(ui), ptr(vr), ptr(vi)), "set_tide_data")

    def set_tides(self, time):
        self._chk(self.L.roms_gpu_set_tides(time), "set_tides")

    def bulk_flux(self):
        self._chk(self.L.roms_gpu_bulk_flux(ctypes.byref(self.t)), "bulk_flux")

    def _r(self, fn):
        self._chk(getattr(self.L, "roms_gpu_" + fn)(ctypes.byref(self.t)), fn)

    def set_HUV(self): self._r("set_huv")
    def omega(self): self._r("omega")
    def prsgrd(self): self._r("prsgrd")
    def pre_step3d(self): self._r("pre_step3d")
    def set_HUV1(self): self._r("set_huv1")
    def step3d_uv1(self): self._r("step3d_uv1")
    def visc3d(self): self._r("visc3d")
    def step2d(self): self._r("step2d")
    def step3d_uv2(self): self._r("step3d_uv2")
    def step3d_t(self): self._r("step3d_t")
    def t3dmix(self): self._r("t3dmix")
    def set_depth(self): self._r("set_depth")
    def swr_frac(self): self._r("swr_frac")
    def init_sequence(self): self._r("init_sequence")

    def step(self, n=1):
        for _ in range(n):
            self._r("step")

    def time_routine(self, routine, nsteps):
        ms = ctypes.c_double()
        n = ctypes.c_long()
        self._chk(self.L.roms_gpu_time_routine(ROUTINES.index(routine), nsteps, ctypes.byref(self.t), ctypes.byref(ms),
                                               ctypes.byref(n)), "time_routine")
        return ms.value, n.value

    def selftest_zero_fill(self, n, chunks=1):
        nz = ctypes.c_long()
        self._chk(self.L.roms_gpu_selftest_zero_fill(ctypes.c_long(n), ctypes.c_int(chunks), ctypes.byref(nz)),
                  "selftest_zero_fill")
        return nz.value

    def halo_transport(self):
        r = self.L.roms_gpu_halo_transport()
        return {1: "ipc", 0: "rccl", -1: "ipc-timeout"}.get(r, "error")

    def halo_overlap(self):
        return bool(self.L.roms_gpu_halo_overlap())

    def s2d_window(self):
        return bool(self.L.roms_gpu_s2d_window())

    def kpp_lean(self):
        r = self.L.roms_gpu_kpp_lean()
        self._chk(min(r, 0), "kpp_lean")
        return r % 256, r // 256

    def vgrid(self):
        r = self.L.roms_gpu_vgrid()
        self._chk(min(r, 0), "vgrid")
        return r % 256, bool(r // 256)

    def vgrid_mismatch(self):
        out = (ctypes.c_long * 3)()
        self._chk(self.L.roms_gpu_vgrid_check(out), "vgrid_check")
        return out[0], out[1], out[2]

    def column_path(self):
        r = self.L.roms_gpu_column_path()
        self._chk(min(r, 0), "column_path")
        return bool(r & 1), bool(r & 2)

    def horizontal_path(self):
        out = (ctypes.c_int * 8)()
        self._chk(self.L.roms_gpu_horizontal_path(out), "horizontal_path")
        return {"edges": out[0], "strips": (out[2], out[3], out[4]) if out[1] else None, "omega_seg": bool(out[5])}

    def fast_step_edge_modes(self):
        out = (ctypes.c_int * 8)()
        self._chk(self.L.roms_gpu_horizontal_path(out), "horizontal_path")
        return {m for m in range(3) if out[6] >> m & 1}

    def halo_exchanges(self):
        n, k = ctypes.c_long(), ctypes.c_int()
        self._chk(self.L.roms_gpu_halo_exchanges(ctypes.byref(n), ctypes.byref(k)), "halo_exchanges")
        return n.value, k.value

    def diag(self):
        out = (ctypes.c_double * 4)()
        self._chk(self.L.roms_gpu_diag(ctypes.byref(self.t), out), "diag")
        return list(out)

    def time(self, dt):
        return dt * (self.t.iic - self.t.ntstart + 1) + getattr(self, "start_time", 0.0)

    def wrt_rst(self, path, rec, total_rec, time):
        self._chk(self.L.roms_gpu_wrt_rst(path.encode(), rec, total_rec, time, ctypes.byref(self.t)), "wrt_rst")

    def wrt_his(self, path, rec, total_rec, time, mask=WRT_DEFAULT):
        self._chk(self.L.roms_gpu_wrt_his(path.encode(), rec, total_rec, time, ctypes.byref(self.t), mask), "wrt_his")

    def io_wait(self):
        self._chk(self.L.roms_gpu_io_wait(), "io_wait")

    def get_init(self, path, req_rec, tindx):
        st = ctypes.c_double()
        rc = self.L.roms_gpu_get_init(path.encode(), req_rec, tindx, ctypes.byref(self.t), ctypes.byref(st))
        if rc < 0:
            self._chk(rc, "get_init")
        if tindx == 1:
            self.start_time = st.value
        return rc

    def restart(self, path, rec=0, exact=True):
        self.t.forw_start = 0
        if exact:
            nrec = rec if rec > 0 else self._nrecs(path)
            if nrec >= 2:
                self.get_init(path, nrec - 1, 2)
            rec = nrec
        self.get_init(path, rec, 1)
        self.init_sequence()

    @staticmethod
    def _nrecs(path):
        with open(path, "rb") as f:
            h = f.read(8)
        return int.from_bytes(h[4:8], "big")

    def time_steps(self, n):
        ms = ctypes.c_double()
        self._chk(self.L.roms_gpu_time_steps(ctypes.byref(self.t), n, ctypes.byref(ms)), "time_steps")
        return ms.value
```

Before: 2.318 billion cell-updates/s.

## Recompute Hz and z_w on the fly in omega, huv1, uv2, visc3d, t3dmix

Extends the analytic vertical-grid path to five more kernels. Layer thickness Hz and interface depth z_w are rebuilt from z, h, hinv and Cs_w instead of being loaded from 3D arrays. Each variant is a template selected by a new bit mask (ROMS_GPU_VGRID2, all bits on by default) that is packed into the existing vg flags. The aim is to cut the global-memory traffic for Hz and z_w in these bandwidth-bound kernels. In exchange it adds floating-point work, extra registers and LDS, and a risk of rounding differences from the stored arrays.

```diff
diff --git a/include/roms_gpu.h b/include/roms_gpu.h
--- a/include/roms_gpu.h
+++ b/include/roms_gpu.h
@@ -5,7 +5,7 @@
 extern "C" {
 #endif
 
-#define ROMS_GPU_ABI_VERSION 20
+#define ROMS_GPU_ABI_VERSION 21
 #define ROMS_MAX_FAST 288
 
 typedef struct roms_dims {
@@ -150,6 +150,7 @@
 int roms_gpu_column_path(void);
 int roms_gpu_kpp_lean(void);
 int roms_gpu_vgrid(void);
+int roms_gpu_vgrid2(void);
 int roms_gpu_vgrid_check(long out[3]);
 int roms_gpu_horizontal_path(int out[8]);
 int roms_gpu_selftest_zero_fill(long n, int chunks, long *bad);
diff --git a/ucla-roms_amd/csrc/k_chain.h b/ucla-roms_amd/csrc/k_chain.h
--- a/ucla-roms_amd/csrc/k_chain.h
+++ b/ucla-roms_amd/csrc/k_chain.h
@@ -5,6 +5,7 @@
 
 constexpr int kChainCW = 16;
 constexpr int kChainG = 4;
+constexpr int kChainVgGroup = 8;
 
 struct ChainLane {
   int col, g;
diff --git a/ucla-roms_amd/csrc/k_step3d_t.hip b/ucla-roms_amd/csrc/k_step3d_t.hip
--- a/ucla-roms_amd/csrc/k_step3d_t.hip
+++ b/ucla-roms_amd/csrc/k_step3d_t.hip
@@ -611,6 +611,8 @@
 }
 
 constexpr int kTMW = kBX + 2, kTMN = kTMW * (kBY + 2), kTMQ = (3 * kTMN + kBX * kBY - 1) / (kBX * kBY);
+constexpr int kTMG = (kTMN + kBX * kBY - 1) / (kBX * kBY);
+template <bool VG>
 __global__ void __launch_bounds__(256) k_t3dmix_stg(Dev d, Range R, int nnew, int nrhs) {
   const uint3 bI = xcd_tile();
   __shared__ double sW[3 * kTMN];
@@ -648,11 +650,38 @@
     wf[m] = ok ? f : -1;
     wo[m] = ok ? IJ(b, ii, jj) : 0;
   }
+  double gz[kTMG], gh[kTMG], gi[kTMG], gw[kTMG];
+  double csw = 0.0;
+  if constexpr (VG) {
+#pragma unroll
+    for (int m = 0; m < kTMG; m++) {
+      const bool hzm = wf[m] == 0;
+      gz[m] = hzm ? F.z_sd[wo[m]] : 0.0;
+      gh[m] = hzm ? F.h[wo[m]] : 0.0;
+      gi[m] = hzm ? F.hinv[wo[m]] : 0.0;
+      gw[m] = -gh[m];
+    }
+    csw = F.Cs_w[1];
+  }
   auto ldw = [&](int k, double (&x)[kTMQ]) {
     const long kk = (long)(k - 1) * n2;
-#pragma unroll
-    for (int m = 0; m < kTMQ; m++)
-      x[m] = wf[m] == 0 ? F.Hz[wo[m] + kk] : wf[m] == 1 ? Tr[0][wo[m] + kk] : wf[m] == 2 ? Tr[1][wo[m] + kk] : 0.0;
+    const double cs = csw;
+    if constexpr (VG) csw = F.Cs_w[min(k + 1, b.N)];
+    if constexpr (VG) {
+#pragma unroll
+      for (int m = 0; m < kTMQ; m++) x[m] = wf[m] == 1 ? Tr[0][wo[m] + kk] : wf[m] == 2 ? Tr[1][wo[m] + kk] : 0.0;
+      __builtin_amdgcn_sched_barrier(0);
+#pragma unroll
+      for (int m = 0; m < kTMG; m++) {
+        const double z = vg_make(d, gz[m], gh[m], gi[m]).zw1(k, cs);
+        x[m] = wf[m] == 0 ? z - gw[m] : x[m];
+        gw[m] = z;
+      }
+    } else {
+#pragma unroll
+      for (int m = 0; m < kTMQ; m++)
+        x[m] = wf[m] == 0 ? F.Hz[wo[m] + kk] : wf[m] == 1 ? Tr[0][wo[m] + kk] : wf[m] == 2 ? Tr[1][wo[m] + kk] : 0.0;
+    }
   };
   const int c = (threadIdx.x + 1) + (threadIdx.y + 1) * kTMW;
   double w[kTMQ];
@@ -687,7 +716,9 @@
   Range R{b.istr, b.iend, b.jstr, b.jend};
   const bool stg = d.p.t3dmix_stg && b.NT == 2;
   auto run = [&](const Range& r) {
-    if (stg) hipLaunchKernelGGL(k_t3dmix_stg, grid_of(r), dim3(kBX, kBY), 0, s, d, r, t.nnew, t.nrhs);
+    if (stg && (d.p.vg & (kVg2T3dmix << kVg2Shift)))
+      hipLaunchKernelGGL(k_t3dmix_stg<true>, grid_of(r), dim3(kBX, kBY), 0, s, d, r, t.nnew, t.nrhs);
+    else if (stg) hipLaunchKernelGGL(k_t3dmix_stg<false>, grid_of(r), dim3(kBX, kBY), 0, s, d, r, t.nnew, t.nrhs);
     else hipLaunchKernelGGL(k_t3dmix, grid_of(r), dim3(kBX, kBY), 0, s, d, r, t.nnew, t.nrhs);
   };
   ExchList L;
diff --git a/ucla-roms_amd/csrc/k_step3d_uv.hip b/ucla-roms_amd/csrc/k_step3d_uv.hip
--- a/ucla-roms_amd/csrc/k_step3d_uv.hip
+++ b/ucla-roms_amd/csrc/k_step3d_uv.hip
@@ -551,10 +551,14 @@
 constexpr int kVVW = kBX + 2, kVVN = kVVW * (kBY + 3);
 constexpr int kVHW = kBX + 2, kVHN = kVHW * (kBY + 2);
 constexpr int kVSN = kVUN + kVVN + kVHN, kVSQ = (kVSN + kBX * kBY - 1) / (kBX * kBY);
+constexpr int kVG0 = (kVUN + kVVN) / (kBX * kBY);
+constexpr int kVGS = kVHN + 1;
+template <bool VG>
 __global__ void __launch_bounds__(256, 3) k_visc3d_stg(Dev d, Range R, int nstp) {
   const uint3 bI = xcd_tile();
   __shared__ double sUFx[kVN], sVFe[kVN], sUFe[kVN], sVFx[kVN];
   __shared__ double sRaw[kVSN];
+  __shared__ double sG[VG ? 4 * kVGS : 1];
   const Bounds& b = d.b;
   const Fields& F = d.f;
   const int indx = 3 - nstp;
@@ -609,11 +613,49 @@
     wf[m] = f;
     wo[m] = f >= 0 ? IJ(b, ii, jj) : 0;
   }
+  double csw = 0.0;
+  if constexpr (VG) {
+#pragma unroll
+    for (int m = kVG0; m < kVSQ; m++) {
+      const int hq = tid + m * kBX * kBY - (kVUN + kVVN);
+      if (hq >= 0 && hq < kVHN) {
+        const bool on = wf[m] == 2;
+        const double h = on ? F.h[wo[m]] : 0.0;
+        sG[hq] = on ? F.z_sd[wo[m]] : 0.0;
+        sG[kVGS + hq] = h;
+        sG[2 * kVGS + hq] = on ? F.hinv[wo[m]] : 0.0;
+        sG[3 * kVGS + hq] = -h;
+      }
+    }
+    if (tid == 0) sG[kVHN] = sG[kVGS + kVHN] = sG[2 * kVGS + kVHN] = sG[3 * kVGS + kVHN] = 0.0;
+    csw = F.Cs_w[1];
+  }
   auto ldraw = [&](int k, double (&x)[kVSQ]) {
     const long kk = (long)(k - 1) * b.n2;
-#pragma unroll
-    for (int m = 0; m < kVSQ; m++)
-      x[m] = wf[m] == 0 ? U[wo[m] + kk] : wf[m] == 1 ? V[wo[m] + kk] : wf[m] == 2 ? F.Hz[wo[m] + kk] : 0.0;
+    const double cs = csw;
+    if constexpr (VG) csw = F.Cs_w[min(k + 1, b.N)];
+    double hzv[kVSQ - kVG0 > 0 ? kVSQ - kVG0 : 1];
+    if constexpr (VG) {
+#pragma unroll
+      for (int m = kVG0; m < kVSQ; m++) {
+        const int hq = tid + m * kBX * kBY - (kVUN + kVVN);
+        const int hs = hq >= 0 && hq < kVHN ? hq : kVHN;
+        const double z = vg_make(d, sG[hs], sG[kVGS + hs], sG[2 * kVGS + hs]).zw1(k, cs);
+        hzv[m - kVG0] = z - sG[3 * kVGS + hs];
+        sG[3 * kVGS + hs] = z;
+      }
+      __builtin_amdgcn_sched_barrier(0);
+    }
+#pragma unroll
+    for (int m = 0; m < kVSQ; m++) {
+      if (VG && m >= kVG0) {
+        const double hz = hzv[m - kVG0];
+        if (m * kBX * kBY < kVUN + kVVN) x[m] = wf[m] == 1 ? V[wo[m] + kk] : wf[m] == 2 ? hz : 0.0;
+        else x[m] = wf[m] == 2 ? hz : 0.0;
+      } else {
+        x[m] = wf[m] == 0 ? U[wo[m] + kk] : wf[m] == 1 ? V[wo[m] + kk] : !VG && wf[m] == 2 ? F.Hz[wo[m] + kk] : 0.0;
+      }
+    }
   };
   auto Uw = [&](int ii, int jj) { return sRaw[(ii - (i0 - 1)) + (jj - (j0 - 1)) * kVUW]; };
   auto Vw = [&](int ii, int jj) { return sRaw[kVUN + (ii - (i0 - 1)) + (jj - (j0 - 1)) * kVVW]; };
@@ -693,8 +735,10 @@
 void launch_visc3d(const Dev& d, hipStream_t s, const Tlev& t) {
   const Bounds& b = d.b;
   Range R{b.istr, b.iend, b.jstr, b.jend};
-  if (d.p.visc_stg)
-    hipLaunchKernelGGL(k_visc3d_stg, grid_of(R), dim3(kBX, kBY), 0, s, d, R, t.nstp);
+  if (d.p.visc_stg && (d.p.vg & (kVg2Visc << kVg2Shift)))
+    hipLaunchKernelGGL(k_visc3d_stg<true>, grid_of(R), dim3(kBX, kBY), 0, s, d, R, t.nstp);
+  else if (d.p.visc_stg)
+    hipLaunchKernelGGL(k_visc3d_stg<false>, grid_of(R), dim3(kBX, kBY), 0, s, d, R, t.nstp);
   else
     hipLaunchKernelGGL(k_visc3d, grid_of(R), dim3(kBX, kBY), 0, s, d, R, t.nstp);
 }
@@ -816,7 +860,7 @@
   }
 }
 
-template <int KL, bool FULL = false>
+template <int KL, bool FULL = false, bool VG = false>
 __global__ void __launch_bounds__(256, KL > 13 ? 3 : 4) k_uv2_fused(Dev d, Range R, int nnew, int nstp, int knew) {
   constexpr bool kHcLds = KL > 13;
   __shared__ double sHc[kHcLds ? KL * 256 : 1];
@@ -854,11 +898,30 @@
       double* r;
       __device__ __forceinline__ double& operator[](int q) const { return kHcLds ? l[q * 256] : r[q]; }
     } const hc{sHc + threadIdx.x, hcr};
-#pragma unroll
-    for (int q = 0; q < KL; q++) {
-      un[q] = bUn.ld(vq(q), so(q));
-      hc[q] = 0.5 * (bHz.ld(vq(q), so(q)) + bHz.ld(vqm(q), so(q)));
-      if (q % 8 == 7) __builtin_amdgcn_sched_barrier(0);
+    if constexpr (VG) {
+      const VGrid g0 = vg_column(d, ij), gm = vg_column(d, ij - s);
+      int lv = lo;
+      __asm__ volatile("" : "+v"(lv));
+      const int kb = min(lv, N) - 1;
+      const double csb = F.Cs_w[kb];
+      double w0 = g0.zw(kb, csb), wm = gm.zw(kb, csb);
+#pragma unroll
+      for (int q = 0; q < KL; q++) {
+        const int k = min(lv + q, N);
+        const double cs = F.Cs_w[k];
+        un[q] = bUn.ld(vq(q), so(q));
+        const double z0 = g0.zw1(k, cs), zm = gm.zw1(k, cs);
+        hc[q] = 0.5 * ((z0 - w0) + (zm - wm));
+        w0 = z0; wm = zm;
+        if (q % kChainVgGroup == kChainVgGroup - 1) __builtin_amdgcn_sched_barrier(0);
+      }
+    } else {
+#pragma unroll
+      for (int q = 0; q < KL; q++) {
+        un[q] = bUn.ld(vq(q), so(q));
+        hc[q] = 0.5 * (bHz.ld(vq(q), so(q)) + bHz.ld(vqm(q), so(q)));
+        if (q % 8 == 7) __builtin_amdgcn_sched_barrier(0);
+      }
     }
     double CF0, DC0;
     chain2(CF0, DC0, [&](double& a, double& c) {
@@ -1028,10 +1091,15 @@
   if (!d.p.obc && d.p.uv2_fused && kl <= 25) {
     dim3 gf = chain_grid_of(R1);
     gf.z = d.p.chain_dirz ? 2 : 1;
-    if (kl <= 5) hipLaunchKernelGGL(k_uv2_fused<5>, gf, dim3(256), 0, s, d, R1, t.nnew, t.nstp, t.knew);
-    else if (kl <= 13) hipLaunchKernelGGL(k_uv2_fused<13>, gf, dim3(256), 0, s, d, R1, t.nnew, t.nstp, t.knew);
-    else if (b.N == 100) hipLaunchKernelGGL((k_uv2_fused<25, true>), gf, dim3(256), 0, s, d, R1, t.nnew, t.nstp, t.knew);
-    else hipLaunchKernelGGL(k_uv2_fused<25>, gf, dim3(256), 0, s, d, R1, t.nnew, t.nstp, t.knew);
+    const bool vg = (d.p.vg & (kVg2Uv2 << kVg2Shift)) != 0;
+    auto fused = [&](auto kern, auto kern_vg) {
+      if (vg) hipLaunchKernelGGL(kern_vg, gf, dim3(256), 0, s, d, R1, t.nnew, t.nstp, t.knew);
+      else hipLaunchKernelGGL(kern, gf, dim3(256), 0, s, d, R1, t.nnew, t.nstp, t.knew);
+    };
+    if (kl <= 5) fused(k_uv2_fused<5>, k_uv2_fused<5, false, true>);
+    else if (kl <= 13) fused(k_uv2_fused<13>, k_uv2_fused<13, false, true>);
+    else if (b.N == 100) fused(k_uv2_fused<25, true>, k_uv2_fused<25, true, true>);
+    else fused(k_uv2_fused<25>, k_uv2_fused<25, false, true>);
     if (d.f.uv2e_couple && d.p.uv2e_nc > 0 && d.p.uv2e_nf > 0) {
       const int nc = d.p.uv2e_nc, nf = d.p.uv2e_nf;
       const dim3 gc((nc + 63) / 64), gf2((nf + 63) / 64);
diff --git a/ucla-roms_amd/csrc/k_vertical.hip b/ucla-roms_amd/csrc/k_vertical.hip
--- a/ucla-roms_amd/csrc/k_vertical.hip
+++ b/ucla-roms_amd/csrc/k_vertical.hip
@@ -197,7 +197,7 @@
   }
 }
 
-template <int KL, bool FULL = false>
+template <int KL, bool FULL = false, bool VG = false>
 __global__ void __launch_bounds__(256, KL > 13 ? 3 : 4) k_set_huv1_chain(Dev d, Range R, int nnew, int first) {
   constexpr bool kDcLds = KL > 13;
   __shared__ double sDc[kDcLds ? KL * 256 : 1];
@@ -230,11 +230,30 @@
       double* r;
       __device__ __forceinline__ double& operator[](int q) const { return kDcLds ? l[q * 256] : r[q]; }
     } const dc{sDc + threadIdx.x, dcr};
-#pragma unroll
-    for (int q = 0; q < KL; q++) {
-      uu[q] = bU.ld(vq(q), so(q));
-      dc[q] = 0.5 * (bHz.ld(vq(q), so(q)) + bHz.ld(vqm(q), so(q))) * dn;
-      if (q % 8 == 7) __builtin_amdgcn_sched_barrier(0);
+    if constexpr (VG) {
+      const VGrid g0 = vg_column(d, ij), gm = vg_column(d, ij - s);
+      int lo = cl.lo;
+      __asm__ volatile("" : "+v"(lo));
+      const int kb = min(lo, N) - 1;
+      const double csb = F.Cs_w[kb];
+      double w0 = g0.zw(kb, csb), wm = gm.zw(kb, csb);
+#pragma unroll
+      for (int q = 0; q < KL; q++) {
+        const int k = min(lo + q, N);
+        const double cs = F.Cs_w[k];
+        uu[q] = bU.ld(vq(q), so(q));
+        const double z0 = g0.zw1(k, cs), zm = gm.zw1(k, cs);
+        dc[q] = 0.5 * ((z0 - w0) + (zm - wm)) * dn;
+        w0 = z0; wm = zm;
+        if (q % kChainVgGroup == kChainVgGroup - 1) __builtin_amdgcn_sched_barrier(0);
+      }
+    } else {
+#pragma unroll
+      for (int q = 0; q < KL; q++) {
+        uu[q] = bU.ld(vq(q), so(q));
+        dc[q] = 0.5 * (bHz.ld(vq(q), so(q)) + bHz.ld(vqm(q), so(q))) * dn;
+        if (q % 8 == 7) __builtin_amdgcn_sched_barrier(0);
+      }
     }
     double DC0, FC0;
     chain_down(cl, DC0, FC0, [&](double& a, double& c) {
@@ -267,11 +286,15 @@
   const int kl = chain_kl(b.N), first = (int)(t.iic == t.forw_start);
   dim3 gc = chain_grid_of(R);
   gc.z = d.p.chain_dirz ? 2 : 1;
-  if (d.p.chain && kl == 5) hipLaunchKernelGGL(k_set_huv1_chain<5>, gc, dim3(256), 0, s, d, R, t.nnew, first);
-  else if (d.p.chain && kl == 13) hipLaunchKernelGGL(k_set_huv1_chain<13>, gc, dim3(256), 0, s, d, R, t.nnew, first);
-  else if (d.p.chain && kl == 25 && b.N == 100)
-    hipLaunchKernelGGL((k_set_huv1_chain<25, true>), gc, dim3(256), 0, s, d, R, t.nnew, first);
-  else if (d.p.chain && kl == 25) hipLaunchKernelGGL(k_set_huv1_chain<25>, gc, dim3(256), 0, s, d, R, t.nnew, first);
+  const bool vg = (d.p.vg & (kVg2Huv1 << kVg2Shift)) != 0;
+  auto chain = [&](auto kern, auto kern_vg) {
+    if (vg) hipLaunchKernelGGL(kern_vg, gc, dim3(256), 0, s, d, R, t.nnew, first);
+    else hipLaunchKernelGGL(kern, gc, dim3(256), 0, s, d, R, t.nnew, first);
+  };
+  if (d.p.chain && kl == 5) chain(k_set_huv1_chain<5>, k_set_huv1_chain<5, false, true>);
+  else if (d.p.chain && kl == 13) chain(k_set_huv1_chain<13>, k_set_huv1_chain<13, false, true>);
+  else if (d.p.chain && kl == 25 && b.N == 100) chain(k_set_huv1_chain<25, true>, k_set_huv1_chain<25, true, true>);
+  else if (d.p.chain && kl == 25) chain(k_set_huv1_chain<25>, k_set_huv1_chain<25, false, true>);
   else hipLaunchKernelGGL(k_set_huv1, grid_of(R), dim3(kBX, kBY), 0, s, d, R, t.nnew, first);
   launch_exchange_list(d, s, ExchList{{d.f.FlxU, d.f.FlxV, d.f.u + (long)(t.nnew - 1) * b.n3,
                                         d.f.v + (long)(t.nnew - 1) * b.n3}, {b.N, b.N, b.N, b.N}, 4});
@@ -409,7 +432,7 @@
 
 constexpr int kOmR = kSegRows;
 constexpr int kOmCW = kCX, kOmBlock = kSegMaxS * kOmCW;
-template <bool kHB, int CW = kOmCW>
+template <bool kHB, int CW = kOmCW, bool VG = false>
 __global__ void __launch_bounds__(kSegMaxS * CW, 2) k_omega_seg(Dev d, Range R, double dtau, double hcff) {
   const uint3 bI = xcd_tile();
   const Bounds& b = d.b;
@@ -435,15 +458,37 @@
   __shared__ double Lw[kSegMaxS][CW], Lcx[kSegMaxS][CW], Lhz[kSegMaxS][CW];
   __shared__ double Lte[kHB ? kSegMaxS : 1][CW], Lti[kHB ? kSegMaxS : 1][CW];
   double fu1[kOmR], fu0[kOmR], fv1[kOmR], fv0[kOmR], cx[kOmR], hz[kOmR], zk[kOmR];
+  const int kb = min(c0, N) - 1;
+  const double csb = VG ? F.Cs_w[kb] : 0.0, csN = VG ? F.Cs_w[N] : 0.0;
 #pragma unroll
   for (int q = 0; q < kOmR; q++) {
     const int k = min(c0 + q, N);
     const unsigned o = (unsigned)(k - 1) * lv;
     fu1[q] = LD(FU, vo + 8u, o); fu0[q] = LD(FU, vo, o); fv1[q] = LD(FV, vo + (unsigned)sj * 8u, o); fv0[q] = LD(FV, vo, o);
-    hz[q] = LD(Hz, vo, o);
-    zk[q] = LD(zw, vo, (unsigned)k * lv);
-  }
-  const double zw0 = zw.ld(vo, 0), zwN = zw.ld(vo, (unsigned)N * lv);
+    if constexpr (VG) {
+      zk[q] = F.Cs_w[k];
+    } else {
+      hz[q] = LD(Hz, vo, o);
+      zk[q] = LD(zw, vo, (unsigned)k * lv);
+    }
+  }
+  double zw0, zwN;
+  if constexpr (VG) {
+    const VGrid g = vg_column(d, ij);
+    zw0 = g.zw0();
+    zwN = g.zw1(N, csN);
+    double zb = g.zw(kb, csb);
+#pragma unroll
+    for (int q = 0; q < kOmR; q++) {
+      const double z = g.zw1(min(c0 + q, N), zk[q]);
+      hz[q] = q == 0 || c0 + q <= N ? z - zb : hz[q > 0 ? q - 1 : 0];
+      zk[q] = z;
+      zb = z;
+    }
+  } else {
+    zw0 = zw.ld(vo, 0);
+    zwN = zw.ld(vo, (unsigned)N * lv);
+  }
   const double wsrf = F.swflx[ij] * F.dm_r[ij] * F.dn_r[ij];
   const double CX0 = dtau * F.pm[ij] * F.pn[ij];
   const int pidx = d.p.npip > 0 ? F.pipe_idx[ij] : 0;
@@ -575,6 +620,8 @@
 void setup_omega_seg() {
   (void)hipFuncSetAttribute((const void*)k_omega_seg<true>, hipFuncAttributeMaxDynamicSharedMemorySize,
                             (int)omega_hb_lds_bytes(kOmBlock));
+  (void)hipFuncSetAttribute((const void*)k_omega_seg<true, kOmCW, true>, hipFuncAttributeMaxDynamicSharedMemorySize,
+                            (int)omega_hb_lds_bytes(kOmBlock));
 }
 
 template <bool kHB, int CW>
@@ -582,7 +629,8 @@
   const Bounds& b = d.b;
   const dim3 gs((r.i1 - tile_i0(r.i0) + CW) / CW, r.j1 - r.j0 + 1), bs(kCX, seg_waves<CW>(b.N));
   const size_t lds = kHB ? omega_hb_lds_bytes(bs.x * bs.y) : 0;
-  hipLaunchKernelGGL((k_omega_seg<kHB, CW>), gs, bs, lds, s, d, r, dtau, hcff);
+  if (d.p.vg & (kVg2Omega << kVg2Shift)) hipLaunchKernelGGL((k_omega_seg<kHB, CW, true>), gs, bs, lds, s, d, r, dtau, hcff);
+  else hipLaunchKernelGGL((k_omega_seg<kHB, CW, false>), gs, bs, lds, s, d, r, dtau, hcff);
 }
 template <bool kHB>
 static void omega_seg(const Dev& d, hipStream_t s, const Range& r, double dtau, double hcff) {
diff --git a/ucla-roms_amd/csrc/roms_dev.h b/ucla-roms_amd/csrc/roms_dev.h
--- a/ucla-roms_amd/csrc/roms_dev.h
+++ b/ucla-roms_amd/csrc/roms_dev.h
@@ -56,7 +56,8 @@
   int preuv_lds;
   int seg_jrows;
   int seg_buf;
-  int reserved_[8];
+  int vgrid2;
+  int reserved_[7];
   int s2d_k;
   int uv2e_nc, uv2e_nf;
   int npip;
@@ -72,6 +73,8 @@
   double rdrg, Zob, Tcoef, T0, Scoef, S0;
   double Akv_bak, Akt_bak[2];
 };
+static_assert(offsetof(Params, s2d_k) == 196 && offsetof(Params, ubind) == 240 && sizeof(Params) == 384,
+              "Params: no member from s2d_k on may move");
 
 struct Fields {
   double *h, *hinv, *f, *fomn, *pm, *pn, *dm_r, *dn_r, *dm_u, *dn_u, *dm_v, *dn_v, *dm_p, *dn_p,
@@ -151,6 +154,8 @@
 
 constexpr int kVgRho = 1, kVgKppExt = 2, kVgKppInt = 4, kVgHuv = 8, kVgAll = 15;
 constexpr int kVgDefault = kVgRho | kVgKppExt | kVgHuv;
+constexpr int kVg2Omega = 1, kVg2Huv1 = 2, kVg2Uv2 = 4, kVg2Visc = 8, kVg2T3dmix = 16, kVg2All = 31, kVg2Shift = 8;
+constexpr int kVg2Default = kVg2All;
 struct VGrid {
   const double *Cs_w, *Cs_r;
   double z, h, hinv, hc, ds;
diff --git a/ucla-roms_amd/csrc/roms_shim.cpp b/ucla-roms_amd/csrc/roms_shim.cpp
--- a/ucla-roms_amd/csrc/roms_shim.cpp
+++ b/ucla-roms_amd/csrc/roms_shim.cpp
@@ -109,7 +109,7 @@
 }
 void vg_set(bool valid) {
   g.vgrid_valid = valid;
-  g.d.p.vg = valid ? g.d.p.vgrid : (short)0;
+  g.d.p.vg = valid ? (short)(g.d.p.vgrid | (g.d.p.vgrid2 << kVg2Shift)) : (short)0;
 }
 void vg_host_write(int id) {
   if (id != ROMS_Hz && id != ROMS_z_r && id != ROMS_z_w && id != ROMS_h && id != ROMS_hinv && id != ROMS_Cs_w &&
@@ -755,6 +755,7 @@
   P.kpp_lean = (short)env_int("ROMS_GPU_KPP_LEAN", 7, 0, 7);
   P.kpp_fckeep = (short)env_int("ROMS_GPU_KPP_FCKEEP", kKppFcKeepMax, 1, kKppFcKeepMax);
   P.vgrid = (short)env_int("ROMS_GPU_VGRID", kVgDefault, 0, kVgAll);
+  P.vgrid2 = env_int("ROMS_GPU_VGRID2", kVg2Default, 0, kVg2All);
   P.vg = 0;
   g.vgrid_valid = false;
   P.hoist = !env_off("ROMS_GPU_HOIST");
@@ -1011,6 +1012,11 @@
 int roms_gpu_vgrid(void) {
   REQUIRE_INIT_NOJOIN();
   return g.d.p.vgrid + (g.vgrid_valid ? 256 : 0);
+}
+
+int roms_gpu_vgrid2(void) {
+  REQUIRE_INIT_NOJOIN();
+  return g.d.p.vgrid2 + (g.vgrid_valid ? 256 : 0);
 }
 
 int roms_gpu_vgrid_check(long out[3]) {
diff --git a/ucla-roms_amd/romsgpu/__init__.py b/ucla-roms_amd/romsgpu/__init__.py
--- a/ucla-roms_amd/romsgpu/__init__.py
+++ b/ucla-roms_amd/romsgpu/__init__.py
@@ -487,6 +487,11 @@
         self._chk(min(r, 0), "vgrid")
         return r % 256, bool(r // 256)
 
+    def vgrid2(self):
+        r = self.L.roms_gpu_vgrid2()
+        self._chk(min(r, 0), "vgrid2")
+        return r % 256, bool(r // 256)
+
     def vgrid_mismatch(self):
         out = (ctypes.c_long * 3)()
         self._chk(self.L.roms_gpu_vgrid_check(out), "vgrid_check")
```

New measurement: 2.369 billion cell-updates/s, median of 6. 1.02x the previous value.
